# nubot-nudt/LCR-Net

Measured on AMD Instinct MI355X. Metric: scans/s (120k-pt KITTI-shape scan -> 256-D descriptor), higher is better.
Workload: dtype f32 (K-deep GEMMs, K >= 288 and N >= 64: fp32 operands as bf16 x 3 split, 6 of 9 products on the bf16 matrix cores, fp32 accumulate — error vs fp64 <= the fp32-MFMA kernel's; every other GEMM, KPConv and attention: fp32 MFMA); 1 GPU; configs[1]: batch of 8 synthetic 64-beam scans (~120k pts, 0.3 m voxel -> ~16k pts), voxelise + 3 subsamples + 10 radius searches + KPConv encoder + NetVLAD, seeded random weights; distinct_input_batches=4, streams=pre-processing stream (own host thread, 2 batches ahead) + 2 encoder stream(s), parallelism=scan-parallel x1, all-gather of descriptors

## Files before the change

### include/lcr_hip.h

```cpp
#ifndef LCR_HIP_H
#define LCR_HIP_H
#include <stddef.h>
#include <stdint.h>
#ifdef __cplusplus
extern "C" {
#endif

#define LCR_OK 0
#define LCR_EARG (-1)
#define LCR_ESPACE (-2)
#define LCR_EHIP (-3)

#define LCR_STATUS_KEY_OVERFLOW 1u
#define LCR_STATUS_LEN_MISMATCH 2u
#define LCR_GN_REPLICAS 8

const char* lcr_last_error(void);
void lcr_ktimer_enable(int on);
void lcr_ktimer_sample(int every);
void lcr_ktimer_kinds(unsigned mask);
int lcr_ktimer_read(int kind, int max_records, double* seconds, int64_t* meta);
int lcr_ktimer_read2(int kind, int max_records, double* seconds, double* seconds_kernel, int64_t* meta);
int lcr_stream_spin(int microseconds, void* stream);
int lcr_version(void);

int lcr_grid_subsample_ws_bytes(int64_t n_cap, int B, size_t* bytes);
int lcr_grid_subsample(const float* xyz, const int64_t* len, int B, int64_t n_cap, float voxel,
                       float* out_xyz, int64_t* out_len, uint32_t* status,
                       void* ws, size_t ws_bytes, void* stream);
int lcr_grid_subsample_ex(const float* xyz, const int64_t* len, int B, int64_t n_cap, float voxel, int key_bits_hint,
                          float* out_xyz, int64_t* out_len, uint32_t* status,
                          void* ws, size_t ws_bytes, void* stream);
int lcr_grid_subsample_rows(const float* xyz, int row_floats, const int64_t* len, int B, int64_t n_cap, float voxel, int key_bits_hint,
                            float* out_xyz, int64_t* out_len, uint32_t* status,
                            void* ws, size_t ws_bytes, void* stream);
int lcr_hashmap_order_host(const uint64_t* keys_host, int64_t n, int64_t* order_host);
int lcr_hashmap_bucket_host(const uint64_t* codes_host, int64_t n, int phase, int64_t* out_host);

int lcr_voxel_down_sample_ws_bytes(int64_t n_cap, int B, size_t* bytes);
int lcr_voxel_down_sample(const float* rows, int row_floats, int out_cols, const int64_t* len, int B, int64_t n_cap, double voxel,
                          int key_bits_hint, float* out_f32, double* out_f64, int64_t* out_len, uint32_t* status,
                          void* ws, size_t ws_bytes, void* stream);

int lcr_support_grid_ws_bytes(int64_t ns_cap, int B, size_t* bytes);
int lcr_support_grid_build(const float* s, const int64_t* slen, int B, int64_t ns_cap, float radius,
                           uint32_t* status, void* grid_ws, size_t grid_ws_bytes, void* stream);
int lcr_radius_query(const float* q, const int64_t* qlen, int B, int64_t nq_cap,
                     const void* grid_ws, int64_t ns_cap , float radius, int limit,
                     int64_t* out_idx64, int32_t* out_idx32, int32_t* out_cnt, void* stream);
int lcr_radius_query_ordered(const float* q, const int64_t* qlen, int B, int64_t nq_cap,
                             const void* grid_ws, int64_t ns_cap, float radius, int limit,
                             int64_t* out_idx64, int32_t* out_idx32, int32_t* out_cnt, const int32_t* q_order, void* stream);
typedef struct LcrRadiusQuery {
    const float*   q;
    const int64_t* qlen;
    int64_t        nq_cap;
    const void*    grid_ws;
    int64_t        ns_cap;
    float          radius;
    int            limit;
    int32_t*       out_idx32;
    const int32_t* q_order;
} LcrRadiusQuery;
#define LCR_RADIUS_QUERY_MULTI_MAX 12
int lcr_radius_query_multi(const LcrRadiusQuery* list, int n, int B, void* stream);
int lcr_support_grid_build_ex(const float* s, const int64_t* slen, int B, int64_t ns_cap, float radius,
                              uint32_t* status, void* grid_ws, size_t grid_ws_bytes, int32_t* order, void* stream);
int lcr_support_grid_order(const void* grid_ws, int64_t ns_cap, int B, int32_t* order, void* stream);
int lcr_radius_search_ws_bytes(int64_t nq_cap, int64_t ns_cap, int B, size_t* bytes);
int lcr_radius_search(const float* q, const float* s, const int64_t* qlen, const int64_t* slen, int B,
                      int64_t nq_cap, int64_t ns_cap, float radius, int limit,
                      int64_t* out_idx64, int32_t* out_idx32, int32_t* out_cnt, uint32_t* status,
                      void* ws, size_t ws_bytes, void* stream);

#define LCR_MAX_STAGES 8
typedef struct LcrPrecomputeLayout {
  int     num_stages, B, upsampling;
  int64_t n_raw;
  int     limits[LCR_MAX_STAGES];
  int64_t cap[LCR_MAX_STAGES];
  size_t  off_points[LCR_MAX_STAGES];
  size_t  off_lengths[LCR_MAX_STAGES];
  size_t  off_order[LCR_MAX_STAGES];
  size_t  off_neighbors[LCR_MAX_STAGES];
  size_t  off_subsampling[LCR_MAX_STAGES];
  size_t  off_upsampling[LCR_MAX_STAGES];
  size_t  out_bytes, ws_bytes;
} LcrPrecomputeLayout;
int lcr_precompute_layout(int64_t n0, int B, int num_stages, const int* limits, int upsampling, int64_t n_raw,
                          LcrPrecomputeLayout* layout);
int lcr_precompute_batch(const float* points0, const int64_t* lengths0, const LcrPrecomputeLayout* layout, float voxel_size,
                         float radius, float raw_voxel, int key_bits_hint, void* out, size_t out_bytes, void* ws, size_t ws_bytes,
                         int64_t* lengths_host, uint32_t* status_host, void* stream);
int lcr_precompute_batch_rows(const float* points0, int raw_row_floats, const int64_t* lengths0, const LcrPrecomputeLayout* layout,
                              float voxel_size, float radius, float raw_voxel, int key_bits_hint, void* out, size_t out_bytes, void* ws,
                              size_t ws_bytes, int64_t* lengths_host, uint32_t* status_host, void* stream);
int lcr_precompute_ws_bytes_ex(const LcrPrecomputeLayout* layout, int raw_method, size_t* bytes);
int lcr_precompute_batch_rows_ex(const float* points0, int raw_row_floats, const int64_t* lengths0, const LcrPrecomputeLayout* layout,
                                 float voxel_size, float radius, double raw_voxel, int raw_method, int key_bits_hint, void* out,
                                 size_t out_bytes, void* ws, size_t ws_bytes, int64_t* lengths_host, uint32_t* status_host, void* stream);

int lcr_gemm_f32(const float* A, const float* B, float* C, int64_t M, int N, int K, int transA, int transB,
                 const float* bias, const float* rowdiv, const int64_t* seg_len, int S, int groups, double* stats,
                 void* stream);
int lcr_split_bf16x3(const float* w, int64_t n, uint16_t* planes, void* stream);
int lcr_split_bf16x3_tiles(const float* w, int N, int K, uint16_t* tiles, void* stream);
int lcr_gemm_f32_bsplit(const float* A, const uint16_t* Bs_tiles, float* C, int64_t M, int N, int K, const float* bias, const float* rowdiv,
                        const int64_t* seg_len, int S, int groups, double* stats, void* stream);
int lcr_gemm_f32_masked(const float* A, const float* B, float* C, int64_t M, int N, int K, const float* bias, const float* rowdiv,
                        const int64_t* seg_len, int S, int groups, double* stats, const uint16_t* row_mask, int block_k, void* stream);
int lcr_gemm_f32_bsplit_masked(const float* A, const uint16_t* Bs_tiles, float* C, int64_t M, int N, int K, const float* bias,
                               const float* rowdiv, const int64_t* seg_len, int S, int groups, double* stats, const uint16_t* row_mask,
                               int block_k, void* stream);
int lcr_kpconv_mask_ok(int64_t M, int N, int K, int split);
int lcr_gemm_f32_anorm(const float* A, const float* B, float* C, int64_t M, int N, int K, const float* bias,
                       const double* a_stats, const float* a_gamma, const float* a_beta, int a_groups, float a_eps,
                       float a_slope, const int64_t* seg_len, int S, int groups, double* stats, void* stream);
int lcr_gemm_f32_batched_ta(const float* A, const float* B, float* C, int64_t M, int N, int count, const int* k_host,
                            const int64_t* a_off_host, const int64_t* b_off_host, const int64_t* c_off_host, void* stream);
int lcr_kpconv_aggregate(const float* s_feats, const uint8_t* s_pos, const float* q_pts, const float* s_pts,
                         const void* idx, int idx_is_64, int64_t M, int64_t Ns, int H, int C,
                         const float* kernel_points_host, float sigma, float* A, float* nn,
                         const int32_t* order , void* stream);
#define LCR_KP_VALID_FIRST 1
int lcr_kpconv_aggregate_ex(const float* s_feats, const uint8_t* s_pos, const float* q_pts, const float* s_pts,
                            const void* idx, int idx_is_64, int64_t M, int64_t Ns, int H, int C,
                            const float* kernel_points_host, float sigma, float* A, float* nn,
                            const int32_t* order, int flags, void* stream);
int lcr_kpconv_aggregate_mask(const float* s_feats, const uint8_t* s_pos, const float* q_pts, const float* s_pts,
                              const void* idx, int idx_is_64, int64_t M, int64_t Ns, int H, int C,
                              const float* kernel_points_host, float sigma, float* A, float* nn, uint16_t* mask,
                              const int32_t* order, int flags, void* stream);
int lcr_kpconv_fused(const float* s_feats, const uint8_t* s_pos, const float* q_pts, const float* s_pts, const void* idx,
                     int idx_is_64, int64_t M, int64_t Ns, int H, int C, const float* kernel_points_host, float sigma,
                     const float* W, const float* bias, float* out, const int64_t* seg_len, int S, int groups, double* stats,
                     const int32_t* order, void* stream);
int lcr_kpconv_cin1(const float* s_feats, const float* q_pts, const float* s_pts, const void* idx, int idx_is_64,
                    int64_t M, int64_t Ns, int H, const float* kernel_points_host, float sigma, const float* W,
                    const float* bias, int Cout, float* out, const int32_t* order, void* stream);
int lcr_maxpool(const float* x, const void* idx, int idx_is_64, int64_t M, int64_t Ns, int H, int C, float* out,
                const int32_t* order, void* stream);
int lcr_row_positive(const float* x, int64_t N, int C, uint8_t* pos, void* stream);
int lcr_groupnorm_stats(const float* x, int64_t N, int C, int groups, const int64_t* seg_len, int S, double* stats, void* stream);
int lcr_groupnorm_apply(const float* x, const double* stats, const float* gamma, const float* beta, const float* res,
                        const double* res_stats, const float* res_gamma, const float* res_beta, float* y, int64_t N, int C,
                        int groups, const int64_t* seg_len, int S, float eps, float slope, int act, uint8_t* pos, void* stream);

#define LCR_ENC_BLOCKS 10
typedef struct LcrUnaryW {
  const float *w, *b;
  const float *gn_w, *gn_b;
  const uint16_t* w_split;
} LcrUnaryW;
typedef struct LcrBlockW {
  int   cin, cout, strided;
  float sigma;
  const float* kernel_points_host;
  const float *kp_w, *kp_b;
  const float* kp_wt;
  const uint16_t* kp_wt_split;
  const float *normconv_w, *normconv_b;
  LcrUnaryW unary1, unary2, shortcut;
} LcrBlockW;
typedef struct LcrEncoderW {
  int   groups, c1_cout;
  float c1_sigma;
  const float* c1_kernel_points_host;
  const float *c1_w, *c1_b;
  const float *c1_gn_w, *c1_gn_b;
  LcrBlockW blocks[LCR_ENC_BLOCKS];
} LcrEncoderW;
int lcr_encoder_ws_bytes(const LcrEncoderW* W, const int64_t* n_host, int S, size_t* bytes);
int lcr_encoder_forward(const LcrEncoderW* W, const float* feats0, const float* const* points, const int32_t* const* neighbors,
                        const int32_t* const* subsampling, const int32_t* const* order, const int64_t* const* seg_len, int S,
                        const int64_t* n_host, const int64_t* seg_min_rows_host, const int* limits, float* const* out_feats, void* ws,
                        size_t ws_bytes, void* stream);
#define LCR_ENC_LISTS_VALID_FIRST 1u
int lcr_encoder_forward_ex(const LcrEncoderW* W, const float* feats0, const float* const* points, const int32_t* const* neighbors,
                           const int32_t* const* subsampling, const int32_t* const* order, const int64_t* const* seg_len, int S,
                           const int64_t* n_host, const int64_t* seg_min_rows_host, const int* limits, float* const* out_feats,
                           unsigned flags, void* ws, size_t ws_bytes, void* stream);

typedef struct LcrNetvladWeights {
  const float* cluster_weights;
  const float* cluster_weights2;
  const float* hidden1_weights;
  const float *bn1_w, *bn1_b, *bn1_mean, *bn1_var;
  const float *bn2_w, *bn2_b, *bn2_mean, *bn2_var;
  const float* gating_weights;
  const float *gbn_w, *gbn_b, *gbn_mean, *gbn_var;
} LcrNetvladWeights;
int lcr_netvlad_ws_bytes(int64_t n_rows, int S, size_t* bytes);
int lcr_netvlad_forward(const float* feats , const int64_t* seg_len_host, int S,
                        const LcrNetvladWeights* weights_host, float* out , void* ws, size_t ws_bytes, void* stream);

int lcr_rotary_embed(float* x, const float* theta, int64_t N, int heads, void* stream);
int lcr_attention_f32(const float* q, const float* k, const float* v, int64_t Nq, int64_t Nk, int heads, int head_dim,
                      float* out, void* stream);
int lcr_attention_seg_f32(const float* q, const float* k, const float* v, const int64_t* q_len_host, const int64_t* k_len_host, int P,
                          int heads, int head_dim, float* out, void* stream);
int lcr_attention_topk_f32(const float* q, const float* k, const float* v, const int64_t* q_len_host, const int64_t* k_len_host,
                           const int* kk_host, int P, int heads, int head_dim, float* out, void* stream);
int lcr_add_layernorm(const float* a, const float* b, const float* gamma, const float* beta, int64_t N, int D, float eps,
                      float* y, void* stream);
int lcr_relu_inplace(float* x, int64_t n, void* stream);

#define LCR_ROFORMER_MAX_BLOCKS 16
typedef struct LcrLinearW {
  const float *w, *b;
} LcrLinearW;
typedef struct LcrRoformerLayerW {
  LcrLinearW   q, k, v, lin;
  const float *ln1_w, *ln1_b;
  float        ln1_eps;
  LcrLinearW   expand, squeeze;
  const float *ln2_w, *ln2_b;
  float        ln2_eps;
} LcrRoformerLayerW;
typedef struct LcrRoformerW {
  int        d_in, d_model, d_out, heads, num_blocks;
  int        block_is_self[LCR_ROFORMER_MAX_BLOCKS];
  LcrLinearW emb1, emb2, in_proj, out_proj;
  LcrRoformerLayerW layers[LCR_ROFORMER_MAX_BLOCKS];
} LcrRoformerW;
int lcr_roformer_ws_bytes(const LcrRoformerW* W, int64_t n_rows, size_t* bytes);
int lcr_roformer_forward(const LcrRoformerW* W, const float* points, const float* feats, const int64_t* lens0_host, const int64_t* lens1_host,
                         int P, float* out, float* theta_out, void* ws, size_t ws_bytes, void* stream);

int lcr_retrieval_ws_bytes(int64_t Q, int64_t C, size_t* bytes);
int lcr_retrieval_topk(const float* queries , int64_t Q, int64_t q0, const float* database , int64_t C,
                       int D, int k, int exclude, int32_t* out_idx , float* out_d2 ,
                       void* ws, size_t ws_bytes, void* stream);

int lcr_gemm_f32_strided_batched(const float* A, const float* B, float* C, int64_t M, int N, int K, int transA, int transB,
                                 int64_t strideA, int64_t strideB, int64_t strideC, int count, void* stream);

int lcr_vote_shift(const float* xyz, const float* offsets, int64_t N, float max_range, float* out, void* stream);
int lcr_greedy_nms_ws_bytes(int64_t n_total, size_t* bytes);
int lcr_greedy_nms(const float* pts, const int64_t* len, int B, int64_t n_total, float radius, uint8_t* keep,
                   int64_t* out_len, void* ws, void* stream);
int lcr_neighbor_mean(const float* pts, const void* idx, int idx_is_64, int64_t M, int H, int64_t pad, float* out, void* stream);
int lcr_point_to_node_ws_bytes(int64_t N, int M, size_t* bytes);
int lcr_point_to_node_partition(const float* points, int64_t N, const float* nodes, int M, int K, int32_t* p2n, int64_t* knn,
                                uint8_t* knn_mask, uint8_t* node_mask, uint32_t* status, void* ws, size_t ws_bytes, void* stream);

int lcr_point_to_node_partition_stack(const float* points, const int64_t* point_off, const float* nodes, const int64_t* node_off, int C, int K,
                                      int32_t* p2n_out, int64_t* knn, uint8_t* knn_mask, uint8_t* node_mask, uint32_t* status, void* ws,
                                      size_t ws_bytes, void* stream);
int lcr_build_padded_scores(const float* raw, const uint8_t* row_mask, const uint8_t* col_mask, int64_t B, int M, int N,
                            float scale, const float* alpha, float inf_val, float* S, void* stream);
int lcr_log_sinkhorn(float* S, const uint8_t* row_mask, const uint8_t* col_mask, int64_t B, int M, int N, int iters,
                     float inf_val, float* uv_ws, void* stream);
int lcr_log_sinkhorn_ws_floats(int64_t B, int M, int N, size_t* floats);
int lcr_log_sinkhorn_form(int64_t B, int M, int N, int* form);
int lcr_log_sinkhorn_ex(float* S, const uint8_t* row_mask, const uint8_t* col_mask, int64_t B, int M, int N, int iters,
                        float inf_val, float* uv_ws, size_t uv_floats, void* stream);
int lcr_top1_matching_ws_bytes(int64_t B, int M, int N, size_t* bytes);
int lcr_top1_matching(const float* logS, int64_t B, int M, int N, const uint8_t* row_mask, const uint8_t* col_mask,
                      int64_t* total, int32_t* out_bij, float* out_score, void* ws, size_t ws_bytes, void* stream);
int lcr_top1_matching_ex(const float* logS, int64_t B, int M, int N, const uint8_t* row_mask, const uint8_t* col_mask, int mutual,
                         int64_t* total, int32_t* out_bij, float* out_score, void* ws, size_t ws_bytes, void* stream);
int lcr_patch_scores(const float* feats_a, int64_t Na, const float* feats_b, int64_t Nb, int C, const int64_t* idx_a, const int64_t* idx_b,
                     const uint8_t* mask_a, const uint8_t* mask_b, int64_t P, int K, float scale, const float* alpha, float inf_val, float* S,
                     void* stream);
int lcr_topk_matching_ws_bytes(int64_t B, int M, int N, size_t* bytes);
int lcr_topk_matching(const float* logS, int64_t B, int M, int N, const uint8_t* row_mask, const uint8_t* col_mask, int K, int mutual,
                      int64_t* total, int32_t* out_bij, float* out_score, void* ws, size_t ws_bytes, void* stream);
int lcr_topk_matching_ex(const float* logS, int64_t B, int M, int N, const uint8_t* row_mask, const uint8_t* col_mask, int K, int mutual,
                         int use_dustbin, float confidence_threshold, const float* global_scores, int64_t* total, int32_t* out_bij,
                         float* out_score, void* ws, size_t ws_bytes, void* stream);
int lcr_upsample_concat(const float* x, int64_t Nx, int C1, const void* idx, int idx_is_64, int H, const float* skip, int C2,
                        int64_t N, float* out, void* stream);
int lcr_gather_rows(const float* src, int64_t pad, int C, const int64_t* idx, int64_t R, float* out, void* stream);
int lcr_procrustes_batched(const float* src, const float* ref, const float* w, const int32_t* start, int P, float eps, float* T, void* stream);
int lcr_inlier_count(const float* T, int P, const float* src, const float* ref, int n, float radius, const int32_t* start,
                     int min_count, int32_t* counts, int32_t* best, void* stream);
int lcr_lgr_ws_bytes(int64_t n, int H, int S, size_t* bytes);
int lcr_local_global_registration(const float* src, const float* ref, const float* score, int64_t n, const int32_t* hyp_start, int H,
                                  const int32_t* seg_hyp_start, int S, float radius, int min_count, int steps, float* T_out,
                                  float* hyp_out, int32_t* counts_out, int32_t* best_out, void* ws, size_t ws_bytes, void* stream);
int lcr_local_global_registration_ex(const float* src, const float* ref, const float* score, int64_t n, const int32_t* hyp_start, int H,
                                     const int32_t* seg_hyp_start, int S, float radius, int min_count, int steps, int correspondence_limit,
                                     float* T_out, float* hyp_out, int32_t* counts_out, int32_t* best_out, void* ws, size_t ws_bytes,
                                     void* stream);
int lcr_inlier_weights(const float* T_all, const int32_t* sel, const float* src, const float* ref, const float* score, int n,
                       float radius, float* w_out, void* stream);

int lcr_ransac_ws_bytes(int S, int iterations, size_t* bytes);
int lcr_ransac_correspondences(const float* src, const float* ref, const int32_t* start, int S, float thr, int ransac_n, int iterations,
                               uint64_t seed, float* T, int32_t* inliers, float* rmse, int32_t* best_h, float* T_all, int32_t* counts_all,
                               float* sse_all, void* ws, size_t ws_bytes, void* stream);
int lcr_ransac_sample_host(uint64_t seed, int64_t h0, int64_t count, int ransac_n, int64_t n, int32_t* idx_host);
int lcr_ransac_ex_ws_bytes(int S, int iterations, int64_t n_corr, size_t* bytes);
int lcr_ransac_correspondences_ex(const float* src, const float* ref, const int32_t* start, int S, const int32_t* corr, const int32_t* src_start,
                                  const int32_t* ref_start, int64_t n_corr, float thr, int ransac_n, int iterations, uint64_t seed,
                                  float edge_similarity, float checker_distance, float* T, int32_t* inliers, float* rmse, int32_t* best_h,
                                  float* T_all, int32_t* counts_all, float* sse_all, uint8_t* reject_all, void* ws, size_t ws_bytes, void* stream);

int lcr_feature_nn_ws_bytes(int S, int64_t nq, int64_t nd, size_t* bytes);
int lcr_feature_nn(const float* qf, const float* df, const int32_t* q_start, const int32_t* d_start, int S, int C, int64_t nq, int64_t nd,
                   int32_t* nn, float* d2, void* ws, size_t ws_bytes, void* stream);
int lcr_feature_correspondences_ws_bytes(int S, size_t* bytes);
int lcr_feature_correspondences(const int32_t* nn_sr, const int32_t* src_start, const int32_t* nn_rs, const int32_t* ref_start, int S, int min_rows,
                                int32_t* corr, int32_t* start, int32_t* mutual_used, void* ws, size_t ws_bytes, void* stream);

#define LCR_STATUS_CAP_EXCEEDED 4u
int lcr_node_correspondences_ws_bytes(const int64_t* point_off, const int64_t* node_off, int P, int K, size_t* bytes);
int lcr_node_correspondences(const float* points, const int64_t* point_off, const float* nodes, const int64_t* node_off, const int64_t* knn,
                             const uint8_t* knn_mask, const uint8_t* node_mask, const float* transforms, int P, int K, double pos_radius,
                             int64_t cap, int32_t* corr, float* overlap, int32_t* start, uint32_t* status, void* ws, size_t ws_bytes,
                             void* stream);

int lcr_icp_ws_bytes(int S, int64_t ns, int64_t nt, size_t* bytes);
int lcr_icp_point_to_point(const float* src, const int64_t* src_len, const float* tgt, const int64_t* tgt_len, int S, const double* init,
                           float max_correspondence_distance, int max_iteration, double relative_fitness, double relative_rmse, double* T,
                           double* fitness, double* inlier_rmse, int32_t* iterations, int32_t* corr, double* T_hist, double* fitness_hist,
                           double* rmse_hist, int check_every, void* ws, size_t ws_bytes, void* stream);

int lcr_icp_plane_ws_bytes(int S, int64_t ns, int64_t nt, size_t* bytes);
int lcr_icp_point_to_plane(const float* src, const int64_t* src_len, const float* tgt, const int64_t* tgt_len, const float* tgt_normals, int S,
                           const double* init, float max_correspondence_distance, int max_iteration, double relative_fitness,
                           double relative_rmse, double* T, double* fitness, double* inlier_rmse, int32_t* iterations, int32_t* corr,
                           double* T_hist, double* fitness_hist, double* rmse_hist, int check_every, void* ws, size_t ws_bytes, void* stream);

int lcr_normals_ws_bytes(int B, int64_t n, size_t* bytes);
int lcr_estimate_normals(const float* points, const int64_t* lengths, int B, float radius, int max_nn, const float* viewpoint, float* normals,
                         float* curvature, int32_t* count, void* ws, size_t ws_bytes, void* stream);

int lcr_fpfh_ws_bytes(int B, int64_t n, int max_nn, size_t* bytes);
int lcr_fpfh(const float* points, const float* normals, const int64_t* lengths, int B, float radius, int max_nn, float* features, float* spfh,
             int32_t* count, void* ws, size_t ws_bytes, void* stream);

int lcr_range_images_ws_bytes(int B, size_t* bytes);
int lcr_range_images(const float* points, const int64_t* lengths, int B, int H, int W, double fov_up, double fov_down, double max_range,
                     float* images, int32_t* valid, void* ws, size_t ws_bytes, void* stream);
int lcr_scan_overlap_ws_bytes(int B, int64_t P, size_t* bytes);
int lcr_scan_overlap(const float* points, const int64_t* lengths, int B, const float* images, const int32_t* valid, const int32_t* pairs,
                     const double* rel, int64_t P, int H, int W, double fov_up, double fov_down, double max_range, double eps, int32_t* counts,
                     int32_t* status, void* ws, size_t ws_bytes, void* stream);

#define LCR_STATUS_INDEX_RANGE 8u
#define LCR_GAP_LABELS_POINTS 0
#define LCR_GAP_LABELS_OVERLAPS 1
int lcr_gap_loss_ws_bytes(int64_t rows, int64_t cols, size_t* bytes);
int lcr_gap_loss(const float* S, const int64_t* soff, const int64_t* roff, const int64_t* coff, const int32_t* seg_start, int64_t B, int P,
                 int n_max, int m_max, int64_t elems, int64_t rows, int64_t cols, int source, const float* p_pts, const float* q_pts,
                 const float* transforms, double positive_radius, const int64_t* corr, const float* overlaps, const int32_t* corr_start,
                 int64_t C, int64_t c_max, double positive_overlap, const uint8_t* pmask, const uint8_t* qmask, double gamma, float* terms,
                 int32_t* kept, uint8_t* labels, double* line_pos, double* line_hinge, int32_t* line_count, int32_t* line_active,
                 uint32_t* status, void* ws, size_t ws_bytes, void* stream);
int lcr_gap_loss_grad(const float* S, const int64_t* soff, const int64_t* roff, const int64_t* coff, const int32_t* seg_start, int64_t B,
                      int P, int n_max, int m_max, int64_t elems, int64_t rows, int64_t cols, double gamma, const float* upstream,
                      const int32_t* kept, const uint8_t* labels, const double* line_pos, const double* line_hinge,
                      const int32_t* line_count, const int32_t* line_active, float* dS, void* stream);
int lcr_min_dist(const float* A, const int32_t* a_start, int64_t na, const float* D, const int32_t* d_start, int64_t nd,
                 const uint8_t* valid, int P, int64_t q_max, float* dist, int32_t* arg, float* mean, int32_t* count, void* stream);
int lcr_min_dist_grad(const float* A, const int32_t* a_start, int64_t na, const float* D, const int32_t* d_start, int64_t nd,
                      const uint8_t* valid, int P, int64_t q_max, const int32_t* arg, const float* dist, const int32_t* count,
                      const float* upstream, float* dA, void* stream);

#ifdef __cplusplus
}
#endif
#endif
```

### lcr-net_amd/_lib.py

```python
import ctypes
import os

import torch

_PKG = os.path.dirname(os.path.abspath(__file__))
LIB_PATH = os.path.join(_PKG, "liblcr_hip.so")

_lib = None

c_f32p = ctypes.c_void_p
c_vp = ctypes.c_void_p
c_i64 = ctypes.c_int64
c_int = ctypes.c_int
c_float = ctypes.c_float
c_size_p = ctypes.POINTER(ctypes.c_size_t)
c_size_t = ctypes.c_size_t

_SIGS = {
    "lcr_last_error": (ctypes.c_char_p, []),
    "lcr_version": (c_int, []),
    "lcr_support_grid_ws_bytes": (c_int, [c_i64, c_int, c_size_p]),
    "lcr_support_grid_build": (c_int, [c_vp, c_vp, c_int, c_i64, c_float, c_vp, c_vp, ctypes.c_size_t, c_vp]),
    "lcr_precompute_layout": (c_int, [c_i64, c_int, c_int, c_vp, c_int, c_i64, c_vp]),
    "lcr_precompute_batch": (c_int, [c_vp, c_vp, c_vp, c_float, c_float, c_float, c_int, c_vp, c_size_t, c_vp, c_size_t, c_vp, c_vp, c_vp]),
    "lcr_precompute_batch_rows": (c_int, [c_vp, c_int, c_vp, c_vp, c_float, c_float, c_float, c_int, c_vp, c_size_t, c_vp, c_size_t, c_vp, c_vp, c_vp]),
    "lcr_precompute_ws_bytes_ex": (c_int, [c_vp, c_int, c_size_p]),
    "lcr_precompute_batch_rows_ex": (c_int, [c_vp, c_int, c_vp, c_vp, c_float, c_float, ctypes.c_double, c_int, c_int, c_vp, c_size_t, c_vp, c_size_t,
                                             c_vp, c_vp, c_vp]),
    "lcr_radius_query_multi": (c_int, [c_vp, c_int, c_int, c_vp]),
    "lcr_radius_query": (c_int, [c_vp, c_vp, c_int, c_i64, c_vp, c_i64, c_float, c_int, c_vp, c_vp, c_vp, c_vp]),
    "lcr_stream_spin": (c_int, [c_int, c_vp]),
    "lcr_radius_query_ordered": (c_int, [c_vp, c_vp, c_int, c_i64, c_vp, c_i64, c_float, c_int, c_vp, c_vp, c_vp, c_vp, c_vp]),
    "lcr_radius_search_ws_bytes": (c_int, [c_i64, c_i64, c_int, c_size_p]),
    "lcr_radius_search": (c_int, [c_vp, c_vp, c_vp, c_vp, c_int, c_i64, c_i64, c_float, c_int, c_vp, c_vp, c_vp, c_vp,
                                  c_vp, ctypes.c_size_t, c_vp]),
    "lcr_grid_subsample_ws_bytes": (c_int, [c_i64, c_int, c_size_p]),
    "lcr_grid_subsample": (c_int, [c_vp, c_vp, c_int, c_i64, c_float, c_vp, c_vp, c_vp, c_vp, ctypes.c_size_t, c_vp]),
    "lcr_grid_subsample_ex": (c_int, [c_vp, c_vp, c_int, c_i64, c_float, c_int, c_vp, c_vp, c_vp, c_vp, ctypes.c_size_t, c_vp]),
    "lcr_grid_subsample_rows": (c_int, [c_vp, c_int, c_vp, c_int, c_i64, c_float, c_int, c_vp, c_vp, c_vp, c_vp, ctypes.c_size_t, c_vp]),
    "lcr_hashmap_order_host": (c_int, [c_vp, c_i64, c_vp]),
    "lcr_hashmap_bucket_host": (c_int, [c_vp, c_i64, c_int, c_vp]),
    "lcr_voxel_down_sample_ws_bytes": (c_int, [c_i64, c_int, c_size_p]),
    "lcr_voxel_down_sample": (c_int, [c_vp, c_int, c_int, c_vp, c_int, c_i64, ctypes.c_double, c_int, c_vp, c_vp, c_vp, c_vp, c_vp, ctypes.c_size_t,
                                      c_vp]),
    "lcr_gemm_f32": (c_int, [c_vp, c_vp, c_vp, c_i64, c_int, c_int, c_int, c_int, c_vp, c_vp, c_vp, c_int, c_int, c_vp, c_vp]),
    "lcr_gemm_f32_anorm": (c_int, [c_vp, c_vp, c_vp, c_i64, c_int, c_int, c_vp, c_vp, c_vp, c_vp, c_int, c_float, c_float, c_vp, c_int,
                                   c_int, c_vp, c_vp]),
    "lcr_ktimer_enable": (None, [c_int]),
    "lcr_ktimer_sample": (None, [c_int]),
    "lcr_ktimer_kinds": (None, [ctypes.c_uint]),
    "lcr_ktimer_read": (c_int, [c_int, c_int, c_vp, c_vp]),
    "lcr_ktimer_read2": (c_int, [c_int, c_int, c_vp, c_vp, c_vp]),
    "lcr_encoder_ws_bytes": (c_int, [c_vp, c_vp, c_int, c_size_p]),
    "lcr_encoder_forward": (c_int, [c_vp, c_vp, c_vp, c_vp, c_vp, c_vp, c_vp, c_int, c_vp, c_vp, c_vp, c_vp, c_vp, c_size_t, c_vp]),
    "lcr_roformer_ws_bytes": (c_int, [c_vp, c_i64, c_size_p]),
    "lcr_roformer_forward": (c_int, [c_vp, c_vp, c_vp, c_vp, c_vp, c_int, c_vp, c_vp, c_vp, c_size_t, c_vp]),
    "lcr_encoder_forward_ex": (c_int, [c_vp, c_vp, c_vp, c_vp, c_vp, c_vp, c_vp, c_int, c_vp, c_vp, c_vp, c_vp, ctypes.c_uint, c_vp, c_size_t, c_vp]),
    "lcr_kpconv_aggregate": (c_int, [c_vp, c_vp, c_vp, c_vp, c_vp, c_int, c_i64, c_i64, c_int, c_int, c_vp, c_float, c_vp, c_vp, c_vp, c_vp]),
    "lcr_kpconv_aggregate_mask": (c_int, [c_vp, c_vp, c_vp, c_vp, c_vp, c_int, c_i64, c_i64, c_int, c_int, c_vp, c_float, c_vp, c_vp, c_vp, c_vp,
                                          c_int, c_vp]),
    "lcr_kpconv_fused": (c_int, [c_vp, c_vp, c_vp, c_vp, c_vp, c_int, c_i64, c_i64, c_int, c_int, c_vp, c_float, c_vp, c_vp, c_vp, c_vp, c_int,
                                 c_int, c_vp, c_vp, c_vp]),
    "lcr_kpconv_cin1": (c_int, [c_vp, c_vp, c_vp, c_vp, c_int, c_i64, c_i64, c_int, c_vp, c_float, c_vp, c_vp, c_int, c_vp, c_vp, c_vp]),
    "lcr_maxpool": (c_int, [c_vp, c_vp, c_int, c_i64, c_i64, c_int, c_int, c_vp, c_vp, c_vp]),
    "lcr_support_grid_order": (c_int, [c_vp, c_i64, c_int, c_vp, c_vp]),
    "lcr_row_positive": (c_int, [c_vp, c_i64, c_int, c_vp, c_vp]),
    "lcr_groupnorm_stats": (c_int, [c_vp, c_i64, c_int, c_int, c_vp, c_int, c_vp, c_vp]),
    "lcr_groupnorm_apply": (c_int, [c_vp, c_vp, c_vp, c_vp, c_vp, c_vp, c_vp, c_vp, c_vp, c_i64, c_int, c_int, c_vp, c_int,
                                    c_float, c_float, c_int, c_vp, c_vp]),
    "lcr_rotary_embed": (c_int, [c_vp, c_vp, c_i64, c_int, c_vp]),
    "lcr_attention_f32": (c_int, [c_vp, c_vp, c_vp, c_i64, c_i64, c_int, c_int, c_vp, c_vp]),
    "lcr_attention_seg_f32": (c_int, [c_vp, c_vp, c_vp, c_vp, c_vp, c_int, c_int, c_int, c_vp, c_vp]),
    "lcr_attention_topk_f32": (c_int, [c_vp, c_vp, c_vp, c_vp, c_vp, c_vp, c_int, c_int, c_int, c_vp, c_vp]),
    "lcr_add_layernorm": (c_int, [c_vp, c_vp, c_vp, c_vp, c_i64, c_int, c_float, c_vp, c_vp]),
    "lcr_relu_inplace": (c_int, [c_vp, c_i64, c_vp]),
    "lcr_retrieval_ws_bytes": (c_int, [c_i64, c_i64, c_size_p]),
    "lcr_retrieval_topk": (c_int, [c_vp, c_i64, c_i64, c_vp, c_i64, c_int, c_int, c_int, c_vp, c_vp, c_vp, ctypes.c_size_t, c_vp]),
    "lcr_gemm_f32_strided_batched": (c_int, [c_vp, c_vp, c_vp, c_i64, c_int, c_int, c_int, c_int, c_i64, c_i64, c_i64, c_int, c_vp]),
    "lcr_gemm_f32_batched_ta": (c_int, [c_vp, c_vp, c_vp, c_i64, c_int, c_int, c_vp, c_vp, c_vp, c_vp, c_vp]),
    "lcr_vote_shift": (c_int, [c_vp, c_vp, c_i64, c_float, c_vp, c_vp]),
    "lcr_greedy_nms_ws_bytes": (c_int, [c_i64, c_size_p]),
    "lcr_greedy_nms": (c_int, [c_vp, c_vp, c_int, c_i64, c_float, c_vp, c_vp, c_vp, c_vp]),
    "lcr_neighbor_mean": (c_int, [c_vp, c_vp, c_int, c_i64, c_int, c_i64, c_vp, c_vp]),
    "lcr_point_to_node_ws_bytes": (c_int, [c_i64, c_int, c_size_p]),
    "lcr_point_to_node_partition": (c_int, [c_vp, c_i64, c_vp, c_int, c_int, c_vp, c_vp, c_vp, c_vp, c_vp, c_vp, ctypes.c_size_t, c_vp]),
    "lcr_point_to_node_partition_stack": (c_int, [c_vp, c_vp, c_vp, c_vp, c_int, c_int, c_vp, c_vp, c_vp, c_vp, c_vp, c_vp, ctypes.c_size_t, c_vp]),
    "lcr_build_padded_scores": (c_int, [c_vp, c_vp, c_vp, c_i64, c_int, c_int, c_float, c_vp, c_float, c_vp, c_vp]),
    "lcr_log_sinkhorn": (c_int, [c_vp, c_vp, c_vp, c_i64, c_int, c_int, c_int, c_float, c_vp, c_vp]),
    "lcr_log_sinkhorn_ws_floats": (c_int, [c_i64, c_int, c_int, c_size_p]),
    "lcr_log_sinkhorn_form": (c_int, [c_i64, c_int, c_int, ctypes.POINTER(c_int)]),
    "lcr_split_bf16x3": (c_int, [c_vp, c_i64, c_vp, c_vp]),
    "lcr_split_bf16x3_tiles": (c_int, [c_vp, c_int, c_int, c_vp, c_vp]),
    "lcr_gemm_f32_bsplit": (c_int, [c_vp, c_vp, c_vp, c_i64, c_int, c_int, c_vp, c_vp, c_vp, c_int, c_int, c_vp, c_vp]),
    "lcr_gemm_f32_bsplit_masked": (c_int, [c_vp, c_vp, c_vp, c_i64, c_int, c_int, c_vp, c_vp, c_vp, c_int, c_int, c_vp, c_vp, c_int, c_vp]),
    "lcr_gemm_f32_masked": (c_int, [c_vp, c_vp, c_vp, c_i64, c_int, c_int, c_vp, c_vp, c_vp, c_int, c_int, c_vp, c_vp, c_int, c_vp]),
    "lcr_kpconv_mask_ok": (c_int, [c_i64, c_int, c_int, c_int]),
    "lcr_log_sinkhorn_ex": (c_int, [c_vp, c_vp, c_vp, c_i64, c_int, c_int, c_int, c_float, c_vp, ctypes.c_size_t, c_vp]),
    "lcr_top1_matching_ws_bytes": (c_int, [c_i64, c_int, c_int, c_size_p]),
    "lcr_top1_matching": (c_int, [c_vp, c_i64, c_int, c_int, c_vp, c_vp, c_vp, c_vp, c_vp, c_vp, ctypes.c_size_t, c_vp]),
    "lcr_top1_matching_ex": (c_int, [c_vp, c_i64, c_int, c_int, c_vp, c_vp, c_int, c_vp, c_vp, c_vp, c_vp, ctypes.c_size_t, c_vp]),
    "lcr_topk_matching_ws_bytes": (c_int, [c_i64, c_int, c_int, c_size_p]),
    "lcr_topk_matching": (c_int, [c_vp, c_i64, c_int, c_int, c_vp, c_vp, c_int, c_int, c_vp, c_vp, c_vp, c_vp, ctypes.c_size_t, c_vp]),
    "lcr_patch_scores": (c_int, [c_vp, c_i64, c_vp, c_i64, c_int, c_vp, c_vp, c_vp, c_vp, c_i64, c_int, c_float, c_vp, c_float, c_vp, c_vp]),
    "lcr_topk_matching_ex": (c_int, [c_vp, c_i64, c_int, c_int, c_vp, c_vp, c_int, c_int, c_int, c_float, c_vp, c_vp, c_vp, c_vp, c_vp, ctypes.c_size_t,
                                     c_vp]),
    "lcr_local_global_registration_ex": (c_int, [c_vp, c_vp, c_vp, c_i64, c_vp, c_int, c_vp, c_int, c_float, c_int, c_int, c_int, c_vp, c_vp, c_vp, c_vp,
                                                 c_vp, ctypes.c_size_t, c_vp]),
    "lcr_upsample_concat": (c_int, [c_vp, c_i64, c_int, c_vp, c_int, c_int, c_vp, c_int, c_i64, c_vp, c_vp]),
    "lcr_gather_rows": (c_int, [c_vp, c_i64, c_int, c_vp, c_i64, c_vp, c_vp]),
    "lcr_procrustes_batched": (c_int, [c_vp, c_vp, c_vp, c_vp, c_int, c_float, c_vp, c_vp]),
    "lcr_inlier_count": (c_int, [c_vp, c_int, c_vp, c_vp, c_int, c_float, c_vp, c_int, c_vp, c_vp, c_vp]),
    "lcr_inlier_weights": (c_int, [c_vp, c_vp, c_vp, c_vp, c_vp, c_int, c_float, c_vp, c_vp]),
    "lcr_lgr_ws_bytes": (c_int, [c_i64, c_int, c_int, c_size_p]),
    "lcr_local_global_registration": (c_int, [c_vp, c_vp, c_vp, c_i64, c_vp, c_int, c_vp, c_int, c_float, c_int, c_int, c_vp, c_vp, c_vp, c_vp, c_vp,
                                              ctypes.c_size_t, c_vp]),
    "lcr_netvlad_ws_bytes": (c_int, [c_i64, c_int, c_size_p]),
    "lcr_netvlad_forward": (c_int, [c_vp, c_vp, c_int, c_vp, c_vp, c_vp, ctypes.c_size_t, c_vp]),
    "lcr_ransac_ws_bytes": (c_int, [c_int, c_int, c_size_p]),
    "lcr_ransac_correspondences": (c_int, [c_vp, c_vp, c_vp, c_int, c_float, c_int, c_int, ctypes.c_uint64, c_vp, c_vp, c_vp, c_vp, c_vp, c_vp, c_vp,
                                           c_vp, ctypes.c_size_t, c_vp]),
    "lcr_ransac_sample_host": (c_int, [ctypes.c_uint64, c_i64, c_i64, c_int, c_i64, c_vp]),
    "lcr_ransac_ex_ws_bytes": (c_int, [c_int, c_int, c_i64, c_size_p]),
    "lcr_ransac_correspondences_ex": (c_int, [c_vp, c_vp, c_vp, c_int, c_vp, c_vp, c_vp, c_i64, c_float, c_int, c_int, ctypes.c_uint64, c_float,
                                              c_float, c_vp, c_vp, c_vp, c_vp, c_vp, c_vp, c_vp, c_vp, c_vp, ctypes.c_size_t, c_vp]),
    "lcr_feature_nn_ws_bytes": (c_int, [c_int, c_i64, c_i64, c_size_p]),
    "lcr_feature_nn": (c_int, [c_vp, c_vp, c_vp, c_vp, c_int, c_int, c_i64, c_i64, c_vp, c_vp, c_vp, ctypes.c_size_t, c_vp]),
    "lcr_feature_correspondences_ws_bytes": (c_int, [c_int, c_size_p]),
    "lcr_feature_correspondences": (c_int, [c_vp, c_vp, c_vp, c_vp, c_int, c_int, c_vp, c_vp, c_vp, c_vp, ctypes.c_size_t, c_vp]),
    "lcr_node_correspondences_ws_bytes": (c_int, [c_vp, c_vp, c_int, c_int, c_size_p]),
    "lcr_node_correspondences": (c_int, [c_vp, c_vp, c_vp, c_vp, c_vp, c_vp, c_vp, c_vp, c_int, c_int, ctypes.c_double, c_i64, c_vp, c_vp, c_vp,
                                         c_vp, c_vp, ctypes.c_size_t, c_vp]),
    "lcr_icp_ws_bytes": (c_int, [c_int, c_i64, c_i64, c_size_p]),
    "lcr_icp_point_to_point": (c_int, [c_vp, c_vp, c_vp, c_vp, c_int, c_vp, c_float, c_int, ctypes.c_double, ctypes.c_double, c_vp, c_vp, c_vp, c_vp,
                                       c_vp, c_vp, c_vp, c_vp, c_int, c_vp, ctypes.c_size_t, c_vp]),
    "lcr_icp_plane_ws_bytes": (c_int, [c_int, c_i64, c_i64, c_size_p]),
    "lcr_icp_point_to_plane": (c_int, [c_vp, c_vp, c_vp, c_vp, c_vp, c_int, c_vp, c_float, c_int, ctypes.c_double, ctypes.c_double, c_vp, c_vp,
                                       c_vp, c_vp, c_vp, c_vp, c_vp, c_vp, c_int, c_vp, ctypes.c_size_t, c_vp]),
    "lcr_normals_ws_bytes": (c_int, [c_int, c_i64, c_size_p]),
    "lcr_estimate_normals": (c_int, [c_vp, c_vp, c_int, c_float, c_int, c_vp, c_vp, c_vp, c_vp, c_vp, ctypes.c_size_t, c_vp]),
    "lcr_fpfh_ws_bytes": (c_int, [c_int, c_i64, c_int, c_size_p]),
    "lcr_fpfh": (c_int, [c_vp, c_vp, c_vp, c_int, c_float, c_int, c_vp, c_vp, c_vp, c_vp, ctypes.c_size_t, c_vp]),
    "lcr_range_images_ws_bytes": (c_int, [c_int, c_size_p]),
    "lcr_range_images": (c_int, [c_vp, c_vp, c_int, c_int, c_int, ctypes.c_double, ctypes.c_double, ctypes.c_double, c_vp, c_vp, c_vp,
                                 ctypes.c_size_t, c_vp]),
    "lcr_scan_overlap_ws_bytes": (c_int, [c_int, c_i64, c_size_p]),
    "lcr_scan_overlap": (c_int, [c_vp, c_vp, c_int, c_vp, c_vp, c_vp, c_vp, c_i64, c_int, c_int, ctypes.c_double, ctypes.c_double, ctypes.c_double,
                                 ctypes.c_double, c_vp, c_vp, c_vp, ctypes.c_size_t, c_vp]),
    "lcr_gap_loss_ws_bytes": (c_int, [c_i64, c_i64, c_size_p]),
    "lcr_gap_loss": (c_int, [c_vp, c_vp, c_vp, c_vp, c_vp, c_i64, c_int, c_int, c_int, c_i64, c_i64, c_i64, c_int, c_vp, c_vp, c_vp,
                             ctypes.c_double, c_vp, c_vp, c_vp, c_i64, c_i64, ctypes.c_double, c_vp, c_vp, ctypes.c_double, c_vp, c_vp, c_vp,
                             c_vp, c_vp, c_vp, c_vp, c_vp, c_vp, ctypes.c_size_t, c_vp]),
    "lcr_gap_loss_grad": (c_int, [c_vp, c_vp, c_vp, c_vp, c_vp, c_i64, c_int, c_int, c_int, c_i64, c_i64, c_i64, ctypes.c_double, c_vp, c_vp,
                                  c_vp, c_vp, c_vp, c_vp, c_vp, c_vp, c_vp]),
    "lcr_min_dist": (c_int, [c_vp, c_vp, c_i64, c_vp, c_vp, c_i64, c_vp, c_int, c_i64, c_vp, c_vp, c_vp, c_vp, c_vp]),
    "lcr_min_dist_grad": (c_int, [c_vp, c_vp, c_i64, c_vp, c_vp, c_i64, c_vp, c_int, c_i64, c_vp, c_vp, c_vp, c_vp, c_vp, c_vp]),
}


_RELEASES_GIL = {"lcr_roformer_forward", "lcr_precompute_batch", "lcr_precompute_batch_rows", "lcr_precompute_batch_rows_ex", "lcr_hashmap_bucket_host", "lcr_encoder_forward", "lcr_encoder_forward_ex", "lcr_ktimer_read",
                 "lcr_ktimer_read2", "lcr_hashmap_order_host", "lcr_ransac_sample_host", "lcr_icp_point_to_point", "lcr_icp_point_to_plane", "lcr_netvlad_forward", "lcr_log_sinkhorn", "lcr_log_sinkhorn_ex",
                 "lcr_local_global_registration", "lcr_local_global_registration_ex", "lcr_retrieval_topk", "lcr_stream_spin"}


def build():
    import importlib.util
    spec = importlib.util.spec_from_file_location("_lcr_build", os.path.join(_PKG, "csrc", "build.py"))
    mod = importlib.util.module_from_spec(spec)
    spec.loader.exec_module(mod)
    return mod.build()


def lib():
    global _lib
    if _lib is None:
        if not os.path.exists(LIB_PATH):
            raise RuntimeError(
                "liblcr_hip.so not found at %s — build it with `python lcr-net_amd/csrc/build.py` "
                "(there is no CPU fallback for the lcr-net_amd hot path)" % LIB_PATH)
        L = ctypes.CDLL(LIB_PATH)
        for name, (res, args) in _SIGS.items():
            if not hasattr(L, name):
                continue
            fn = getattr(L, name)
            fn.restype = res
            fn.argtypes = args
        if os.environ.get("LCR_CTYPES_KEEP_GIL", "1") != "0":
            K = ctypes.PyDLL(LIB_PATH)
            for name, (res, args) in _SIGS.items():
                if name in _RELEASES_GIL or not hasattr(K, name):
                    continue
                fn = getattr(K, name)
                fn.restype = res
                fn.argtypes = args
                setattr(L, name, fn)
        _lib = L
    return _lib


def check(rc, what):
    if rc != 0:
        msg = lib().lcr_last_error()
        raise RuntimeError("%s failed (rc=%d): %s" % (what, rc, msg.decode() if msg else ""))


def ptr(t):
    return ctypes.c_void_p(t.data_ptr()) if t is not None else ctypes.c_void_p(0)


def stream_ptr(device=None):
    idx = device.index if isinstance(device, torch.device) else None
    if idx is None:
        idx = torch.cuda.current_device() if not isinstance(device, int) else device
    return ctypes.c_void_p(torch._C._cuda_getCurrentRawStream(idx))


def require_cuda(*tensors):
    for t in tensors:
        if t is not None and not t.is_cuda:
            raise RuntimeError("lcr-net_amd ops run on the GPU only: got a %s tensor (no CPU fallback)" % t.device)


def workspace(nbytes, device):
    return torch.empty(max(int(nbytes), 256), dtype=torch.uint8, device=device)
```

### lcr-net_amd/csrc/encoder.hip

```cpp
#include <algorithm>
#include <cstdlib>
#include <cstring>

#include "common.h"

#define TURN(call) ([&]() { LaunchTurn turn_; return (call); }())

namespace lcr {

constexpr float ENC_GN_EPS = 1e-5f;
constexpr float ENC_SLOPE = 0.1f;

struct Arena {
  char*  base;
  size_t off, cap;
  template <typename T>
  T* take(size_t n) {
    const size_t o = off;
    off = align_up(off + n * sizeof(T));
    return (base && off <= cap) ? reinterpret_cast<T*>(base + o) : nullptr;
  }
};

struct StageIO {
  const float*   pts;
  const int64_t* seg;
  const int32_t* order;
  int64_t        n;
  int64_t        min_rows;
};

struct StatsPool {
  double* base;
  size_t  off, cap;
  int     S, groups;
  double* take() {
    const size_t n = static_cast<size_t>(GN_REPLICAS) * S * groups * 2;
    if (off + n > cap) return nullptr;
    double* p = base + off;
    off += n;
    return p;
  }
};

static size_t stats_doubles(int S, int groups) { return static_cast<size_t>(GN_REPLICAS) * S * groups * 2 * 44; }

static int unary_raw(const LcrUnaryW& u, const float* x, int64_t n, int cin, int cout, const StageIO& st, StatsPool& sp, Arena& ws,
                     float** y_out, double** stats_out, hipStream_t s) {
  float* y = ws.take<float>(static_cast<size_t>(n) * cout);
  double* stats = sp.take();
  if (!y || !stats) return LCR_ESPACE;
  const bool split = u.w_split && cin >= 288 && cin % 32 == 0 && cout >= 64;
  int rc = split ? TURN(lcr_gemm_f32_bsplit(x, u.w_split, y, n, cout, cin, u.b, nullptr, st.seg, sp.S, sp.groups, stats, s))
                 : TURN(lcr_gemm_f32(x, u.w, y, n, cout, cin, 0, 1, u.b, nullptr, st.seg, sp.S, sp.groups, stats, s));
  *y_out = y;
  *stats_out = stats;
  return rc;
}

static int residual_block(const LcrBlockW& b, const float* s_feats, const StageIO& q, const StageIO& sup, const void* idx, int H,
                          StatsPool& sp, Arena& ws, float* out, unsigned enc_flags, hipStream_t s) {
  const int mid = b.cout / 4, g = sp.groups;
  const int64_t M = q.n, Ns = sup.n;
  int rc;
  const float* x = s_feats;
  uint8_t* pos = ws.take<uint8_t>(static_cast<size_t>(Ns));
  if (!pos) return LCR_ESPACE;
  if (b.unary1.w) {
    float* y1;
    double* st1;
    if ((rc = unary_raw(b.unary1, s_feats, Ns, b.cin, mid, sup, sp, ws, &y1, &st1, s))) return rc;
    float* x1 = ws.take<float>(static_cast<size_t>(Ns) * mid);
    if (!x1) return LCR_ESPACE;
    if ((rc = TURN(lcr_groupnorm_apply(y1, st1, b.unary1.gn_w, b.unary1.gn_b, nullptr, nullptr, nullptr, nullptr, x1, Ns, mid, g, sup.seg, sp.S,
                                  ENC_GN_EPS, ENC_SLOPE, 1, pos, s))))
      return rc;
    x = x1;
  } else if ((rc = TURN(lcr_row_positive(s_feats, Ns, b.cin, pos, s)))) {
    return rc;
  }
  float* A = ws.take<float>(static_cast<size_t>(M) * 15 * mid);
  float* nn = ws.take<float>(static_cast<size_t>(M));
  float* kpo = ws.take<float>(static_cast<size_t>(M) * mid);
  uint16_t* kmask = ws.take<uint16_t>(static_cast<size_t>(M));
  double* stc = sp.take();
  if (!A || !nn || !kpo || !kmask || !stc) return LCR_ESPACE;
  static const bool vf_env_off = getenv("LCR_KP_VALID_FIRST") && atoi(getenv("LCR_KP_VALID_FIRST")) == 0;
  const int vf_flag = ((enc_flags & LCR_ENC_LISTS_VALID_FIRST) && !vf_env_off) ? LCR_KP_VALID_FIRST : 0;
  static const bool fused32 = getenv("LCR_KPCONV_FUSED") != nullptr;
  if (fused32 && mid == 32 && sp.S <= 64) {
    if ((rc = TURN(lcr_kpconv_fused(x, pos, q.pts, sup.pts, idx, 0, M, Ns, H, mid, b.kernel_points_host, b.sigma, b.kp_w, b.kp_b, kpo, q.seg, sp.S, g,
                                    stc, q.order, s))))
      return rc;
  } else {
    const bool split = b.kp_wt_split && mid >= 64;
    if (!((split || b.kp_wt) && lcr_kpconv_mask_ok(M, mid, 15 * mid, split))) kmask = nullptr;
    if ((rc = TURN(lcr_kpconv_aggregate_mask(x, pos, q.pts, sup.pts, idx, 0, M, Ns, H, mid, b.kernel_points_host, b.sigma, A, nn, kmask, q.order, vf_flag,
                                             s))))
      return rc;
    if (split) {
      if ((rc = TURN(kmask ? lcr_gemm_f32_bsplit_masked(A, b.kp_wt_split, kpo, M, mid, 15 * mid, b.kp_b, nn, q.seg, sp.S, g, stc, kmask, mid, s)
                           : lcr_gemm_f32_bsplit(A, b.kp_wt_split, kpo, M, mid, 15 * mid, b.kp_b, nn, q.seg, sp.S, g, stc, s))))
        return rc;
    } else if (kmask) {
      if ((rc = TURN(lcr_gemm_f32_masked(A, b.kp_wt, kpo, M, mid, 15 * mid, b.kp_b, nn, q.seg, sp.S, g, stc, kmask, mid, s)))) return rc;
    } else if ((rc = TURN(b.kp_wt ? lcr_gemm_f32(A, b.kp_wt, kpo, M, mid, 15 * mid, 0, 1, b.kp_b, nn, q.seg, sp.S, g, stc, s)
                                  : lcr_gemm_f32(A, b.kp_w, kpo, M, mid, 15 * mid, 0, 0, b.kp_b, nn, q.seg, sp.S, g, stc, s)))) return rc;
  }
  float* y;
  double* sty;
  static const bool no_anorm = getenv("LCR_NO_NORM_ON_LOAD") != nullptr;
  if (!no_anorm && mid <= 256 && mid % 4 == 0 && b.cout > 32 && q.min_rows >= 64) {
    y = ws.take<float>(static_cast<size_t>(M) * b.cout);
    sty = sp.take();
    if (!y || !sty) return LCR_ESPACE;
    if ((rc = TURN(lcr_gemm_f32_anorm(kpo, b.unary2.w, y, M, b.cout, mid, b.unary2.b, stc, b.normconv_w, b.normconv_b, g, ENC_GN_EPS, ENC_SLOPE,
                                      q.seg, sp.S, g, sty, s))))
      return rc;
  } else {
    float* x2 = ws.take<float>(static_cast<size_t>(M) * mid);
    if (!x2) return LCR_ESPACE;
    if ((rc = TURN(lcr_groupnorm_apply(kpo, stc, b.normconv_w, b.normconv_b, nullptr, nullptr, nullptr, nullptr, x2, M, mid, g, q.seg, sp.S, ENC_GN_EPS,
                                  ENC_SLOPE, 1, nullptr, s))))
      return rc;
    if ((rc = unary_raw(b.unary2, x2, M, mid, b.cout, q, sp, ws, &y, &sty, s))) return rc;
  }
  const float* res = s_feats;
  if (b.strided) {
    float* pooled = ws.take<float>(static_cast<size_t>(M) * b.cin);
    if (!pooled) return LCR_ESPACE;
    if ((rc = TURN(lcr_maxpool(s_feats, idx, 0, M, Ns, H, b.cin, pooled, q.order, s)))) return rc;
    res = pooled;
  }
  const double* str = nullptr;
  if (b.shortcut.w) {
    float* r;
    double* st;
    if ((rc = unary_raw(b.shortcut, res, M, b.cin, b.cout, q, sp, ws, &r, &st, s))) return rc;
    res = r;
    str = st;
  }
  return TURN(lcr_groupnorm_apply(y, sty, b.unary2.gn_w, b.unary2.gn_b, res, str, str ? b.shortcut.gn_w : nullptr, str ? b.shortcut.gn_b : nullptr, out,
                             M, b.cout, g, q.seg, sp.S, ENC_GN_EPS, ENC_SLOPE, 1, nullptr, s));
}

static size_t block_ws_bytes(const LcrBlockW& b, int64_t M, int64_t Ns) {
  Arena a{nullptr, 0, ~size_t(0)};
  const int mid = b.cout / 4;
  a.take<uint8_t>(Ns);
  a.take<float>(static_cast<size_t>(Ns) * mid);
  a.take<float>(static_cast<size_t>(Ns) * mid);
  a.take<float>(static_cast<size_t>(M) * 15 * mid);
  a.take<float>(M);
  a.take<float>(static_cast<size_t>(M) * mid);
  a.take<uint16_t>(static_cast<size_t>(M));
  a.take<float>(static_cast<size_t>(M) * mid);
  a.take<float>(static_cast<size_t>(M) * b.cout);
  a.take<float>(static_cast<size_t>(M) * b.cin);
  a.take<float>(static_cast<size_t>(M) * b.cout);
  return a.off;
}

static const int BLOCK_Q[LCR_ENC_BLOCKS] = {0, 1, 1, 1, 2, 2, 2, 3, 3, 3};
static const int BLOCK_S[LCR_ENC_BLOCKS] = {0, 0, 1, 1, 1, 2, 2, 2, 3, 3};

}

using namespace lcr;

extern "C" int lcr_encoder_ws_bytes(const LcrEncoderW* W, const int64_t* n_host, int S, size_t* bytes) {
  if (!W || !n_host || !bytes || S < 1) return LCR_EARG;
  size_t blk = 0, pp = 0;
  for (int i = 0; i < LCR_ENC_BLOCKS; ++i) {
    blk = std::max(blk, block_ws_bytes(W->blocks[i], n_host[BLOCK_Q[i]], n_host[BLOCK_S[i]]));
    pp = std::max(pp, align_up(sizeof(float) * static_cast<size_t>(n_host[BLOCK_Q[i]]) * W->blocks[i].cout));
  }
  pp = std::max(pp, align_up(sizeof(float) * static_cast<size_t>(n_host[0]) * W->c1_cout * 2));
  *bytes = blk + 2 * pp + align_up(sizeof(double) * stats_doubles(S, W->groups)) + 4096;
  return LCR_OK;
}

extern "C" int lcr_encoder_forward(const LcrEncoderW* W, const float* feats0, const float* const* points, const int32_t* const* neighbors,
                                   const int32_t* const* subsampling, const int32_t* const* order, const int64_t* const* seg_len, int S,
                                   const int64_t* n_host, const int64_t* seg_min_rows_host, const int* limits, float* const* out_feats,
                                   void* ws, size_t ws_bytes, void* stream) {
  return lcr_encoder_forward_ex(W, feats0, points, neighbors, subsampling, order, seg_len, S, n_host, seg_min_rows_host, limits, out_feats, 0u, ws,
                                ws_bytes, stream);
}

extern "C" int lcr_encoder_forward_ex(const LcrEncoderW* W, const float* feats0, const float* const* points, const int32_t* const* neighbors,
                                      const int32_t* const* subsampling, const int32_t* const* order, const int64_t* const* seg_len, int S,
                                      const int64_t* n_host, const int64_t* seg_min_rows_host, const int* limits, float* const* out_feats,
                                      unsigned flags, void* ws, size_t ws_bytes, void* stream) {
  if (!W || !feats0 || !points || !neighbors || !subsampling || !seg_len || !n_host || !limits || !out_feats || !ws || S < 1) {
    set_error("lcr_encoder_forward: bad argument");
    return LCR_EARG;
  }
  size_t need = 0;
  lcr_encoder_ws_bytes(W, n_host, S, &need);
  if (ws_bytes < need) {
    set_error("lcr_encoder_forward: workspace too small (%zu < %zu)", ws_bytes, need);
    return LCR_ESPACE;
  }
  hipStream_t s = static_cast<hipStream_t>(stream);
  StageIO st[4];
  for (int i = 0; i < 4; ++i) st[i] = StageIO{points[i], seg_len[i], order ? order[i] : nullptr, n_host[i], seg_min_rows_host ? seg_min_rows_host[i] : 0};
  Arena top{static_cast<char*>(ws), 0, ws_bytes};
  StatsPool sp{top.take<double>(stats_doubles(S, W->groups)), 0, stats_doubles(S, W->groups), S, W->groups};
  size_t pp = 0;
  for (int i = 0; i < LCR_ENC_BLOCKS; ++i) pp = std::max(pp, sizeof(float) * static_cast<size_t>(n_host[BLOCK_Q[i]]) * W->blocks[i].cout);
  pp = std::max(pp, sizeof(float) * static_cast<size_t>(n_host[0]) * W->c1_cout * 2);
  float* ping = reinterpret_cast<float*>(top.take<char>(pp));
  float* pong = reinterpret_cast<float*>(top.take<char>(pp));
  const size_t scratch0 = top.off;
  if (!sp.base || !ping || !pong) return LCR_ESPACE;
  hipMemsetAsync(sp.base, 0, sizeof(double) * sp.cap, s);

  int rc;
  float* cur;
  {
    const int64_t n0 = n_host[0];
    float* raw = ping;
    float* f = ping + static_cast<size_t>(n0) * W->c1_cout;
    double* stt = sp.take();
    if ((rc = TURN(lcr_kpconv_cin1(feats0, st[0].pts, st[0].pts, neighbors[0], 0, n0, n0, limits[0], W->c1_kernel_points_host, W->c1_sigma, W->c1_w,
                              W->c1_b, W->c1_cout, raw, st[0].order, s))))
      return rc;
    if ((rc = TURN(lcr_groupnorm_stats(raw, n0, W->c1_cout, W->groups, st[0].seg, S, stt, s)))) return rc;
    if ((rc = TURN(lcr_groupnorm_apply(raw, stt, W->c1_gn_w, W->c1_gn_b, nullptr, nullptr, nullptr, nullptr, f, n0, W->c1_cout, W->groups, st[0].seg, S,
                                  ENC_GN_EPS, ENC_SLOPE, 1, nullptr, s))))
      return rc;
    cur = f;
  }
  static const int STAGE_LAST[4] = {0, 3, 6, 9};
  for (int i = 0; i < LCR_ENC_BLOCKS; ++i) {
    const int qs = BLOCK_Q[i], ss = BLOCK_S[i];
    const bool strided = qs != ss;
    const void* idx = strided ? static_cast<const void*>(subsampling[ss]) : static_cast<const void*>(neighbors[qs]);
    const int H = limits[ss];
    float* out = nullptr;
    for (int k = 0; k < 4; ++k)
      if (STAGE_LAST[k] == i) out = out_feats[k];
    if (!out) out = (cur >= ping && cur < ping + pp / sizeof(float)) ? pong : ping;
    Arena scratch{static_cast<char*>(ws), scratch0, ws_bytes};
    if ((rc = residual_block(W->blocks[i], cur, st[qs], st[ss], idx, H, sp, scratch, out, flags, s))) {
      if (rc == LCR_ESPACE) set_error("lcr_encoder_forward: block %d ran out of workspace", i);
      return rc;
    }
    cur = out;
  }
  return check_launch("lcr_encoder_forward");
}
```

### lcr-net_amd/csrc/gemm_f32.hip

```cpp
#include <cstdio>
#include <cstdlib>
#include <map>
#include <mutex>
#include <type_traits>

#include "common.h"

namespace lcr {

typedef float floatx16 __attribute__((ext_vector_type(16)));

constexpr int GM_BK = 32;
constexpr int GM_T = 256;

constexpr int GM_MAX_BATCH = 64;
struct GemmBatch {
  int     count;
  int     strided;
  int     k[GM_MAX_BATCH];
  int64_t a_off[GM_MAX_BATCH], b_off[GM_MAX_BATCH], c_off[GM_MAX_BATCH];
};

struct GemmEpilogue {
  const float*   bias;
  const float*   rowdiv;
  const int64_t* seg_len;
  int            S;
  int            groups;
  double*        stats;
};

struct ANorm {
  const double* stats;
  const float*  gamma;
  const float*  beta;
  int           groups;
  float         eps, slope;
};
constexpr int AN_KMAX = 256;

__device__ __forceinline__ float4 ld4(const float* p) { return *reinterpret_cast<const float4*>(p); }

template <int R, int LD, bool VEC, bool RM = false>
struct LoaderT {
  static constexpr int PIECES = R * 8 / GM_T;
  float4 reg[PIECES];
  unsigned okmask;
  int kb;
  __device__ __forceinline__ void load(const float* __restrict__ src, int64_t rows_total, int K, int64_t r0, int k0) {
    kb = k0;
#pragma unroll
    for (int j = 0; j < PIECES; ++j) {
      const int f = threadIdx.x + GM_T * j;
      const int row = f >> 3, c4 = f & 7;
      int64_t gr = r0 + row;
      gr = gr < rows_total ? gr : rows_total - 1;
      const int gk = k0 + c4 * 4;
      if (VEC) {
        const bool ok = gk < K;
        reg[j] = ld4(src + gr * K + (ok ? gk : 0));
        okmask = j == 0 ? (ok ? 1u : 0u) : (okmask | (ok ? (1u << j) : 0u));
      } else {
        const float* p = src + gr * K;
        float4 v;
        v.x = gk + 0 < K ? p[gk + 0] : 0.f;
        v.y = gk + 1 < K ? p[gk + 1] : 0.f;
        v.z = gk + 2 < K ? p[gk + 2] : 0.f;
        v.w = gk + 3 < K ? p[gk + 3] : 0.f;
        reg[j] = v;
        okmask = ~0u;
      }
    }
  }
  __device__ __forceinline__ void store_piece(float* __restrict__ S, int j) const {
    const int f = threadIdx.x + GM_T * j;
    const int row = f >> 3, c4 = f & 7;
    const bool ok = (okmask >> j) & 1u;
    if (RM) {
      *reinterpret_cast<float4*>(&S[row * LD + c4 * 4]) = ok ? reg[j] : make_float4(0.f, 0.f, 0.f, 0.f);
      return;
    }
    S[(c4 * 4 + 0) * LD + row] = ok ? reg[j].x : 0.f;
    S[(c4 * 4 + 1) * LD + row] = ok ? reg[j].y : 0.f;
    S[(c4 * 4 + 2) * LD + row] = ok ? reg[j].z : 0.f;
    S[(c4 * 4 + 3) * LD + row] = ok ? reg[j].w : 0.f;
  }
  __device__ __forceinline__ void store(float* __restrict__ S) const {
#pragma unroll
    for (int j = 0; j < PIECES; ++j) store_piece(S, j);
  }
  __device__ __forceinline__ void store_norm(float* __restrict__ S, const float* __restrict__ tab, int split, float slope) const {
    static_assert(RM, "normalise-on-load is built for the row-major A tile");
#pragma unroll
    for (int j = 0; j < PIECES; ++j) {
      const int f = threadIdx.x + GM_T * j;
      const int row = f >> 3, c4 = f & 7;
      const bool ok = (okmask >> j) & 1u;
      const float* t = tab + (row >= split ? 2 * AN_KMAX : 0) + (ok ? kb + c4 * 4 : 0);
      const float4 sc = *reinterpret_cast<const float4*>(t), sh = *reinterpret_cast<const float4*>(t + AN_KMAX);
      float4 v;
      v.x = fmaf(reg[j].x, sc.x, sh.x), v.y = fmaf(reg[j].y, sc.y, sh.y), v.z = fmaf(reg[j].z, sc.z, sh.z), v.w = fmaf(reg[j].w, sc.w, sh.w);
      v.x = v.x > 0.f ? v.x : v.x * slope, v.y = v.y > 0.f ? v.y : v.y * slope;
      v.z = v.z > 0.f ? v.z : v.z * slope, v.w = v.w > 0.f ? v.w : v.w * slope;
      *reinterpret_cast<float4*>(&S[row * LD + c4 * 4]) = ok ? v : make_float4(0.f, 0.f, 0.f, 0.f);
    }
  }
};

template <int W, int LD, bool VEC>
struct LoaderN {
  static constexpr int PIECES = 8 * W / GM_T;
  float4 reg[PIECES];
  unsigned okmask;
  __device__ __forceinline__ void load(const float* __restrict__ src, int64_t cols_total, int K, int64_t c0, int k0) {
#pragma unroll
    for (int j = 0; j < PIECES; ++j) {
      const int f = threadIdx.x + GM_T * j;
      const int kr = f / (W / 4), c4 = f % (W / 4);
      const int gk = k0 + kr;
      const int64_t gc = c0 + c4 * 4;
      const bool kok = gk < K;
      const float* p = src + static_cast<int64_t>(kok ? gk : 0) * cols_total;
      if (VEC) {
        const bool ok = kok && gc < cols_total;
        reg[j] = ld4(p + (gc < cols_total ? gc : 0));
        okmask = j == 0 ? (ok ? 1u : 0u) : (okmask | (ok ? (1u << j) : 0u));
      } else {
        float4 v;
        v.x = (kok && gc + 0 < cols_total) ? p[gc + 0] : 0.f;
        v.y = (kok && gc + 1 < cols_total) ? p[gc + 1] : 0.f;
        v.z = (kok && gc + 2 < cols_total) ? p[gc + 2] : 0.f;
        v.w = (kok && gc + 3 < cols_total) ? p[gc + 3] : 0.f;
        reg[j] = v;
        okmask = ~0u;
      }
    }
  }
  __device__ __forceinline__ void store_piece(float* __restrict__ S, int j) const {
    const int f = threadIdx.x + GM_T * j;
    const int kr = f / (W / 4), c4 = f % (W / 4);
    const bool ok = (okmask >> j) & 1u;
    *reinterpret_cast<float4*>(&S[kr * LD + c4 * 4]) = ok ? reg[j] : make_float4(0.f, 0.f, 0.f, 0.f);
  }
  __device__ __forceinline__ void store(float* __restrict__ S) const {
#pragma unroll
    for (int j = 0; j < PIECES; ++j) store_piece(S, j);
  }
};

__device__ __forceinline__ int seg_of_row(const int64_t* __restrict__ seg_len, int S, int64_t row) {
  int s = 0;
  int64_t end = seg_len[0];
  while (s + 1 < S && row >= end) {
    ++s;
    end += seg_len[s];
  }
  return s;
}

template <int BM, int BN, int WM, int WN, int NT>
__device__ __forceinline__ void gemm_epilogue(floatx16 (&acc)[NT], float* __restrict__ C, int64_t M, int N, int64_t m0, int n0, int64_t m_tile,
                                              const GemmEpilogue& ep, const float (&bias_v)[NT], int blk_first, int64_t blk_seg_start,
                                              int64_t blk_seg_end, int wm, int wn, int lane) {
  const bool want_stats = ep.stats != nullptr;
  const int gs = want_stats ? N / ep.groups : 1;
  const int64_t wrow0 = m0 + wm * 32;

  const bool interior = m0 + BM <= M && n0 + BN <= N && M * static_cast<int64_t>(N) < (int64_t(1) << 30);
  if (interior) {
    const unsigned row_l = static_cast<unsigned>(wrow0) + 4u * static_cast<unsigned>(lane >> 5);
#pragma unroll
    for (int j = 0; j < NT; ++j) {
      const unsigned col = static_cast<unsigned>(n0 + wn * (32 * NT) + j * 32 + (lane & 31));
      const float bv = bias_v[j];
      const unsigned off0 = row_l * static_cast<unsigned>(N) + col;
      if (ep.rowdiv) {
#pragma unroll
        for (int r = 0; r < 16; ++r) {
          const unsigned dr = static_cast<unsigned>((r & 3) + 8 * (r >> 2));
          const float v = acc[j][r] / ep.rowdiv[row_l + dr] + bv;
          C[off0 + dr * static_cast<unsigned>(N)] = v;
          acc[j][r] = v;
        }
      } else {
#pragma unroll
        for (int r = 0; r < 16; ++r) {
          const unsigned dr = static_cast<unsigned>((r & 3) + 8 * (r >> 2));
          const float v = acc[j][r] + bv;
          C[off0 + dr * static_cast<unsigned>(N)] = v;
          acc[j][r] = v;
        }
      }
    }
  } else
#pragma unroll
  for (int j = 0; j < NT; ++j) {
    const int col = n0 + wn * (32 * NT) + j * 32 + (lane & 31);
    const float bv = bias_v[j];
#pragma unroll
    for (int r = 0; r < 16; ++r) {
      const int64_t row = wrow0 + (r & 3) + 8 * (r >> 2) + 4 * (lane >> 5);
      float v = acc[j][r];
      if (row < M) {
        if (ep.rowdiv) v = v / ep.rowdiv[row];
        v += bv;
        if (col < N) C[row * N + col] = v;
      } else {
        v = 0.f;
      }
      acc[j][r] = v;
    }
  }

  if (want_stats) {
    __shared__ float s_part[2][2 * WM][BN];
    double* rep = ep.stats + static_cast<int64_t>(m_tile % GN_REPLICAS) * ep.S * ep.groups * 2;
    int64_t seg_start = blk_seg_start, seg_end = blk_seg_end;
    const int64_t blk_last_row = min(m0 + BM - 1, M - 1);
    constexpr int GN_EXACT_ROWS = 32;
    auto exact_segment = [&](int64_t rows) { return rows < GN_EXACT_ROWS && gs <= 32; };
    const bool uniform = blk_last_row < seg_end && !exact_segment(seg_end - seg_start);
    if (uniform) {
#pragma unroll
      for (int j = 0; j < NT; ++j) {
        float s = 0.f, ss = 0.f;
#pragma unroll
        for (int r = 0; r < 16; ++r) {
          s += acc[j][r];
          ss = fmaf(acc[j][r], acc[j][r], ss);
        }
        const int cl = wn * (32 * NT) + j * 32 + (lane & 31);
        s_part[0][2 * wm + (lane >> 5)][cl] = s;
        s_part[1][2 * wm + (lane >> 5)][cl] = ss;
      }
      __syncthreads();
      if (threadIdx.x < BN) {
        const int cl = threadIdx.x;
        double ds = 0.0, dss = 0.0;
#pragma unroll
        for (int r = 0; r < 2 * WM; ++r) {
          ds += static_cast<double>(s_part[0][r][cl]);
          dss += static_cast<double>(s_part[1][r][cl]);
        }
        const int span = gs < 64 ? gs : 64;
        for (int d = 1; d < span; d <<= 1) {
          ds += __shfl_xor(ds, d);
          dss += __shfl_xor(dss, d);
        }
        const int col = n0 + cl;
        if ((cl & (span - 1)) == 0 && col < N) {
          double* d = rep + (static_cast<int64_t>(blk_first) * ep.groups + col / gs) * 2;
          atomicAdd(d, ds);
          atomicAdd(d + 1, dss);
        }
      }
    } else if (wrow0 < M) {
      const int64_t wlast = min(wrow0 + 31, M - 1);
      int sg = blk_first;
      while (sg + 1 < ep.S && wrow0 >= seg_end) {
        ++sg;
        seg_start = seg_end;
        seg_end += ep.seg_len[sg];
      }
      while (true) {
        const bool whole = seg_start <= wrow0 && wlast < seg_end;
#pragma unroll
        for (int j = 0; j < NT; ++j) {
          const int col = n0 + wn * (32 * NT) + j * 32 + (lane & 31);
          double ds, dss;
          if (exact_segment(seg_end - seg_start)) {
            ds = dss = 0.0;
#pragma unroll
            for (int r = 0; r < 16; ++r) {
              const int64_t row = wrow0 + (r & 3) + 8 * (r >> 2) + 4 * (lane >> 5);
              float vf = (row >= seg_start && row < seg_end) ? acc[j][r] : 0.f;
              asm volatile("" : "+v"(vf));
              const double v = vf;
              ds += v;
              dss = fma(v, v, dss);
            }
          } else {
            float s = 0.f, ss = 0.f;
#pragma unroll
            for (int r = 0; r < 16; ++r) {
              const int64_t row = wrow0 + (r & 3) + 8 * (r >> 2) + 4 * (lane >> 5);
              const float v = (whole || (row >= seg_start && row < seg_end)) ? acc[j][r] : 0.f;
              s += v;
              ss = fmaf(v, v, ss);
            }
            ds = s, dss = ss;
          }
          ds += __shfl_xor(ds, 32);
          dss += __shfl_xor(dss, 32);
          const int span = gs < 32 ? gs : 32;
          for (int d = 1; d < span; d <<= 1) {
            ds += __shfl_xor(ds, d);
            dss += __shfl_xor(dss, d);
          }
          if (lane < 32 && (lane & (span - 1)) == 0 && col < N) {
            double* d = rep + (static_cast<int64_t>(sg) * ep.groups + col / gs) * 2;
            atomicAdd(d, ds);
            atomicAdd(d + 1, dss);
          }
        }
        if (wlast < seg_end || sg + 1 >= ep.S) break;
        ++sg;
        seg_start = seg_end;
        seg_end += ep.seg_len[sg];
      }
    }
  }
}

template <int BM, int BN, int WM, int WN, bool TA, bool TB, bool VEC, bool SHORT = false, bool ANORM = false>
__global__ __launch_bounds__(GM_T, SHORT ? 6 : 2) void k_gemm_f32(const float* __restrict__ A, const float* __restrict__ B, float* __restrict__ C,
                                                       int64_t M, int N, int K, GemmEpilogue ep, GemmBatch batch, ANorm an) {
  static_assert(!ANORM || (SHORT && !TA && VEC && BN / (32 * WN) == 1), "normalise-on-load: light form, row-major A");
  static_assert(WM * WN == 4 && BM == 32 * WM, "one 32-row MFMA tile per wavefront along M");
  constexpr int k_begin = 0;
  if (batch.count) {
    const int z = blockIdx.z;
    if (batch.strided) {
      A += static_cast<int64_t>(z) * batch.a_off[0];
      B += static_cast<int64_t>(z) * batch.b_off[0];
      C += static_cast<int64_t>(z) * batch.c_off[0];
      K = batch.k[0];
    } else {
      A += batch.a_off[z];
      B += batch.b_off[z];
      C += batch.c_off[z];
      K = batch.k[z];
    }
  }
  constexpr int NT = BN / (32 * WN);
  constexpr int NBUF = SHORT ? 1 : 2;
  constexpr bool NEWP = NT == 1;
  constexpr bool ARM = NEWP && !TA, BRM = NEWP && TB;
  constexpr int LDR = GM_BK + 4;
  constexpr int LDA = ARM ? LDR : (TA ? BM + 4 : BM + 1);
  constexpr int LDB = BRM ? LDR : (TB ? BN + 1 : BN + 4);
  __shared__ __attribute__((aligned(16))) float As[NBUF][ARM ? BM * LDR : GM_BK * LDA];
  __shared__ __attribute__((aligned(16))) float Bs[NBUF][BRM ? BN * LDR : GM_BK * LDB];

  const int lane = threadIdx.x & 63, w = __builtin_amdgcn_readfirstlane(threadIdx.x >> 6);
  const int wm = w / WN, wn = w % WN;
  const int ntn = (N + BN - 1) / BN;
  const int xcd = blockIdx.x & 7, slot = blockIdx.x >> 3;
  const int64_t m_tile = static_cast<int64_t>(slot / ntn) * 8 + xcd;
  const int64_t m0 = m_tile * BM;
  const int n0 = (slot % ntn) * BN;
  if (m0 >= M) return;

  LoaderT<BM, LDA, VEC, ARM> la_t[NBUF];
  LoaderN<BM, LDA, VEC> la_n[NBUF];
  LoaderT<BN, LDB, VEC, BRM> lb_t[NBUF];
  LoaderN<BN, LDB, VEC> lb_n[NBUF];

  auto gload = [&](int k0, int r) {
    if (TA) la_n[r].load(A, M, K, m0, k0);
    else la_t[r].load(A, M, K, m0, k0);
    if (TB) lb_t[r].load(B, N, K, n0, k0);
    else lb_n[r].load(B, N, K, n0, k0);
  };
  auto sstore = [&](int buf, int r) {
    if (TA) la_n[r].store(As[buf]);
    else la_t[r].store(As[buf]);
    if (TB) lb_t[r].store(Bs[buf]);
    else lb_n[r].store(Bs[buf]);
  };

  constexpr int NACC = (NT == 1 && BM == 128) ? 2 : 1;
  floatx16 acc[NT], acc2[NT];
#pragma unroll
  for (int j = 0; j < NT; ++j)
#pragma unroll
    for (int r = 0; r < 16; ++r) {
      acc[j][r] = 0.f;
      acc2[j][r] = 0.f;
    }

  const int nk = (K + GM_BK - 1) / GM_BK;
  gload(k_begin, 0);
  if (!SHORT) gload(k_begin + GM_BK, NBUF - 1);
  const bool want_stats = ep.stats != nullptr;
  float bias_v[NT];
#pragma unroll
  for (int j = 0; j < NT; ++j) {
    const int col = n0 + (w % WN) * (32 * NT) + j * 32 + (lane & 31);
    bias_v[j] = (ep.bias && col < N) ? ep.bias[col] : 0.f;
  }
  float an_g[2] = {0.f, 0.f}, an_b[2] = {0.f, 0.f};
  if constexpr (ANORM) {
#pragma unroll
    for (int u = 0; u < 2; ++u) {
      const int e = threadIdx.x + u * GM_T;
      if (e < 2 * K) {
        const int k = e >= K ? e - K : e;
        an_g[u] = an.gamma[k];
        an_b[u] = an.beta[k];
      }
    }
  }
  int blk_first = 0;
  int64_t blk_seg_start = 0, blk_seg_end = 0;
  if (want_stats || ANORM) {
    blk_seg_end = ep.seg_len[0];
    while (blk_first + 1 < ep.S && m0 >= blk_seg_end) {
      ++blk_first;
      blk_seg_start = blk_seg_end;
      blk_seg_end += ep.seg_len[blk_first];
    }
  }
  __shared__ __attribute__((aligned(16))) float s_an[ANORM ? 4 * AN_KMAX : 4];
  int an_split = BM;
  if constexpr (ANORM) {
    an_split = static_cast<int>(min(static_cast<int64_t>(BM), blk_seg_end - m0));
    const int gs = K / an.groups;
    __shared__ float2 s_mr[2 * 64];
    for (int e = threadIdx.x; e < 2 * an.groups; e += GM_T) {
      const int slot = e >= an.groups ? 1 : 0, g = e - slot * an.groups;
      const int sg = min(blk_first + slot, ep.S - 1);
      const double cnt = static_cast<double>(ep.seg_len[sg]) * gs;
      double sx = 0.0, sxx = 0.0;
      for (int rep = 0; rep < GN_REPLICAS; ++rep) {
        const int64_t o = ((static_cast<int64_t>(rep) * ep.S + sg) * an.groups + g) * 2;
        sx += an.stats[o];
        sxx += an.stats[o + 1];
      }
      const double mean = sx / cnt;
      const double var = fmax(sxx / cnt - mean * mean, 0.0);
      s_mr[e] = make_float2(static_cast<float>(mean), static_cast<float>(1.0 / sqrt(var + static_cast<double>(an.eps))));
    }
    __syncthreads();
#pragma unroll
    for (int u = 0; u < 2; ++u) {
      const int e = threadIdx.x + u * GM_T;
      if (e < 2 * K) {
        const int slot = e >= K ? 1 : 0, k = e - slot * K;
        const float2 mr = s_mr[slot * an.groups + k / gs];
        const float sc = mr.y * an_g[u];
        s_an[slot * 2 * AN_KMAX + k] = sc;
        s_an[slot * 2 * AN_KMAX + AN_KMAX + k] = fmaf(-mr.x, sc, an_b[u]);
      }
    }
    __syncthreads();
  }
  auto sstore_a0 = [&]() {
    if constexpr (ANORM) la_t[0].store_norm(As[0], s_an, an_split, an.slope);
  };
  if constexpr (ANORM) {
    sstore_a0();
    lb_t[0].store(Bs[0]);
  } else {
    sstore(0, 0);
  }
  __syncthreads();
  const int half = lane >> 5;
  const int a_off = ARM ? (wm * 32 + (lane & 31)) * LDR + half * 16 : half * (NEWP ? 16 : 1) * LDA + wm * 32 + (lane & 31);
  const int b_off = BRM ? (wn * (32 * NT) + (lane & 31)) * LDR + half * 16 : half * (NEWP ? 16 : 1) * LDB + wn * (32 * NT) + (lane & 31);
  auto fetch4_a = [&](const float* as, int q, float (&o)[4]) {
    if (ARM) {
      const float4 v = *reinterpret_cast<const float4*>(as + 4 * q);
      o[0] = v.x, o[1] = v.y, o[2] = v.z, o[3] = v.w;
    } else {
#pragma unroll
      for (int i = 0; i < 4; ++i) o[i] = as[(4 * q + i) * LDA];
    }
  };
  auto fetch4_b = [&](const float* bs, int q, float (&o)[4]) {
    if (BRM) {
      const float4 v = *reinterpret_cast<const float4*>(bs + 4 * q);
      o[0] = v.x, o[1] = v.y, o[2] = v.z, o[3] = v.w;
    } else {
#pragma unroll
      for (int i = 0; i < 4; ++i) o[i] = bs[(4 * q + i) * LDB];
    }
  };
  if constexpr (SHORT) {
    constexpr int KKS = GM_BK / 2, PFS = 4;
    for (int t = 0; t < nk; ++t) {
      if (t > 0) {
        gload(k_begin + t * GM_BK, 0);
        __syncthreads();
        if constexpr (ANORM) {
          sstore_a0();
          lb_t[0].store(Bs[0]);
        } else {
          sstore(0, 0);
        }
        __syncthreads();
      }
      const float* as = As[0] + a_off;
      const float* bs = Bs[0] + b_off;
      static_assert(NEWP, "the light form is only instantiated for single-accumulator tiles");
      float af[2][4], bf[2][4];
      fetch4_a(as, 0, af[0]);
      fetch4_b(bs, 0, bf[0]);
      fetch4_a(as, 1, af[1]);
      fetch4_b(bs, 1, bf[1]);
#pragma unroll
      for (int q = 0; q < KKS / 4; ++q) {
#pragma unroll
        for (int i = 0; i < 4; ++i) acc[0] = __builtin_amdgcn_mfma_f32_32x32x2f32(af[q & 1][i], bf[q & 1][i], acc[0], 0, 0, 0);
        if (q + 2 < KKS / 4) {
          fetch4_a(as, q + 2, af[q & 1]);
          fetch4_b(bs, q + 2, bf[q & 1]);
        }
      }
    }
  } else {
  constexpr int KK = GM_BK / 2;
  constexpr int PF = NT == 1 ? KK : (NT == 2 ? 8 : 4);
  constexpr int PA = BM * 8 / GM_T, PB = BN * 8 / GM_T;
  constexpr int ST0 = KK - (PA + PB) - 1 > 2 ? (KK - (PA + PB)) / 2 : 1;
  auto step = [&](auto buf_c, auto full_c, int t) {
    constexpr int BUF = decltype(buf_c)::value;
    constexpr bool FULL = decltype(full_c)::value;
    if (FULL || t + 2 < nk) gload(k_begin + (t + 2) * GM_BK, BUF);
    const bool do_store = FULL || t + 1 < nk;
    const float* as = As[BUF] + a_off;
    const float* bs = Bs[BUF] + b_off;
    float af[PF], bf[PF][NT];
    if constexpr (NEWP) {
#pragma unroll
      for (int q = 0; q < KK / 4; ++q) {
        float a4[4], b4[4];
        fetch4_a(as, q, a4);
        fetch4_b(bs, q, b4);
#pragma unroll
        for (int i = 0; i < 4; ++i) {
          af[4 * q + i] = a4[i];
          bf[4 * q + i][0] = b4[i];
        }
      }
    } else {
#pragma unroll
      for (int d = 0; d < PF; ++d) {
        af[d] = as[d * 2 * LDA];
#pragma unroll
        for (int j = 0; j < NT; ++j) bf[d][j] = bs[d * 2 * LDB + j * 32];
      }
    }
    __builtin_amdgcn_sched_barrier(0);
#pragma unroll
    for (int kk = 0; kk < KK; ++kk) {
      const int sl = kk % PF;
#pragma unroll
      for (int j = 0; j < NT; ++j) {
        if (NACC == 2 && (kk & 1)) acc2[j] = __builtin_amdgcn_mfma_f32_32x32x2f32(af[sl], bf[sl][j], acc2[j], 0, 0, 0);
        else acc[j] = __builtin_amdgcn_mfma_f32_32x32x2f32(af[sl], bf[sl][j], acc[j], 0, 0, 0);
      }
      if (kk + PF < KK) {
        af[sl] = as[(kk + PF) * 2 * LDA];
#pragma unroll
        for (int j = 0; j < NT; ++j) bf[sl][j] = bs[(kk + PF) * 2 * LDB + j * 32];
      }
      const int piece = kk - ST0;
      if (do_store && piece >= 0 && piece < PA + PB) {
        if (piece < PA) {
          if (TA) la_n[1 - BUF].store_piece(As[1 - BUF], piece);
          else la_t[1 - BUF].store_piece(As[1 - BUF], piece);
        } else {
          if (TB) lb_t[1 - BUF].store_piece(Bs[1 - BUF], piece - PA);
          else lb_n[1 - BUF].store_piece(Bs[1 - BUF], piece - PA);
        }
      }
    }
    __syncthreads();
  };
  int t = 0;
  for (; t + 3 < nk; t += 2) {
    step(std::integral_constant<int, 0>{}, std::true_type{}, t);
    step(std::integral_constant<int, 1>{}, std::true_type{}, t + 1);
  }
  for (; t < nk; t += 2) {
    step(std::integral_constant<int, 0>{}, std::false_type{}, t);
    if (t + 1 >= nk) break;
    step(std::integral_constant<int, 1>{}, std::false_type{}, t + 1);
  }

  }

  if (NACC == 2) {
#pragma unroll
    for (int j = 0; j < NT; ++j)
#pragma unroll
      for (int r = 0; r < 16; ++r) acc[j][r] += acc2[j][r];
  }

  gemm_epilogue<BM, BN, WM, WN, NT>(acc, C, M, N, m0, n0, m_tile, ep, bias_v, blk_first, blk_seg_start, blk_seg_end, wm, wn, lane);
}

template <int N_OUTSTANDING>
__device__ __forceinline__ void wait_vmcnt() {
  asm volatile("s_waitcnt vmcnt(%0)" ::"n"(N_OUTSTANDING) : "memory");
}
__device__ __forceinline__ void glds16(const float* base, unsigned off, unsigned lds_dst) {
  unsigned keep;
  asm volatile("s_mov_b32 %0, m0\n\ts_mov_b32 m0, %3\n\ts_nop 0\n\tglobal_load_lds_dwordx4 %1, %2\n\ts_mov_b32 m0, %0"
               : "=&s"(keep)
               : "v"(off), "s"(base), "s"(lds_dst)
               : "memory");
}

__device__ __forceinline__ void glds16_v(const float* addr, unsigned lds_dst) {
  unsigned keep;
  asm volatile("s_mov_b32 %0, m0\n\ts_mov_b32 m0, %2\n\ts_nop 0\n\tglobal_load_lds_dwordx4 %1, off\n\ts_mov_b32 m0, %0"
               : "=&s"(keep)
               : "v"(addr), "s"(lds_dst)
               : "memory");
}
__device__ __attribute__((aligned(16))) float g_zero16[4];

template <int BM, int BN, int WM, int WN, bool MASK = false>
__global__ __launch_bounds__(GM_T, (BM == 64 ? 3 : 2)) void k_gemm_f32_deep(const float* __restrict__ A, const float* __restrict__ B, float* __restrict__ C,
                                                            int64_t M, int N, int K, GemmEpilogue ep, const uint16_t* __restrict__ amask,
                                                            int kshift) {
  static_assert(WM * WN == 4 && BM == 32 * WM && BN == 32 * WN, "one 32x32 accumulator per wavefront");
  constexpr int LA = BM / 32, LB = BN / 32, LPW = LA + LB;
  constexpr int STAGE_A = BM * 128, STAGE = (BM + BN) * 128;
  constexpr int NS = 3;
  __shared__ __attribute__((aligned(1024))) char lds[NS * STAGE];
  const int lane = threadIdx.x & 63, w = __builtin_amdgcn_readfirstlane(threadIdx.x >> 6);
  const int wm = w / WN, wn = w % WN;
  const int ntn = (N + BN - 1) / BN;
  const int xcd = blockIdx.x & 7, slot = blockIdx.x >> 3;
  const int64_t m_tile = static_cast<int64_t>(slot / ntn) * 8 + xcd;
  const int64_t m0 = m_tile * BM;
  const int n0 = (slot % ntn) * BN;
  if (m0 >= M) return;
  const unsigned lds_base = static_cast<unsigned>(reinterpret_cast<uintptr_t>(lds));

  unsigned oa[LA], ob[LB];
  uint32_t rmask[MASK ? LA : 1];
#pragma unroll
  for (int j = 0; j < LA; ++j) {
    const int row = (w * LA + j) * 8 + (lane >> 3);
    const int c = (lane & 7) ^ ((row >> 1) & 7);
    int64_t gr = m0 + row;
    gr = gr < M ? gr : M - 1;
    oa[j] = static_cast<unsigned>((gr * K + c * 4) * 4);
    if constexpr (MASK) rmask[j] = amask[gr];
  }
#pragma unroll
  for (int j = 0; j < LB; ++j) {
    const int row = (w * LB + j) * 8 + (lane >> 3);
    const int c = (lane & 7) ^ ((row >> 1) & 7);
    int gr = n0 + row;
    gr = gr < N ? gr : N - 1;
    ob[j] = static_cast<unsigned>((static_cast<int64_t>(gr) * K + c * 4) * 4);
  }
  const unsigned dst_a = lds_base + w * LA * 1024, dst_b = lds_base + STAGE_A + w * LB * 1024;
  const float* Ak = A;
  const float* Bk = B;
  int kt = 0;
  auto issue_one = [&](int stage, int j) {
    if (j < LA) {
      if constexpr (MASK) {
        const float* src = ((rmask[j] >> (kt >> kshift)) & 1u)
                               ? reinterpret_cast<const float*>(reinterpret_cast<const char*>(A) + (oa[j] + static_cast<unsigned>(kt * GM_BK * 4)))
                               : g_zero16;
        glds16_v(src, dst_a + stage * STAGE + j * 1024);
      } else {
        glds16(Ak, oa[j], dst_a + stage * STAGE + j * 1024);
      }
    } else {
      glds16(Bk, ob[j - LA], dst_b + stage * STAGE + (j - LA) * 1024);
    }
  };
  auto advance = [&] {
    Ak += GM_BK;
    Bk += GM_BK;
    if constexpr (MASK) ++kt;
  };
  auto issue = [&](int stage) {
#pragma unroll
    for (int j = 0; j < LPW; ++j) issue_one(stage, j);
    advance();
  };

  const int half = lane >> 5;
  const int ra = wm * 32 + (lane & 31), rb = wn * 32 + (lane & 31);
  int offa[4], offb[4];
#pragma unroll
  for (int q = 0; q < 4; ++q) {
    offa[q] = ra * 128 + (((4 * half + q) ^ ((ra >> 1) & 7)) << 4);
    offb[q] = STAGE_A + rb * 128 + (((4 * half + q) ^ ((rb >> 1) & 7)) << 4);
  }
  float4 fa[4], fb[4];
  floatx16 acc;
#pragma unroll
  for (int r = 0; r < 16; ++r) acc[r] = 0.f;
  const int nk = K / GM_BK;

  issue(0);
  if (nk > 1) issue(1);
  if (nk > 2) issue(2);
  float bias_v[1];
  {
    const int col = n0 + wn * 32 + (lane & 31);
    bias_v[0] = (ep.bias && col < N) ? ep.bias[col] : 0.f;
  }
  int blk_first = 0;
  int64_t blk_seg_start = 0, blk_seg_end = 0;
  if (ep.stats != nullptr) {
    blk_seg_end = ep.seg_len[0];
    while (blk_first + 1 < ep.S && m0 >= blk_seg_end) {
      ++blk_first;
      blk_seg_start = blk_seg_end;
      blk_seg_end += ep.seg_len[blk_first];
    }
  }
  if (nk > 2) wait_vmcnt<2 * LPW>();
  else if (nk > 1) wait_vmcnt<LPW>();
  else wait_vmcnt<0>();
  __syncthreads();
#pragma unroll
  for (int q = 0; q < 4; ++q) {
    fa[q] = *reinterpret_cast<const float4*>(lds + offa[q]);
    fb[q] = *reinterpret_cast<const float4*>(lds + offb[q]);
  }

  auto mfma = [&](float a, float b) { acc = __builtin_amdgcn_mfma_f32_32x32x2f32(a, b, acc, 0, 0, 0); };
  auto mfma4 = [&](const float4& a, const float4& b) {
    mfma(a.x, b.x);
    mfma(a.y, b.y);
    mfma(a.z, b.z);
    mfma(a.w, b.w);
  };
  auto pin = [] { __builtin_amdgcn_sched_barrier(0); };
  auto step = [&](auto st_c, auto full_c, int t) {
    constexpr int ST = decltype(st_c)::value;
    constexpr bool FULL = decltype(full_c)::value;
    constexpr int NXT = (ST + 1) % NS;
    float4 na[4], nb[4];
    mfma4(fa[0], fb[0]);
    const bool more = FULL || t + 1 < nk;
    const bool load = FULL || t + 3 < nk;
    pin();
    if (more) {
      if (FULL || t + 2 < nk) wait_vmcnt<LPW>();
      else wait_vmcnt<0>();
      __syncthreads();
    }
    const float a1[4] = {fa[1].x, fa[1].y, fa[1].z, fa[1].w}, b1[4] = {fb[1].x, fb[1].y, fb[1].z, fb[1].w};
    const float a2[4] = {fa[2].x, fa[2].y, fa[2].z, fa[2].w}, b2[4] = {fb[2].x, fb[2].y, fb[2].z, fb[2].w};
#pragma unroll
    for (int q = 0; q < 4; ++q) {
      if (more) {
        na[q] = *reinterpret_cast<const float4*>(lds + NXT * STAGE + offa[q]);
        nb[q] = *reinterpret_cast<const float4*>(lds + NXT * STAGE + offb[q]);
      }
      pin();
      mfma(a1[q], b1[q]);
      pin();
    }
#pragma unroll
    for (int q = 0; q < 4; ++q) {
      if (more && load) {
#pragma unroll
        for (int j = q; j < LPW; j += 4) issue_one(ST, j);
      }
      pin();
      mfma(a2[q], b2[q]);
      pin();
    }
    if (more && load) advance();
    mfma4(fa[3], fb[3]);
    if (more) {
#pragma unroll
      for (int q = 0; q < 4; ++q) fa[q] = na[q], fb[q] = nb[q];
    }
  };
  using I0 = std::integral_constant<int, 0>;
  using I1 = std::integral_constant<int, 1>;
  using I2 = std::integral_constant<int, 2>;
  int t = 0;
  for (; t + 6 <= nk; t += 3) {
    step(I0{}, std::true_type{}, t);
    step(I1{}, std::true_type{}, t + 1);
    step(I2{}, std::true_type{}, t + 2);
  }
  for (; t < nk; t += 3) {
    step(I0{}, std::false_type{}, t);
    if (t + 1 < nk) step(I1{}, std::false_type{}, t + 1);
    if (t + 2 < nk) step(I2{}, std::false_type{}, t + 2);
  }

  floatx16 accs[1] = {acc};
  gemm_epilogue<BM, BN, WM, WN, 1>(accs, C, M, N, m0, n0, m_tile, ep, bias_v, blk_first, blk_seg_start, blk_seg_end, wm, wn, lane);
}

template <int BM, int BN, int WM, int WN>
static int launch_gemm_deep(const float* A, const float* B, float* C, int64_t M, int N, int K, const GemmEpilogue& ep, hipStream_t st,
                            const uint16_t* amask = nullptr, int kshift = 0) {
  const int mt8 = (div_up(M, BM) + 7) / 8 * 8;
  if (amask)
    LCR_LAUNCH_TIMED((k_gemm_f32_deep<BM, BN, WM, WN, true>), dim3(mt8 * div_up(N, BN)), dim3(GM_T), 0, st, A, B, C, M, N, K, ep, amask, kshift);
  else
    LCR_LAUNCH_TIMED((k_gemm_f32_deep<BM, BN, WM, WN>), dim3(mt8 * div_up(N, BN)), dim3(GM_T), 0, st, A, B, C, M, N, K, ep, amask, kshift);
  return check_launch("lcr_gemm_f32");
}

typedef __bf16 bf16x8_t __attribute__((ext_vector_type(8)));
typedef __bf16 bf16x2_t __attribute__((ext_vector_type(2)));
typedef float f32x2_t __attribute__((ext_vector_type(2)));
typedef float f32x4_t __attribute__((ext_vector_type(4)));
typedef uint32_t u32x4_t __attribute__((ext_vector_type(4)));

__device__ __forceinline__ uint32_t pk_bf16(float a, float b) {
  f32x2_t v = {a, b};
  return __builtin_bit_cast(uint32_t, __builtin_convertvector(v, bf16x2_t));
}
__device__ __forceinline__ void split2(float x0, float x1, uint32_t& h1, uint32_t& h2, uint32_t& h3) {
  h1 = pk_bf16(x0, x1);
  const float r0 = fsub(x0, __uint_as_float(h1 << 16)), r1 = fsub(x1, __uint_as_float(h1 & 0xffff0000u));
  h2 = pk_bf16(r0, r1);
  const float s0 = fsub(r0, __uint_as_float(h2 << 16)), s1 = fsub(r1, __uint_as_float(h2 & 0xffff0000u));
  h3 = pk_bf16(s0, s1);
}

__global__ __launch_bounds__(256) void k_split_bf16x3(const float* __restrict__ w, int64_t n, uint16_t* __restrict__ planes) {
  for (int64_t i = (blockIdx.x * static_cast<int64_t>(blockDim.x) + threadIdx.x) * 2; i < n; i += static_cast<int64_t>(gridDim.x) * blockDim.x * 2) {
    const float x0 = w[i], x1 = i + 1 < n ? w[i + 1] : 0.f;
    uint32_t h1, h2, h3;
    split2(x0, x1, h1, h2, h3);
    planes[i] = static_cast<uint16_t>(h1), planes[n + i] = static_cast<uint16_t>(h2), planes[2 * n + i] = static_cast<uint16_t>(h3);
    if (i + 1 < n) planes[i + 1] = static_cast<uint16_t>(h1 >> 16), planes[n + i + 1] = static_cast<uint16_t>(h2 >> 16), planes[2 * n + i + 1] = static_cast<uint16_t>(h3 >> 16);
  }
}

__global__ __launch_bounds__(256) void k_split_bf16x3_tiles(const float* __restrict__ w, int N, int K, uint16_t* __restrict__ tiles) {
  const int KS = K / GM_BK;
  const int64_t blk = blockIdx.x;
  const int ct = static_cast<int>(blk / KS), ks = static_cast<int>(blk % KS);
  const int row = threadIdx.x >> 2, kc = threadIdx.x & 3;
  const int n = ct * 64 + row;
  u32x4_t p1 = {0u, 0u, 0u, 0u}, p2 = p1, p3 = p1;
  if (n < N) {
    const float* src = w + static_cast<int64_t>(n) * K + ks * GM_BK + kc * 8;
    const float4 x0 = ld4(src), x1 = ld4(src + 4);
    uint32_t h1, h2, h3;
    split2(x0.x, x0.y, h1, h2, h3), p1.x = h1, p2.x = h2, p3.x = h3;
    split2(x0.z, x0.w, h1, h2, h3), p1.y = h1, p2.y = h2, p3.y = h3;
    split2(x1.x, x1.y, h1, h2, h3), p1.z = h1, p2.z = h2, p3.z = h3;
    split2(x1.z, x1.w, h1, h2, h3), p1.w = h1, p2.w = h2, p3.w = h3;
  }
  char* dst = reinterpret_cast<char*>(tiles) + blk * 12288 + row * 64 + ((kc ^ ((row >> 2) & 3)) << 4);
  *reinterpret_cast<u32x4_t*>(dst) = p1;
  *reinterpret_cast<u32x4_t*>(dst + 4096) = p2;
  *reinterpret_cast<u32x4_t*>(dst + 8192) = p3;
}

template <int ABL, int NWM, int D = 2, bool MASK = false>
__global__ __launch_bounds__(128 * NWM, 2) void k_gemm_f32_bsplit_p(const float* __restrict__ A, const uint16_t* __restrict__ Bs, float* __restrict__ C,
                                                             int64_t M, int N, int K, GemmEpilogue ep, const uint16_t* __restrict__ amask,
                                                             int kshift) {
  constexpr int BM = 32 * NWM, BN = 64, RS = 64, T = 128 * NWM, PLA = BM * RS, STGA = 3 * PLA, PL = 64 * RS;
  constexpr int NPB = (768 + T - 1) / T;
  constexpr int STG = 3 * PL + (NPB * T - 768) * 16;
  __shared__ __attribute__((aligned(16))) char sA[2 * STGA];
  __shared__ __attribute__((aligned(16))) char sB[2 * STG];
  const int lane = threadIdx.x & 63, w = __builtin_amdgcn_readfirstlane(threadIdx.x >> 6);
  const int wm = w >> 1, wn = w & 1;
  const int ntn = (N + BN - 1) / BN;
  const int xcd = blockIdx.x & 7, slot = blockIdx.x >> 3;
  const int64_t m_tile = static_cast<int64_t>(slot / ntn) * 8 + xcd;
  const int64_t m0 = m_tile * BM;
  const int n0 = (slot % ntn) * BN;
  if (m0 >= M) return;
  const int srow = threadIdx.x >> 3, spc = threadIdx.x & 7;
  const float* ap[2];
  int soff[2];
  uint32_t aoff[2], rmask[2];
#pragma unroll
  for (int j = 0; j < 2; ++j) {
    const int r = srow + j * (T / 8);
    int64_t ga = m0 + r;
    ga = ga < M ? ga : M - 1;
    ap[j] = A + ga * K + spc * 4;
    if constexpr (MASK) {
      aoff[j] = static_cast<uint32_t>((ga * K + spc * 4) * 4);
      rmask[j] = amask[ga];
    } else {
      aoff[j] = rmask[j] = 0;
    }
    soff[j] = r * RS + (((spc >> 1) ^ ((r >> 2) & 3)) << 4) + (spc & 1) * 8;
  }
  const char* bp = reinterpret_cast<const char*>(Bs) + static_cast<int64_t>(n0 / 64) * (K / GM_BK) * 12288;
  int bsrc[NPB], bdst[NPB];
#pragma unroll
  for (int j = 0; j < NPB; ++j) {
    const int q = threadIdx.x + T * j;
    bsrc[j] = (q < 768 ? q : threadIdx.x) * 16;
    bdst[j] = q * 16;
  }
  const int fsw = ((lane & 31) >> 2) & 3, fc0 = ((lane >> 5) ^ fsw) << 4, fc1 = (((lane >> 5) + 2) ^ fsw) << 4;
  const int fa = (wm * 32 + (lane & 31)) * RS, fb = (wn * 32 + (lane & 31)) * RS;
  floatx16 acc, acc2;
#pragma unroll
  for (int r = 0; r < 16; ++r) acc[r] = 0.f, acc2[r] = 0.f;
  const int nk = K / GM_BK;
  f32x4_t ra[D][2];
  u32x4_t rb[D][NPB];
  __amdgpu_buffer_rsrc_t arsrc;
  if constexpr (MASK) arsrc = __builtin_amdgcn_make_buffer_rsrc(const_cast<float*>(A), 0, static_cast<int>(M * K * 4), 0x00020000);
  auto fetch = [&](auto st_c, int t) {
    constexpr int st = decltype(st_c)::value;
    const int tt = t < nk ? t : nk - 1;
    if constexpr (MASK) {
      const int kb = tt >> kshift;
#pragma unroll
      for (int j = 0; j < 2; ++j) {
        const uint32_t o = ((rmask[j] >> kb) & 1u) ? aoff[j] + static_cast<uint32_t>(tt * GM_BK * 4) : 0x80000000u;
        ra[st][j] = __builtin_bit_cast(f32x4_t, __builtin_amdgcn_raw_buffer_load_b128(arsrc, static_cast<int>(o), 0, 0));
      }
    } else {
      ra[st][0] = *reinterpret_cast<const f32x4_t*>(ap[0] + tt * GM_BK), ra[st][1] = *reinterpret_cast<const f32x4_t*>(ap[1] + tt * GM_BK);
    }
#pragma unroll
    for (int j = 0; j < NPB; ++j) rb[st][j] = *reinterpret_cast<const u32x4_t*>(bp + static_cast<int64_t>(tt) * 12288 + bsrc[j]);
  };
  auto park = [&](auto st_c, int lds_stage) {
    constexpr int st = decltype(st_c)::value;
    char* da = sA + lds_stage * STGA;
    char* db = sB + lds_stage * STG;
#pragma unroll
    for (int j = 0; j < 2; ++j) {
      uint32_t h1, h2, h3, g1, g2, g3;
      if constexpr (ABL & 2) {
        h1 = __float_as_uint(ra[st][j].x), h2 = __float_as_uint(ra[st][j].y), h3 = h1, g1 = __float_as_uint(ra[st][j].z), g2 = __float_as_uint(ra[st][j].w), g3 = g1;
      } else {
        split2(ra[st][j].x, ra[st][j].y, h1, h2, h3);
        split2(ra[st][j].z, ra[st][j].w, g1, g2, g3);
      }
      if constexpr (ABL & 4) {
        asm volatile("" ::"v"(h1), "v"(h2), "v"(h3), "v"(g1), "v"(g2), "v"(g3));
      } else {
        *reinterpret_cast<uint2*>(da + soff[j]) = make_uint2(h1, g1);
        *reinterpret_cast<uint2*>(da + PLA + soff[j]) = make_uint2(h2, g2);
        *reinterpret_cast<uint2*>(da + 2 * PLA + soff[j]) = make_uint2(h3, g3);
      }
    }
#pragma unroll
    for (int j = 0; j < NPB; ++j) {
      const u32x4_t v = rb[st][j];
      if constexpr (ABL & 4) {
        asm volatile("" ::"v"(v));
      } else {
        *reinterpret_cast<u32x4_t*>(db + bdst[j]) = v;
      }
    }
  };
  using I0 = std::integral_constant<int, 0>;
  fetch(I0{}, 0);
  if constexpr (D > 1) fetch(std::integral_constant<int, 1 % D>{}, 1);
  if constexpr (D > 2) fetch(std::integral_constant<int, 2 % D>{}, 2);
  if constexpr (D > 3) fetch(std::integral_constant<int, 3 % D>{}, 3);
  float bias_v[1];
  {
    const int col = n0 + wn * 32 + (lane & 31);
    bias_v[0] = (ep.bias && col < N) ? ep.bias[col] : 0.f;
  }
  int blk_first = 0;
  int64_t blk_seg_start = 0, blk_seg_end = 0;
  if (ep.stats != nullptr) {
    blk_seg_end = ep.seg_len[0];
    while (blk_first + 1 < ep.S && m0 >= blk_seg_end) {
      ++blk_first;
      blk_seg_start = blk_seg_end;
      blk_seg_end += ep.seg_len[blk_first];
    }
  }
  park(I0{}, 0);
  fetch(I0{}, D);
  __syncthreads();
  auto step = [&](auto lds_c, auto reg_c, int t) {
    constexpr int P = decltype(lds_c)::value;
    using NX = std::integral_constant<int, (decltype(reg_c)::value + 1) % D>;
    const char* la = sA + P * STGA + fa;
    const char* lb = sB + P * STG + fb;
    bf16x8_t a0[3], b0[3], a1[3], b1[3];
    auto mm = [&](const bf16x8_t& x, const bf16x8_t& y, floatx16& c) {
      if constexpr (ABL & 1) {
        asm volatile("" ::"v"(x), "v"(y));
      } else {
        c = __builtin_amdgcn_mfma_f32_32x32x16_bf16(x, y, c, 0, 0, 0);
      }
    };
    if constexpr (ABL & 16) {
      u32x4_t z = {static_cast<uint32_t>(t), 0u, 0u, 0u};
      asm volatile("" : "+v"(z));
#pragma unroll
      for (int p = 0; p < 3; ++p) a0[p] = b0[p] = a1[p] = b1[p] = __builtin_bit_cast(bf16x8_t, z);
      (void)la, (void)lb;
    } else {
#pragma unroll
      for (int p = 0; p < 3; ++p) {
        a0[p] = __builtin_bit_cast(bf16x8_t, *reinterpret_cast<const u32x4_t*>(la + p * PLA + fc0));
        b0[p] = __builtin_bit_cast(bf16x8_t, *reinterpret_cast<const u32x4_t*>(lb + p * PL + fc0));
      }
#pragma unroll
      for (int p = 0; p < 3; ++p) {
        a1[p] = __builtin_bit_cast(bf16x8_t, *reinterpret_cast<const u32x4_t*>(la + p * PLA + fc1));
        b1[p] = __builtin_bit_cast(bf16x8_t, *reinterpret_cast<const u32x4_t*>(lb + p * PL + fc1));
      }
    }
    mm(a0[2], b0[0], acc);
    mm(a0[0], b0[2], acc2);
    mm(a0[1], b0[1], acc);
    mm(a0[1], b0[0], acc2);
    mm(a0[0], b0[1], acc);
    mm(a0[0], b0[0], acc2);
    park(NX{}, P ^ 1);
    mm(a1[2], b1[0], acc);
    mm(a1[0], b1[2], acc2);
    mm(a1[1], b1[1], acc);
    mm(a1[1], b1[0], acc2);
    mm(a1[0], b1[1], acc);
    mm(a1[0], b1[0], acc2);
    if constexpr (!(ABL & 8)) fetch(NX{}, t + 1 + D);
    __syncthreads();
  };
  static_assert(D == 2 || D == 4, "register stages");
  using I1 = std::integral_constant<int, 1>;
  using I2 = std::integral_constant<int, 2>;
  using I3 = std::integral_constant<int, 3>;
  int t = 0;
  if constexpr (D == 2) {
    for (; t + 2 <= nk; t += 2) {
      step(I0{}, I0{}, t);
      step(I1{}, I1{}, t + 1);
    }
    if (t < nk) step(I0{}, I0{}, t);
  } else {
    for (; t + 4 <= nk; t += 4) {
      step(I0{}, I0{}, t);
      step(I1{}, I1{}, t + 1);
      step(I0{}, I2{}, t + 2);
      step(I1{}, I3{}, t + 3);
    }
    if (t < nk) step(I0{}, I0{}, t);
    if (t + 1 < nk) step(I1{}, I1{}, t + 1);
    if (t + 2 < nk) step(I0{}, I2{}, t + 2);
  }
#pragma unroll
  for (int r = 0; r < 16; ++r) acc[r] += acc2[r];
  floatx16 accs[1] = {acc};
  gemm_epilogue<BM, BN, NWM, 2, 1>(accs, C, M, N, m0, n0, m_tile, ep, bias_v, blk_first, blk_seg_start, blk_seg_end, wm, wn, lane);
}

struct GemmStreamK {
  float*    partial;
  uint32_t* arrived;
  int       U;
};

template <int BM, int BN, int WM, int WN>
__global__ __launch_bounds__(GM_T, 3) void k_gemm_f32_sk(const float* __restrict__ A, const float* __restrict__ B, float* __restrict__ C,
                                                         int64_t M, int N, int K, GemmEpilogue ep, GemmStreamK sk) {
  static_assert(WM * WN == 4 && BM == 32 * WM, "one 32-row MFMA tile per wavefront along M");
  constexpr int LDA = BM + 1, LDB = BN + 4;
  constexpr int NT = BN / (32 * WN);
  __shared__ __attribute__((aligned(16))) float As[2][GM_BK * LDA];
  __shared__ __attribute__((aligned(16))) float Bs[2][GM_BK * LDB];
  const int lane = threadIdx.x & 63, w = __builtin_amdgcn_readfirstlane(threadIdx.x >> 6);
  const int wm = w / WN, wn = w % WN;
  const int ntn = (N + BN - 1) / BN;
  const int64_t mt = (M + BM - 1) / BM;
  const int xcd = blockIdx.x & 7, u = blockIdx.x >> 3;
  const int64_t mt_x = mt > xcd ? (mt - xcd + 7) / 8 : 0;
  const int nk = (K + GM_BK - 1) / GM_BK;
  const int64_t I = mt_x * ntn * nk;
  auto first_it = [&](int uu) { return static_cast<int64_t>(uu) * I / sk.U; };
  const int64_t it_begin = first_it(u), it_end = first_it(u + 1);
  LoaderT<BM, LDA, true> la[2];
  LoaderN<BN, LDB, true> lb[2];
  const int a_off = (lane >> 5) * LDA + wm * 32 + (lane & 31);
  const int b_off = (lane >> 5) * LDB + wn * (32 * NT) + (lane & 31);
  constexpr int PIECE = NT * 16 * GM_T;
  __shared__ unsigned s_arrived;

  int64_t it = it_begin;
  while (it < it_end) {
    const int64_t lt = it / nk;
    const int ks = static_cast<int>(it - lt * nk);
    const int ns = static_cast<int>(min(static_cast<int64_t>(nk - ks), it_end - it));
    const int64_t m_tile = (lt / ntn) * 8 + xcd;
    const int64_t m0 = m_tile * BM;
    const int n0 = static_cast<int>(lt % ntn) * BN;
    const int k_begin = ks * GM_BK;
    auto gload = [&](int k0, int r) {
      la[r].load(A, M, K, m0, k0);
      lb[r].load(B, N, K, n0, k0);
    };
    floatx16 acc[NT];
#pragma unroll
    for (int j = 0; j < NT; ++j)
#pragma unroll
      for (int r = 0; r < 16; ++r) acc[j][r] = 0.f;
    gload(k_begin, 0);
    gload(k_begin + GM_BK, 1);
    const bool covers_end = ks + ns == nk, covers_start = ks == 0;
    float bias_v[NT];
#pragma unroll
    for (int j = 0; j < NT; ++j) {
      const int col = n0 + wn * (32 * NT) + j * 32 + (lane & 31);
      bias_v[j] = (ep.bias && col < N) ? ep.bias[col] : 0.f;
    }
    int blk_first = 0;
    int64_t blk_seg_start = 0, blk_seg_end = 0;
    la[0].store(As[0]);
    lb[0].store(Bs[0]);
    __syncthreads();

    constexpr int KK = GM_BK / 2;
    constexpr int PF = NT == 1 ? KK : (NT == 2 ? 8 : 4);
    constexpr int PA = BM * 8 / GM_T, PB = BN * 8 / GM_T;
    constexpr int ST0 = KK - (PA + PB) - 1 > 2 ? (KK - (PA + PB)) / 2 : 1;
    auto step = [&](auto buf_c, auto full_c, int t) {
      constexpr int BUF = decltype(buf_c)::value;
      constexpr bool FULL = decltype(full_c)::value;
      if (FULL || t + 2 < ns) gload(k_begin + (t + 2) * GM_BK, BUF);
      const bool do_store = FULL || t + 1 < ns;
      const float* as = As[BUF] + a_off;
      const float* bs = Bs[BUF] + b_off;
      float af[PF], bf[PF][NT];
#pragma unroll
      for (int d = 0; d < PF; ++d) {
        af[d] = as[d * 2 * LDA];
#pragma unroll
        for (int j = 0; j < NT; ++j) bf[d][j] = bs[d * 2 * LDB + j * 32];
      }
      __builtin_amdgcn_sched_barrier(0);
#pragma unroll
      for (int kk = 0; kk < KK; ++kk) {
        const int sl = kk % PF;
#pragma unroll
        for (int j = 0; j < NT; ++j) acc[j] = __builtin_amdgcn_mfma_f32_32x32x2f32(af[sl], bf[sl][j], acc[j], 0, 0, 0);
        if (kk + PF < KK) {
          af[sl] = as[(kk + PF) * 2 * LDA];
#pragma unroll
          for (int j = 0; j < NT; ++j) bf[sl][j] = bs[(kk + PF) * 2 * LDB + j * 32];
        }
        const int piece = kk - ST0;
        if (do_store && piece >= 0 && piece < PA + PB) {
          if (piece < PA) la[1 - BUF].store_piece(As[1 - BUF], piece);
          else lb[1 - BUF].store_piece(Bs[1 - BUF], piece - PA);
        }
      }
      __syncthreads();
    };
    int t = 0;
    for (; t + 3 < ns; t += 2) {
      step(std::integral_constant<int, 0>{}, std::true_type{}, t);
      step(std::integral_constant<int, 1>{}, std::true_type{}, t + 1);
    }
    for (; t < ns; t += 2) {
      step(std::integral_constant<int, 0>{}, std::false_type{}, t);
      if (t + 1 >= ns) break;
      step(std::integral_constant<int, 1>{}, std::false_type{}, t + 1);
    }

    bool finish = true;
    if (!(covers_start && covers_end)) {
      float* mine = sk.partial + (static_cast<int64_t>(blockIdx.x) * 2 + (it == it_begin ? 0 : 1)) * PIECE;
#pragma unroll
      for (int j = 0; j < NT; ++j)
#pragma unroll
        for (int r = 0; r < 16; ++r)
          __hip_atomic_store(&mine[(j * 16 + r) * GM_T + threadIdx.x], acc[j][r], __ATOMIC_RELAXED, __HIP_MEMORY_SCOPE_AGENT);
      const int64_t tile_it0 = lt * nk, tile_it1 = tile_it0 + nk;
      int uf = static_cast<int>(tile_it0 * sk.U / I);
      while (uf > 0 && first_it(uf) > tile_it0) --uf;
      while (first_it(uf + 1) <= tile_it0) ++uf;
      int ul = uf, pieces = 0;
      for (int uu = uf; uu < sk.U && first_it(uu) < tile_it1; ++uu)
        if (first_it(uu + 1) > first_it(uu)) {
          ul = uu;
          ++pieces;
        }
      __builtin_amdgcn_s_waitcnt(0);
      __builtin_amdgcn_fence(__ATOMIC_RELEASE, "workgroup");
      __syncthreads();
      uint32_t* cnt = sk.arrived + (m_tile * ntn + lt % ntn);
      if (threadIdx.x == 0) s_arrived = __hip_atomic_fetch_add(cnt, 1u, __ATOMIC_RELAXED, __HIP_MEMORY_SCOPE_AGENT);
      __syncthreads();
      finish = s_arrived == static_cast<unsigned>(pieces - 1);
      if (finish) {
        __builtin_amdgcn_fence(__ATOMIC_ACQUIRE, "workgroup");
#pragma unroll
        for (int j = 0; j < NT; ++j)
#pragma unroll
          for (int r = 0; r < 16; ++r) acc[j][r] = 0.f;
        for (int uu = uf; uu <= ul; ++uu) {
          if (first_it(uu + 1) <= first_it(uu)) continue;
          const float* pp = sk.partial + (static_cast<int64_t>(uu * 8 + xcd) * 2 + (first_it(uu) >= tile_it0 ? 0 : 1)) * PIECE;
#pragma unroll
          for (int j = 0; j < NT; ++j)
#pragma unroll
            for (int r = 0; r < 16; ++r)
              acc[j][r] += __hip_atomic_load(&pp[(j * 16 + r) * GM_T + threadIdx.x], __ATOMIC_RELAXED, __HIP_MEMORY_SCOPE_AGENT);
        }
        if (threadIdx.x == 0) __hip_atomic_store(cnt, 0u, __ATOMIC_RELAXED, __HIP_MEMORY_SCOPE_AGENT);
      }
    }
    if (finish) {
      if (ep.stats != nullptr) {
        blk_first = 0;
        blk_seg_start = 0;
        blk_seg_end = ep.seg_len[0];
        while (blk_first + 1 < ep.S && m0 >= blk_seg_end) {
          ++blk_first;
          blk_seg_start = blk_seg_end;
          blk_seg_end += ep.seg_len[blk_first];
        }
      }
      gemm_epilogue<BM, BN, WM, WN, NT>(acc, C, M, N, m0, n0, m_tile, ep, bias_v, blk_first, blk_seg_start, blk_seg_end, wm, wn, lane);
    }
    it += ns;
    __syncthreads();
  }
}

template <int BM, int BN, int WM, int WN, bool VEC, bool SHORT = false>
static int launch_gemm(const float* A, const float* B, float* C, int64_t M, int N, int K, int transA, int transB, const GemmEpilogue& ep,
                       hipStream_t st, const GemmBatch* batch = nullptr) {
  static const GemmBatch no_batch = {};
  const GemmBatch& bt = batch ? *batch : no_batch;
  const int mt8 = (div_up(M, BM) + 7) / 8 * 8;
  dim3 grid(mt8 * div_up(N, BN), 1, bt.count ? bt.count : 1);
  dim3 block(GM_T);
  if (!transA && !transB) LCR_LAUNCH_TIMED((k_gemm_f32<BM, BN, WM, WN, false, false, VEC, SHORT>), grid, block, 0, st, A, B, C, M, N, K, ep, bt, ANorm{});
  else if (!transA && transB) LCR_LAUNCH_TIMED((k_gemm_f32<BM, BN, WM, WN, false, true, VEC, SHORT>), grid, block, 0, st, A, B, C, M, N, K, ep, bt, ANorm{});
  else if (transA && !transB) LCR_LAUNCH_TIMED((k_gemm_f32<BM, BN, WM, WN, true, false, VEC, SHORT>), grid, block, 0, st, A, B, C, M, N, K, ep, bt, ANorm{});
  else LCR_LAUNCH_TIMED((k_gemm_f32<BM, BN, WM, WN, true, true, VEC, SHORT>), grid, block, 0, st, A, B, C, M, N, K, ep, bt, ANorm{});
  return check_launch("lcr_gemm_f32");
}

struct SkScratch {
  float*    partial = nullptr;
  uint32_t* arrived = nullptr;
};
static std::mutex g_sk_mu;
static std::map<std::pair<int, hipStream_t>, SkScratch> g_sk_scratch;
constexpr int SK_MAX_GRID = 1024;
constexpr int SK_MAX_TILES = 8192;

static int sk_cu_count() {
  static const int n = [] {
    int dev = 0, cus = 0;
    hipGetDevice(&dev);
    if (hipDeviceGetAttribute(&cus, hipDeviceAttributeMultiprocessorCount, dev) != hipSuccess || cus <= 0) cus = 256;
    return cus;
  }();
  return n;
}

static bool sk_worth(int64_t M, int N, int K) {
  const int cus = sk_cu_count();
  const int64_t tiles = static_cast<int64_t>(div_up(M, 64)) * div_up(N, 64);
  if (K < 480 || tiles < cus / 2 || tiles > 6 * static_cast<int64_t>(cus) || tiles > SK_MAX_TILES) return false;
  const double avg = static_cast<double>(tiles) / cus;
  const double worst = static_cast<double>((tiles + cus - 1) / cus);
  return worst / avg >= 1.10;
}

static int launch_gemm_sk(const float* A, const float* B, float* C, int64_t M, int N, int K, const GemmEpilogue& ep, hipStream_t st) {
  const int cus = sk_cu_count();
  const int64_t iters = static_cast<int64_t>(div_up(M, 64)) * div_up(N, 64) * div_up(K, GM_BK);
  int per_cu = 3;
  while (per_cu > 1 && iters / (static_cast<int64_t>(cus) * per_cu) < 24) --per_cu;
  if (getenv("LCR_SK_PER_CU")) per_cu = atoi(getenv("LCR_SK_PER_CU"));
  int U = cus * per_cu / 8;
  if (U < 1) U = 1;
  if (8 * U > SK_MAX_GRID) U = SK_MAX_GRID / 8;
  int dev = 0;
  hipGetDevice(&dev);
  GemmStreamK sk;
  {
    std::lock_guard<std::mutex> lk(g_sk_mu);
    SkScratch& sc = g_sk_scratch[{dev, st}];
    if (!sc.partial) {
      if (hipMalloc(reinterpret_cast<void**>(&sc.partial), sizeof(float) * 2 * 16 * GM_T * SK_MAX_GRID) != hipSuccess ||
          hipMalloc(reinterpret_cast<void**>(&sc.arrived), sizeof(uint32_t) * SK_MAX_TILES) != hipSuccess) {
        set_error("lcr_gemm_f32: cannot allocate the stream-K scratch");
        return LCR_EHIP;
      }
      hipMemsetAsync(sc.arrived, 0, sizeof(uint32_t) * SK_MAX_TILES, st);
    }
    sk.partial = sc.partial;
    sk.arrived = sc.arrived;
    sk.U = U;
  }
  LCR_LAUNCH_TIMED((k_gemm_f32_sk<64, 64, 2, 2>), dim3(8 * U), dim3(GM_T), 0, st, A, B, C, M, N, K, ep, sk);
  return check_launch("lcr_gemm_f32");
}

}

using namespace lcr;

static int g_force_tile = 0;
extern "C" void lcr_gemm_debug_force_tile(int t) { g_force_tile = t; }
static int g_force_streamk = -1;
static int g_force_deep = -1;
extern "C" void lcr_gemm_debug_deep(int mode) { g_force_deep = mode; }
extern "C" void lcr_gemm_debug_streamk(int mode) { g_force_streamk = mode; }

static int gemm_impl(const float* A, const float* B, float* C, int64_t M, int N, int K, int transA, int transB, const float* bias,
                     const float* rowdiv, const int64_t* seg_len, int S, int groups, double* stats, void* stream);

static int env_int(const char* name, int unset) { return getenv(name) ? atoi(getenv(name)) : unset; }
enum GemmForm { GF_SCALAR, GF_FORCED_TILE, GF_SHORT, GF_DEEP, GF_STREAMK, GF_TILE };
static GemmForm gemm_form(int64_t M, int N, int K, int transA, int transB, bool vec) {
  static const bool no_short = getenv("LCR_GEMM_NO_SHORT") != nullptr;
  static const int short_k = env_int("LCR_GEMM_SHORT_K", 256);
  static const int deep_env = env_int("LCR_GEMM_DEEP", 1);
  static const int sk_env = env_int("LCR_GEMM_STREAMK", 0);
  if (!vec) return GF_SCALAR;
  if (g_force_tile >= 1 && g_force_tile <= 5) return GF_FORCED_TILE;
  const int deep_mode = g_force_deep >= 0 ? g_force_deep : deep_env;
  const bool deep_ok = !transA && transB && K % GM_BK == 0 && !g_force_tile && M * K < (int64_t(1) << 30) && static_cast<int64_t>(N) * K < (int64_t(1) << 30);
  if (deep_mode == 2 && deep_ok) return GF_DEEP;
  if (!no_short && K <= short_k && !transA) return GF_SHORT;
  if (deep_mode && deep_ok) return GF_DEEP;
  if (N <= 32) return GF_TILE;
  const int sk_mode = g_force_streamk >= 0 ? g_force_streamk : sk_env;
  const bool sk_legal = !transA && !transB && K >= 64 && static_cast<int64_t>(div_up(M, 64)) * div_up(N, 64) <= SK_MAX_TILES;
  if (sk_mode && sk_legal && (sk_mode == 2 || sk_worth(M, N, K))) return GF_STREAMK;
  return GF_TILE;
}

extern "C" int lcr_gemm_f32_anorm(const float* A, const float* B, float* C, int64_t M, int N, int K, const float* bias,
                                  const double* a_stats, const float* a_gamma, const float* a_beta, int a_groups, float a_eps,
                                  float a_slope, const int64_t* seg_len, int S, int groups, double* stats, void* stream) {
  if (!A || !B || !C || M < 0 || N <= 32 || K <= 0 || K > AN_KMAX || K % 4 != 0 || !a_stats || !a_gamma || !a_beta || a_groups < 1 ||
      K % a_groups != 0 || a_groups > 64 || !seg_len || S < 1 || reinterpret_cast<uintptr_t>(A) % 16 != 0 || reinterpret_cast<uintptr_t>(B) % 16 != 0) {
    set_error("lcr_gemm_f32_anorm: needs 32 < N, K <= 256, K % 4 == 0, a_groups dividing K, a segment table and 16-byte aligned operands");
    return LCR_EARG;
  }
  if (stats) {
    const int gs = groups >= 1 && N % groups == 0 ? N / groups : 3;
    if ((gs & (gs - 1)) != 0) {
      set_error("lcr_gemm_f32_anorm: statistics need groups dividing N into power-of-two sized groups");
      return LCR_EARG;
    }
  }
  hipStream_t st = static_cast<hipStream_t>(stream);
  KernelTimerScope timed(KT_GEMM, st, M, N, K);
  if (M == 0) return LCR_OK;
  GemmEpilogue ep{bias, nullptr, seg_len, S, groups, stats};
  ANorm an{a_stats, a_gamma, a_beta, a_groups, a_eps, a_slope};
  const int mt8 = (div_up(M, 64) + 7) / 8 * 8;
  LCR_LAUNCH_TIMED((k_gemm_f32<64, 64, 2, 2, false, true, true, true, true>), dim3(mt8 * div_up(N, 64)), dim3(GM_T), 0, st, A, B, C, M,
                     N, K, ep, GemmBatch{}, an);
  return check_launch("lcr_gemm_f32_anorm");
}

extern "C" int lcr_gemm_f32(const float* A, const float* B, float* C, int64_t M, int N, int K, int transA, int transB, const float* bias,
                            const float* rowdiv, const int64_t* seg_len, int S, int groups, double* stats, void* stream) {
  return gemm_impl(A, B, C, M, N, K, transA, transB, bias, rowdiv, seg_len, S, groups, stats, stream);
}

static int gemm_impl(const float* A, const float* B, float* C, int64_t M, int N, int K, int transA, int transB, const float* bias,
                     const float* rowdiv, const int64_t* seg_len, int S, int groups, double* stats, void* stream) {
  if (!A || !B || !C || M < 0 || N <= 0 || K <= 0) {
    set_error("lcr_gemm_f32: bad argument");
    return LCR_EARG;
  }
  if (stats && (!seg_len || S < 1 || groups < 1 || N % groups != 0)) {
    set_error("lcr_gemm_f32: statistics need seg_len, S >= 1 and groups dividing N");
    return LCR_EARG;
  }
  if (stats) {
    const int gs = N / groups;
    if ((gs & (gs - 1)) != 0) {
      set_error("lcr_gemm_f32: channels per group must be a power of two");
      return LCR_EARG;
    }
  }
  hipStream_t st = static_cast<hipStream_t>(stream);
  KernelTimerScope timed(KT_GEMM, st, M, N, K);
  if (M == 0) return LCR_OK;
  GemmEpilogue ep{bias, rowdiv, seg_len, S, groups, stats};
  const int64_t lda = transA ? M : K, ldb = transB ? K : N;
  const bool vec = (lda % 4 == 0) && (ldb % 4 == 0) && (reinterpret_cast<uintptr_t>(A) % 16 == 0) && (reinterpret_cast<uintptr_t>(B) % 16 == 0);
  switch (gemm_form(M, N, K, transA, transB, vec)) {
    case GF_SCALAR: return launch_gemm<128, 64, 4, 1, false>(A, B, C, M, N, K, transA, transB, ep, st);
    case GF_FORCED_TILE:
      switch (g_force_tile) {
        case 1: return launch_gemm<128, 128, 4, 1, true>(A, B, C, M, N, K, transA, transB, ep, st);
        case 2: return launch_gemm<128, 64, 4, 1, true>(A, B, C, M, N, K, transA, transB, ep, st);
        case 3: return launch_gemm<128, 32, 4, 1, true>(A, B, C, M, N, K, transA, transB, ep, st);
        case 4: return launch_gemm<64, 64, 2, 2, true>(A, B, C, M, N, K, transA, transB, ep, st);
        default: return launch_gemm<64, 128, 2, 2, true>(A, B, C, M, N, K, transA, transB, ep, st);
      }
    case GF_SHORT:
      if (N <= 32) return launch_gemm<128, 32, 4, 1, true, true>(A, B, C, M, N, K, transA, transB, ep, st);
      return launch_gemm<64, 64, 2, 2, true, true>(A, B, C, M, N, K, transA, transB, ep, st);
    case GF_DEEP:
      if (N <= 32) return launch_gemm_deep<128, 32, 4, 1>(A, B, C, M, N, K, ep, st);
      return launch_gemm_deep<64, 64, 2, 2>(A, B, C, M, N, K, ep, st);
    case GF_STREAMK: return launch_gemm_sk(A, B, C, M, N, K, ep, st);
    case GF_TILE: break;
  }
  if (N <= 32) return launch_gemm<128, 32, 4, 1, true>(A, B, C, M, N, K, transA, transB, ep, st);
  const int64_t b128 = (M + 127) / 128, nb128 = (N + 127) / 128;
  if (K >= 512 && b128 * nb128 >= 512) return launch_gemm<128, 128, 4, 1, true>(A, B, C, M, N, K, transA, transB, ep, st);
  return launch_gemm<64, 64, 2, 2, true>(A, B, C, M, N, K, transA, transB, ep, st);
}

extern "C" int lcr_split_bf16x3(const float* w, int64_t n, uint16_t* planes, void* stream) {
  if (!w || !planes || n < 0) {
    set_error("lcr_split_bf16x3: bad argument");
    return LCR_EARG;
  }
  if (n == 0) return LCR_OK;
  hipLaunchKernelGGL(k_split_bf16x3, dim3(min(div_up(n, 512), 2048)), dim3(256), 0, static_cast<hipStream_t>(stream), w, n, planes);
  return check_launch("lcr_split_bf16x3");
}

extern "C" int lcr_split_bf16x3_tiles(const float* w, int N, int K, uint16_t* tiles, void* stream) {
  if (!w || !tiles || N < 1 || K < GM_BK || K % GM_BK != 0 || reinterpret_cast<uintptr_t>(w) % 16 != 0 || reinterpret_cast<uintptr_t>(tiles) % 16 != 0) {
    set_error("lcr_split_bf16x3_tiles: needs K %% 32 == 0 and 16-byte aligned buffers");
    return LCR_EARG;
  }
  hipLaunchKernelGGL(k_split_bf16x3_tiles, dim3(div_up(N, 64) * (K / GM_BK)), dim3(256), 0, static_cast<hipStream_t>(stream), w, N, K, tiles);
  return check_launch("lcr_split_bf16x3_tiles");
}

static int bsplit_impl(const float* A, const uint16_t* Bs, float* C, int64_t M, int N, int K, const float* bias, const float* rowdiv,
                       const int64_t* seg_len, int S, int groups, double* stats, const uint16_t* amask, int kshift, void* stream) {
  if (!A || !Bs || !C || M < 0 || N <= 0 || K <= 0 || K % GM_BK != 0 || reinterpret_cast<uintptr_t>(A) % 16 != 0 || reinterpret_cast<uintptr_t>(Bs) % 16 != 0 ||
      K < GM_BK) {
    set_error("lcr_gemm_f32_bsplit: needs K %% 32 == 0 and 16-byte aligned operands");
    return LCR_EARG;
  }
  if (stats && (!seg_len || S < 1 || groups < 1 || N % groups != 0 || ((N / groups) & (N / groups - 1)) != 0)) {
    set_error("lcr_gemm_f32_bsplit: statistics need seg_len, S >= 1 and groups dividing N into power-of-two sized groups");
    return LCR_EARG;
  }
  hipStream_t st = static_cast<hipStream_t>(stream);
  KernelTimerScope timed(KT_GEMM, st, M, N, K);
  if (M == 0) return LCR_OK;
  GemmEpilogue ep{bias, rowdiv, seg_len, S, groups, stats};
  const int mt8 = (div_up(M, 64) + 7) / 8 * 8;
  static const int abl = getenv("LCR_SPLIT_ABL") ? atoi(getenv("LCR_SPLIT_ABL")) : 0;
  const dim3 grid(mt8 * div_up(N, 64)), block(256);
  if (amask) {
    LCR_LAUNCH_TIMED((k_gemm_f32_bsplit_p<0, 2, 2, true>), grid, block, 0, st, A, Bs, C, M, N, K, ep, amask, kshift);
    return check_launch("lcr_gemm_f32_bsplit_masked");
  }
  switch (abl) {
    case 1: LCR_LAUNCH_TIMED((k_gemm_f32_bsplit_p<1, 2>), grid, block, 0, st, A, Bs, C, M, N, K, ep, amask, kshift); break;
    case 2: LCR_LAUNCH_TIMED((k_gemm_f32_bsplit_p<2, 2>), grid, block, 0, st, A, Bs, C, M, N, K, ep, amask, kshift); break;
    case 4: LCR_LAUNCH_TIMED((k_gemm_f32_bsplit_p<4, 2>), grid, block, 0, st, A, Bs, C, M, N, K, ep, amask, kshift); break;
    case 8: LCR_LAUNCH_TIMED((k_gemm_f32_bsplit_p<8, 2>), grid, block, 0, st, A, Bs, C, M, N, K, ep, amask, kshift); break;
    case 16: LCR_LAUNCH_TIMED((k_gemm_f32_bsplit_p<16, 2>), grid, block, 0, st, A, Bs, C, M, N, K, ep, amask, kshift); break;
    case 23: LCR_LAUNCH_TIMED((k_gemm_f32_bsplit_p<23, 2>), grid, block, 0, st, A, Bs, C, M, N, K, ep, amask, kshift); break;
    case 30: LCR_LAUNCH_TIMED((k_gemm_f32_bsplit_p<30, 2>), grid, block, 0, st, A, Bs, C, M, N, K, ep, amask, kshift); break;
    default: LCR_LAUNCH_TIMED((k_gemm_f32_bsplit_p<0, 2>), grid, block, 0, st, A, Bs, C, M, N, K, ep, amask, kshift); break;
  }
  return check_launch("lcr_gemm_f32_bsplit");
}

extern "C" int lcr_gemm_f32_bsplit(const float* A, const uint16_t* Bs, float* C, int64_t M, int N, int K, const float* bias, const float* rowdiv,
                                   const int64_t* seg_len, int S, int groups, double* stats, void* stream) {
  return bsplit_impl(A, Bs, C, M, N, K, bias, rowdiv, seg_len, S, groups, stats, nullptr, 0, stream);
}

static int mask_kshift(int K, int block_k) {
  for (int s = 0; s <= 3; ++s)
    if (block_k == (GM_BK << s)) return K <= 16 * block_k ? s : -1;
  return -1;
}

extern "C" int lcr_gemm_f32_bsplit_masked(const float* A, const uint16_t* Bs, float* C, int64_t M, int N, int K, const float* bias,
                                          const float* rowdiv, const int64_t* seg_len, int S, int groups, double* stats, const uint16_t* row_mask,
                                          int block_k, void* stream) {
  const int ks = mask_kshift(K, block_k);
  if (!row_mask || ks < 0 || M * static_cast<int64_t>(K) >= (int64_t(1) << 29)) {
    set_error("lcr_gemm_f32_bsplit_masked: needs a row mask, block_k = 32 << s (s <= 3) with K <= 16 block_k, and M*K < 2^29");
    return LCR_EARG;
  }
  return bsplit_impl(A, Bs, C, M, N, K, bias, rowdiv, seg_len, S, groups, stats, row_mask, ks, stream);
}

extern "C" int lcr_kpconv_mask_ok(int64_t M, int N, int K, int split) {
  static const bool off = getenv("LCR_KP_MASK") && atoi(getenv("LCR_KP_MASK")) == 0;
  if (off || M <= 0 || N <= 0 || K % 15 != 0 || mask_kshift(K, K / 15) < 0) return 0;
  if (split) return M * static_cast<int64_t>(K) < (int64_t(1) << 29);
  return gemm_form(M, N, K, 0, 1, true) == GF_DEEP;
}

extern "C" int lcr_gemm_f32_masked(const float* A, const float* B, float* C, int64_t M, int N, int K, const float* bias, const float* rowdiv,
                                   const int64_t* seg_len, int S, int groups, double* stats, const uint16_t* row_mask, int block_k, void* stream) {
  const int ks = mask_kshift(K, block_k);
  if (!A || !B || !C || !row_mask || M < 0 || N <= 0 || K <= 0 || K % GM_BK != 0 || ks < 0 || M * static_cast<int64_t>(K) >= (int64_t(1) << 30) ||
      static_cast<int64_t>(N) * K >= (int64_t(1) << 30) || reinterpret_cast<uintptr_t>(A) % 16 != 0 || reinterpret_cast<uintptr_t>(B) % 16 != 0) {
    set_error("lcr_gemm_f32_masked: needs a row mask, block_k = 32 << s (s <= 3) with K <= 16 block_k, K %% 32 == 0, M*K and N*K < 2^30, "
              "16-byte aligned operands");
    return LCR_EARG;
  }
  if (stats && (!seg_len || S < 1 || groups < 1 || N % groups != 0 || ((N / groups) & (N / groups - 1)) != 0)) {
    set_error("lcr_gemm_f32_masked: statistics need seg_len, S >= 1 and groups dividing N into power-of-two sized groups");
    return LCR_EARG;
  }
  hipStream_t st = static_cast<hipStream_t>(stream);
  KernelTimerScope timed(KT_GEMM, st, M, N, K);
  if (M == 0) return LCR_OK;
  GemmEpilogue ep{bias, rowdiv, seg_len, S, groups, stats};
  if (N <= 32) return launch_gemm_deep<128, 32, 4, 1>(A, B, C, M, N, K, ep, st, row_mask, ks);
  return launch_gemm_deep<64, 64, 2, 2>(A, B, C, M, N, K, ep, st, row_mask, ks);
}

extern "C" int lcr_gemm_f32_batched_ta(const float* A, const float* B, float* C, int64_t M, int N, int count, const int* k_host,
                                       const int64_t* a_off_host, const int64_t* b_off_host, const int64_t* c_off_host, void* stream) {
  if (!A || !B || !C || M <= 0 || N <= 0 || count < 1 || count > GM_MAX_BATCH || !k_host || !a_off_host || !b_off_host || !c_off_host) {
    set_error("lcr_gemm_f32_batched_ta: bad argument (count <= %d)", GM_MAX_BATCH);
    return LCR_EARG;
  }
  GemmBatch bt = {};
  bt.count = count;
  for (int i = 0; i < count; ++i) {
    bt.k[i] = k_host[i];
    bt.a_off[i] = a_off_host[i];
    bt.b_off[i] = b_off_host[i];
    bt.c_off[i] = c_off_host[i];
    if (a_off_host[i] % 4 || b_off_host[i] % 4 || k_host[i] < 1) {
      set_error("lcr_gemm_f32_batched_ta: offsets must be multiples of 4 floats and K >= 1");
      return LCR_EARG;
    }
  }
  if ((M % 4) || (N % 4)) {
    set_error("lcr_gemm_f32_batched_ta: M and N must be multiples of 4");
    return LCR_EARG;
  }
  GemmEpilogue ep{nullptr, nullptr, nullptr, 0, 0, nullptr};
  return launch_gemm<64, 64, 2, 2, true>(A, B, C, M, N,  1, 1, 0, ep, static_cast<hipStream_t>(stream), &bt);
}

extern "C" int lcr_gemm_f32_strided_batched(const float* A, const float* B, float* C, int64_t M, int N, int K, int transA, int transB,
                                            int64_t strideA, int64_t strideB, int64_t strideC, int count, void* stream) {
  if (!A || !B || !C || M <= 0 || N <= 0 || K <= 0 || count < 1 || count > 65535 || (strideA % 4) || (strideB % 4)) {
    set_error("lcr_gemm_f32_strided_batched: bad argument");
    return LCR_EARG;
  }
  const int64_t lda = transA ? M : K, ldb = transB ? K : N;
  if ((lda % 4) || (ldb % 4)) {
    set_error("lcr_gemm_f32_strided_batched: leading dimensions must be multiples of 4");
    return LCR_EARG;
  }
  GemmBatch bt = {};
  bt.count = count;
  bt.strided = 1;
  bt.k[0] = K;
  bt.a_off[0] = strideA;
  bt.b_off[0] = strideB;
  bt.c_off[0] = strideC;
  GemmEpilogue ep{nullptr, nullptr, nullptr, 0, 0, nullptr};
  static const int batch_tile = env_int("LCR_GEMM_BATCH_TILE", 64);
  if (batch_tile == 128 && M >= 128 && N >= 128) return launch_gemm<128, 128, 4, 1, true>(A, B, C, M, N, K, transA, transB, ep, static_cast<hipStream_t>(stream), &bt);
  static const bool batch_short = env_int("LCR_GEMM_BATCH_SHORT", 1) != 0;
  if (batch_short && K <= 256 && !transA) return launch_gemm<64, 64, 2, 2, true, true>(A, B, C, M, N, K, transA, transB, ep, static_cast<hipStream_t>(stream), &bt);
  return launch_gemm<64, 64, 2, 2, true>(A, B, C, M, N, K, transA, transB, ep, static_cast<hipStream_t>(stream), &bt);
}
```

### lcr-net_amd/functional.py

```python
import ctypes
import os
import threading

import numpy as np
import torch

from . import _lib

GN_EPS = 1e-5
GN_REPLICAS = 8


class KernelTimer:
    KINDS = {"gemm": 0, "kpconv_aggregate": 1, "radius_query": 2, "attention": 3, "kpconv_fused": 4, "sinkhorn": 5}

    def __init__(self, names):
        self.names = set(names)
        self._cache = None

    def summary(self):
        return {k: [(b, m) for b, _, m in v] for k, v in self.records().items()}

    def records(self):
        if self._cache is None:
            out = {}
            L = _lib.lib()
            for name in self.names:
                kind = self.KINDS[name]
                n = L.lcr_ktimer_read2(kind, 0, None, None, None)
                sec = (ctypes.c_double * max(n, 1))()
                ksec = (ctypes.c_double * max(n, 1))()
                meta = (ctypes.c_int64 * (5 * max(n, 1)))()
                L.lcr_ktimer_read2(kind, n, ctypes.cast(sec, ctypes.c_void_p), ctypes.cast(ksec, ctypes.c_void_p), ctypes.cast(meta, ctypes.c_void_p))
                width = 3 if name == "gemm" else 5
                out[name] = [(sec[i], ksec[i] if ksec[i] >= 0 else None, tuple(int(meta[5 * i + k]) for k in range(width))) for i in range(n)]
            self._cache = out
        return self._cache


def set_timer(timer, sample_every=1):
    _lib.lib().lcr_ktimer_sample(int(sample_every))
    mask = 0
    for name in (timer.names if timer is not None else ()):
        mask |= 1 << KernelTimer.KINDS[name]
    _lib.lib().lcr_ktimer_kinds(mask if timer is not None else 0xffffffff)
    _lib.lib().lcr_ktimer_enable(1 if timer is not None else 0)


def _timed(name, fn, meta=None):
    return fn()


def _seg(seg_len, n, device):
    if seg_len is None:
        return torch.full((1,), int(n), dtype=torch.int64, device=device)
    return seg_len


def host_values(values, dtype, device):
    return torch.tensor(values, dtype=dtype).pin_memory().to(device, non_blocking=True)


def host_tensor(t, device):
    if not torch.is_tensor(t):
        t = torch.from_numpy(t)
    return t.pin_memory().to(device, non_blocking=True)


def _idx_args(idx):
    if idx.dtype == torch.int64:
        return 1
    if idx.dtype == torch.int32:
        return 0
    raise RuntimeError("neighbor indices must be int32 or int64")


class _StatsArena(threading.local):
    buf = None
    off = 0


_ARENA = _StatsArena()


class stats_arena:

    def __init__(self, device, entries=1 << 18):
        self.device, self.entries = device, entries

    def __enter__(self):
        self.prev = (_ARENA.buf, _ARENA.off)
        _ARENA.buf = torch.zeros(self.entries, dtype=torch.float64, device=self.device)
        _ARENA.off = 0
        return self

    def __exit__(self, *exc):
        _ARENA.buf, _ARENA.off = self.prev
        return False


def _zero_stats(S, groups, device):
    n = GN_REPLICAS * S * groups * 2
    buf = _ARENA.buf
    if buf is not None and buf.device == device and _ARENA.off + n <= buf.numel():
        v = buf[_ARENA.off:_ARENA.off + n].view(GN_REPLICAS, S, groups, 2)
        _ARENA.off += n
        return v
    return torch.zeros((GN_REPLICAS, S, groups, 2), dtype=torch.float64, device=device)


def gemm(a, b, trans_b=False, trans_a=False, bias=None, rowdiv=None, seg_len=None, groups=0, row_mask=None):
    if row_mask is not None:
        return _gemm_masked(a, b, trans_b, trans_a, bias, rowdiv, seg_len, groups, row_mask)
    _lib.require_cuda(a, b)
    assert a.dtype == torch.float32 and b.dtype == torch.float32 and a.is_contiguous() and b.is_contiguous()
    M, K = (a.shape[1], a.shape[0]) if trans_a else (a.shape[0], a.shape[1])
    N = b.shape[0] if trans_b else b.shape[1]
    assert (b.shape[1] if trans_b else b.shape[0]) == K, "inner dimensions differ"
    c = torch.empty((M, N), dtype=torch.float32, device=a.device)
    stats = None
    S = 0
    if groups:
        seg_len = _seg(seg_len, M, a.device)
        S = seg_len.numel()
        stats = _zero_stats(S, groups, a.device)
    _timed("gemm", lambda: _lib.check(_lib.lib().lcr_gemm_f32(
        _lib.ptr(a), _lib.ptr(b), _lib.ptr(c), M, N, K, int(trans_a), int(trans_b), _lib.ptr(bias), _lib.ptr(rowdiv),
        _lib.ptr(seg_len) if groups else None, S, int(groups), _lib.ptr(stats), _lib.stream_ptr(a.device)), "lcr_gemm_f32"),
        meta=(M, N, K))
    return c, stats


def kpconv_mask_ok(M, N, K, split):
    return bool(_lib.lib().lcr_kpconv_mask_ok(int(M), int(N), int(K), int(bool(split))))


def _mask_args(a, row_mask):
    M, K = a.shape
    assert row_mask.dtype == torch.int16 and row_mask.is_contiguous() and row_mask.numel() == M and row_mask.device == a.device
    assert K % 15 == 0
    return K // 15


def _gemm_masked(a, b, trans_b, trans_a, bias, rowdiv, seg_len, groups, row_mask):
    _lib.require_cuda(a, b)
    assert trans_b and not trans_a, "the masked form takes A [M,K] and B [N,K]"
    assert a.dtype == torch.float32 and b.dtype == torch.float32 and a.is_contiguous() and b.is_contiguous()
    block_k = _mask_args(a, row_mask)
    M, K = a.shape
    N = b.shape[0]
    assert b.shape[1] == K, "inner dimensions differ"
    c = torch.empty((M, N), dtype=torch.float32, device=a.device)
    stats, S = None, 0
    if groups:
        seg_len = _seg(seg_len, M, a.device)
        S = seg_len.numel()
        stats = _zero_stats(S, groups, a.device)
    _timed("gemm", lambda: _lib.check(_lib.lib().lcr_gemm_f32_masked(
        _lib.ptr(a), _lib.ptr(b), _lib.ptr(c), M, N, K, _lib.ptr(bias), _lib.ptr(rowdiv), _lib.ptr(seg_len) if groups else None, S,
        int(groups), _lib.ptr(stats), _lib.ptr(row_mask), block_k, _lib.stream_ptr(a.device)), "lcr_gemm_f32_masked"), meta=(M, N, K))
    return c, stats


_GEMM_SPLIT = [os.environ.get("LCR_GEMM_SPLIT", "1") not in ("", "0")]


def gemm_split_enabled():
    return _GEMM_SPLIT[0]


def set_gemm_split(on):
    _GEMM_SPLIT[0] = bool(on)


def gemm_split_ok(N, K):
    return K >= 288 and K % 32 == 0 and N >= 64


derived_lock = threading.RLock()


class WeightStamp:
    __slots__ = ("ref", "ptr", "ver", "dev")

    def __init__(self, t):
        import weakref
        self.ref, self.ptr, self.ver, self.dev = weakref.ref(t), t.data_ptr(), t._version, t.device

    def same(self, t):
        return self.ref is not None and self.ref() is t and self.ptr == t.data_ptr() and self.ver == t._version and self.dev == t.device

    def __reduce__(self):
        return (_dead_stamp, ())


def _dead_stamp():
    s = WeightStamp.__new__(WeightStamp)
    s.ref, s.ptr, s.ver, s.dev = None, 0, -1, None
    return s


def drop_derived(module, *names):
    for n in names:
        if n in module.__dict__:
            module.__dict__[n] = None



def publish_derived(t):
    torch.cuda.current_stream(t.device).synchronize()
    return t


def split_bf16x3(w):
    w = w.detach().contiguous()
    N, K = w.shape
    assert K % 32 == 0
    tiles = torch.empty(((N + 63) // 64, K // 32, 3, 64, 32), dtype=torch.int16, device=w.device)
    _lib.check(_lib.lib().lcr_split_bf16x3_tiles(_lib.ptr(w), int(N), int(K), _lib.ptr(tiles), _lib.stream_ptr(w.device)), "lcr_split_bf16x3_tiles")
    tiles.lcr_n = int(N)
    return tiles


def unsplit_bf16x3(tiles):
    CT, KS = tiles.shape[0], tiles.shape[1]
    t = tiles.view(CT, KS, 3, 64, 4, 8)
    row = torch.arange(64, device=tiles.device)
    phys = torch.arange(4, device=tiles.device)[None, :] ^ ((row >> 2) & 3)[:, None]
    t = torch.gather(t, 4, phys.view(1, 1, 1, 64, 4, 1).expand(CT, KS, 3, 64, 4, 8))
    t = t.reshape(CT, KS, 3, 64, 32).permute(2, 0, 3, 1, 4).reshape(3, CT * 64, KS * 32)
    return t[:, :tiles.lcr_n].contiguous().view(torch.bfloat16).float()


def gemm_bsplit(a, planes, bias=None, rowdiv=None, seg_len=None, groups=0, row_mask=None):
    _lib.require_cuda(a, planes)
    assert a.dtype == torch.float32 and a.is_contiguous() and planes.dtype == torch.int16 and planes.is_contiguous() and planes.dim() == 5
    M, K = a.shape
    N = planes.lcr_n
    assert planes.shape[1] * 32 == K and planes.shape[0] == (N + 63) // 64, "inner dimensions differ"
    c = torch.empty((M, N), dtype=torch.float32, device=a.device)
    stats, S = None, 0
    if groups:
        seg_len = _seg(seg_len, M, a.device)
        S = seg_len.numel()
        stats = _zero_stats(S, groups, a.device)
    if row_mask is not None:
        block_k = _mask_args(a, row_mask)
        _lib.check(_lib.lib().lcr_gemm_f32_bsplit_masked(_lib.ptr(a), _lib.ptr(planes), _lib.ptr(c), M, N, K, _lib.ptr(bias), _lib.ptr(rowdiv),
                                                         _lib.ptr(seg_len) if groups else None, S, int(groups), _lib.ptr(stats),
                                                         _lib.ptr(row_mask), block_k, _lib.stream_ptr(a.device)), "lcr_gemm_f32_bsplit_masked")
        return c, stats
    _lib.check(_lib.lib().lcr_gemm_f32_bsplit(_lib.ptr(a), _lib.ptr(planes), _lib.ptr(c), M, N, K, _lib.ptr(bias), _lib.ptr(rowdiv),
                                              _lib.ptr(seg_len) if groups else None, S, int(groups), _lib.ptr(stats), _lib.stream_ptr(a.device)),
               "lcr_gemm_f32_bsplit")
    return c, stats


ANORM_MAX_K, ANORM_MIN_SEG_ROWS = 256, 64


def gemm_anorm_ok(K, N):
    return K <= ANORM_MAX_K and K % 4 == 0 and N > 32


def gemm_anorm(a, a_stats, a_gamma, a_beta, a_groups, weight, bias=None, seg_len=None, groups=0, slope=0.1):
    _lib.require_cuda(a, weight)
    assert a.dtype == torch.float32 and weight.dtype == torch.float32 and a.is_contiguous() and weight.is_contiguous()
    M, K = a.shape
    N = weight.shape[0]
    assert weight.shape[1] == K and gemm_anorm_ok(K, N)
    c = torch.empty((M, N), dtype=torch.float32, device=a.device)
    seg_len = _seg(seg_len, M, a.device)
    S = seg_len.numel()
    stats = _zero_stats(S, groups, a.device) if groups else None
    _timed("gemm", lambda: _lib.check(_lib.lib().lcr_gemm_f32_anorm(
        _lib.ptr(a), _lib.ptr(weight), _lib.ptr(c), M, N, K, _lib.ptr(bias), _lib.ptr(a_stats), _lib.ptr(a_gamma), _lib.ptr(a_beta),
        int(a_groups), GN_EPS, float(slope), _lib.ptr(seg_len), S, int(groups), _lib.ptr(stats), _lib.stream_ptr(a.device)),
        "lcr_gemm_f32_anorm"), meta=(M, N, K))
    return c, stats


def groupnorm_stats(x, groups, seg_len=None):
    seg_len = _seg(seg_len, x.shape[0], x.device)
    stats = _zero_stats(seg_len.numel(), groups, x.device)
    _lib.check(_lib.lib().lcr_groupnorm_stats(_lib.ptr(x), x.shape[0], x.shape[1], groups, _lib.ptr(seg_len), seg_len.numel(),
                                              _lib.ptr(stats), _lib.stream_ptr(x.device)), "lcr_groupnorm_stats")
    return stats


def groupnorm_apply(x, stats, gamma, beta, groups, seg_len=None, res=None, res_norm=None, slope=0.1, act=True, want_pos=False):
    seg_len = _seg(seg_len, x.shape[0], x.device)
    y = torch.empty_like(x)
    pos = torch.empty((x.shape[0],), dtype=torch.uint8, device=x.device) if want_pos else None
    rs, rg, rb = res_norm if res_norm is not None else (None, None, None)
    _lib.check(_lib.lib().lcr_groupnorm_apply(_lib.ptr(x), _lib.ptr(stats), _lib.ptr(gamma), _lib.ptr(beta), _lib.ptr(res), _lib.ptr(rs),
                                              _lib.ptr(rg), _lib.ptr(rb), _lib.ptr(y), x.shape[0], x.shape[1], groups, _lib.ptr(seg_len),
                                              seg_len.numel(), GN_EPS, float(slope), int(act), _lib.ptr(pos),
                                              _lib.stream_ptr(x.device)), "lcr_groupnorm_apply")
    return (y, pos) if want_pos else y


def row_positive(x):
    pos = torch.empty((x.shape[0],), dtype=torch.uint8, device=x.device)
    _lib.check(_lib.lib().lcr_row_positive(_lib.ptr(x), x.shape[0], x.shape[1], _lib.ptr(pos), _lib.stream_ptr(x.device)), "lcr_row_positive")
    return pos


def _kp_host(kernel_points):
    kp = np.ascontiguousarray(kernel_points, dtype=np.float32)
    assert kp.shape == (15, 3)
    return kp


def kpconv_aggregate(s_feats, s_pos, q_points, s_points, idx, kernel_points_host, sigma, order=None, emit_mask=False):
    _lib.require_cuda(s_feats, q_points, s_points, idx)
    M, H = idx.shape
    Ns, C = s_feats.shape
    assert idx.is_contiguous() and s_feats.is_contiguous() and q_points.is_contiguous() and s_points.is_contiguous()
    A = torch.empty((M, 15 * C), dtype=torch.float32, device=s_feats.device)
    nn = torch.empty((M,), dtype=torch.float32, device=s_feats.device)
    kp = _kp_host(kernel_points_host)
    if emit_mask:
        mask = torch.empty((M,), dtype=torch.int16, device=s_feats.device)
        _timed("kpconv_aggregate", lambda: _lib.check(_lib.lib().lcr_kpconv_aggregate_mask(
            _lib.ptr(s_feats), _lib.ptr(s_pos), _lib.ptr(q_points), _lib.ptr(s_points), _lib.ptr(idx), _idx_args(idx), M, Ns, H, C,
            ctypes.c_void_p(kp.ctypes.data), float(sigma), _lib.ptr(A), _lib.ptr(nn), _lib.ptr(mask), _lib.ptr(order), 0,
            _lib.stream_ptr(s_feats.device)), "lcr_kpconv_aggregate_mask"), meta=(M, Ns, H, C, idx.element_size()))
        return A, nn, mask
    _timed("kpconv_aggregate", lambda: _lib.check(_lib.lib().lcr_kpconv_aggregate(
        _lib.ptr(s_feats), _lib.ptr(s_pos), _lib.ptr(q_points), _lib.ptr(s_points), _lib.ptr(idx), _idx_args(idx), M, Ns, H, C,
        ctypes.c_void_p(kp.ctypes.data), float(sigma), _lib.ptr(A), _lib.ptr(nn), _lib.ptr(order), _lib.stream_ptr(s_feats.device)),
        "lcr_kpconv_aggregate"), meta=(M, Ns, H, C, idx.element_size()))
    return A, nn


KPCONV_FUSED_C = 32


def kpconv_fused(s_feats, s_pos, q_points, s_points, idx, kernel_points_host, sigma, weights, bias, seg_len=None, groups=0, order=None):
    _lib.require_cuda(s_feats, q_points, s_points, idx)
    M, H = idx.shape
    Ns, C = s_feats.shape
    assert C == KPCONV_FUSED_C and tuple(weights.shape) == (15, C, C) and weights.is_contiguous()
    assert idx.is_contiguous() and s_feats.is_contiguous() and q_points.is_contiguous() and s_points.is_contiguous()
    out = torch.empty((M, C), dtype=torch.float32, device=s_feats.device)
    stats, S = None, 0
    if groups:
        seg_len = _seg(seg_len, M, s_feats.device)
        S = seg_len.numel()
        stats = _zero_stats(S, groups, s_feats.device)
    kp = _kp_host(kernel_points_host)
    _timed("kpconv_fused", lambda: _lib.check(_lib.lib().lcr_kpconv_fused(
        _lib.ptr(s_feats), _lib.ptr(s_pos), _lib.ptr(q_points), _lib.ptr(s_points), _lib.ptr(idx), _idx_args(idx), M, Ns, H, C,
        ctypes.c_void_p(kp.ctypes.data), float(sigma), _lib.ptr(weights), _lib.ptr(bias), _lib.ptr(out),
        _lib.ptr(seg_len) if groups else None, S, int(groups), _lib.ptr(stats), _lib.ptr(order), _lib.stream_ptr(s_feats.device)),
        "lcr_kpconv_fused"), meta=(M, Ns, H, C, idx.element_size()))
    return out, stats


def kpconv_cin1(s_feats, q_points, s_points, idx, kernel_points_host, sigma, weights, bias, order=None):
    M, H = idx.shape
    Ns = s_feats.shape[0]
    Cout = weights.shape[-1]
    out = torch.empty((M, Cout), dtype=torch.float32, device=s_feats.device)
    kp = _kp_host(kernel_points_host)
    _lib.check(_lib.lib().lcr_kpconv_cin1(_lib.ptr(s_feats), _lib.ptr(q_points), _lib.ptr(s_points), _lib.ptr(idx), _idx_args(idx), M, Ns, H,
                                          ctypes.c_void_p(kp.ctypes.data), float(sigma), _lib.ptr(weights), _lib.ptr(bias), Cout,
                                          _lib.ptr(out), _lib.ptr(order), _lib.stream_ptr(s_feats.device)), "lcr_kpconv_cin1")
    return out


def maxpool(x, idx, order=None):
    M, H = idx.shape
    out = torch.empty((M, x.shape[1]), dtype=torch.float32, device=x.device)
    _lib.check(_lib.lib().lcr_maxpool(_lib.ptr(x), _lib.ptr(idx), _idx_args(idx), M, x.shape[0], H, x.shape[1], _lib.ptr(out),
                                      _lib.ptr(order), _lib.stream_ptr(x.device)), "lcr_maxpool")
    return out


class NetvladWeights(ctypes.Structure):
    _fields_ = [(n, ctypes.c_void_p) for n in (
        "cluster_weights", "cluster_weights2", "hidden1_weights", "bn1_w", "bn1_b", "bn1_mean", "bn1_var",
        "bn2_w", "bn2_b", "bn2_mean", "bn2_var", "gating_weights", "gbn_w", "gbn_b", "gbn_mean", "gbn_var")]


def netvlad_forward(feats, seg_len_host, weights_struct):
    _lib.require_cuda(feats)
    seg = np.ascontiguousarray(seg_len_host, dtype=np.int64)
    S = int(seg.shape[0])
    assert int(seg.sum()) == feats.shape[0] and feats.shape[1] == 1024 and feats.is_contiguous()
    nbytes = ctypes.c_size_t(0)
    _lib.check(_lib.lib().lcr_netvlad_ws_bytes(feats.shape[0], S, ctypes.byref(nbytes)), "lcr_netvlad_ws_bytes")
    ws = _lib.workspace(nbytes.value, feats.device)
    out = torch.empty((S, 256), dtype=torch.float32, device=feats.device)
    _lib.check(_lib.lib().lcr_netvlad_forward(_lib.ptr(feats), ctypes.c_void_p(seg.ctypes.data), S, ctypes.byref(weights_struct),
                                              _lib.ptr(out), _lib.ptr(ws), ws.numel(), _lib.stream_ptr(feats.device)),
               "lcr_netvlad_forward")
    return out


def gemm_batched_ta(a, b, c, M, N, k, a_off, b_off, c_off):
    _lib.require_cuda(a, b, c)
    assert all(t.dtype == torch.float32 and t.is_contiguous() for t in (a, b, c))
    kk = np.ascontiguousarray(k, dtype=np.int32)
    ao, bo, co = (np.ascontiguousarray(v, dtype=np.int64) for v in (a_off, b_off, c_off))
    count = int(kk.shape[0])
    assert ao.shape == bo.shape == co.shape == (count,)
    for i in range(count):
        assert 0 <= ao[i] and ao[i] + max(int(kk[i]), 0) * M <= a.numel(), "A entry out of range"
        assert 0 <= bo[i] and bo[i] + max(int(kk[i]), 0) * N <= b.numel(), "B entry out of range"
        assert 0 <= co[i] and co[i] + M * N <= c.numel(), "C entry out of range"
    _lib.check(_lib.lib().lcr_gemm_f32_batched_ta(_lib.ptr(a), _lib.ptr(b), _lib.ptr(c), int(M), int(N), count, ctypes.c_void_p(kk.ctypes.data),
                                                  ctypes.c_void_p(ao.ctypes.data), ctypes.c_void_p(bo.ctypes.data),
                                                  ctypes.c_void_p(co.ctypes.data), _lib.stream_ptr(a.device)), "lcr_gemm_f32_batched_ta")
    return c


def linear(x, weight, bias=None, relu=False):
    y = gemm(x.contiguous(), weight, trans_b=True, bias=bias)[0]
    if relu:
        _lib.check(_lib.lib().lcr_relu_inplace(_lib.ptr(y), y.numel(), _lib.stream_ptr(y.device)), "lcr_relu_inplace")
    return y


def relu_(x):
    _lib.check(_lib.lib().lcr_relu_inplace(_lib.ptr(x), x.numel(), _lib.stream_ptr(x.device)), "lcr_relu_inplace")
    return x


def rotary_embed_(x, theta, heads):
    assert x.is_contiguous() and theta.is_contiguous() and x.shape[1] == heads * 32 and theta.shape[1] == heads * 16
    _lib.check(_lib.lib().lcr_rotary_embed(_lib.ptr(x), _lib.ptr(theta), x.shape[0], heads, _lib.stream_ptr(x.device)), "lcr_rotary_embed")
    return x


def attention(q, k, v, heads, q_lens=None, k_lens=None):
    assert q.is_contiguous() and k.is_contiguous() and v.is_contiguous()
    out = torch.empty_like(q)
    if q_lens is not None:
        P = len(q_lens)
        assert len(k_lens) == P and sum(q_lens) == q.shape[0] and sum(k_lens) == k.shape[0]
        ql, kl = (ctypes.c_int64 * P)(*[int(x) for x in q_lens]), (ctypes.c_int64 * P)(*[int(x) for x in k_lens])
        _lib.check(_lib.lib().lcr_attention_seg_f32(_lib.ptr(q), _lib.ptr(k), _lib.ptr(v), ctypes.cast(ql, ctypes.c_void_p),
                                                    ctypes.cast(kl, ctypes.c_void_p), P, heads, q.shape[1] // heads, _lib.ptr(out),
                                                    _lib.stream_ptr(q.device)), "lcr_attention_seg_f32")
        return out
    _lib.check(_lib.lib().lcr_attention_f32(_lib.ptr(q), _lib.ptr(k), _lib.ptr(v), q.shape[0], k.shape[0], heads, q.shape[1] // heads,
                                            _lib.ptr(out), _lib.stream_ptr(q.device)), "lcr_attention_f32")
    return out


ATTENTION_TOPK_MAX_KEYS = 4096


def attention_topk(q, k, v, heads, q_lens, k_lens, kks):
    assert q.is_contiguous() and k.is_contiguous() and v.is_contiguous()
    P = len(q_lens)
    assert len(k_lens) == P and len(kks) == P and sum(q_lens) == q.shape[0] and sum(k_lens) == k.shape[0]
    out = torch.empty_like(q)
    ql, kl = (ctypes.c_int64 * P)(*[int(x) for x in q_lens]), (ctypes.c_int64 * P)(*[int(x) for x in k_lens])
    kk = (ctypes.c_int * P)(*[int(x) for x in kks])
    _lib.check(_lib.lib().lcr_attention_topk_f32(_lib.ptr(q), _lib.ptr(k), _lib.ptr(v), ctypes.cast(ql, ctypes.c_void_p), ctypes.cast(kl, ctypes.c_void_p),
                                                 ctypes.cast(kk, ctypes.c_void_p), P, heads, q.shape[1] // heads, _lib.ptr(out), _lib.stream_ptr(q.device)),
               "lcr_attention_topk_f32")
    return out


def add_layernorm(a, b, gamma, beta, eps=1e-5):
    y = torch.empty_like(a)
    _lib.check(_lib.lib().lcr_add_layernorm(_lib.ptr(a), _lib.ptr(b), _lib.ptr(gamma), _lib.ptr(beta), a.shape[0], a.shape[1], float(eps),
                                            _lib.ptr(y), _lib.stream_ptr(a.device)), "lcr_add_layernorm")
    return y


def _L():
    return _lib.lib()


def _sp(t):
    return _lib.stream_ptr(t.device)


def vote_shift(xyz, offsets, max_range):
    out = torch.empty_like(xyz)
    _lib.check(_L().lcr_vote_shift(_lib.ptr(xyz.contiguous()), _lib.ptr(offsets.contiguous()), xyz.shape[0], float(max_range), _lib.ptr(out),
                                   _sp(xyz)), "lcr_vote_shift")
    return out


def greedy_nms(points, lengths, radius):
    n, B = points.shape[0], lengths.numel()
    keep = torch.empty((n,), dtype=torch.uint8, device=points.device)
    out_len = torch.empty((B,), dtype=torch.int64, device=points.device)
    nbytes = ctypes.c_size_t(0)
    _lib.check(_L().lcr_greedy_nms_ws_bytes(n, ctypes.byref(nbytes)), "lcr_greedy_nms_ws_bytes")
    ws = _lib.workspace(nbytes.value, points.device)
    _lib.check(_L().lcr_greedy_nms(_lib.ptr(points.contiguous()), _lib.ptr(lengths), B, n, float(radius), _lib.ptr(keep), _lib.ptr(out_len),
                                   _lib.ptr(ws), _sp(points)), "lcr_greedy_nms")
    return keep, out_len


def neighbor_mean(points, idx, pad):
    out = torch.empty((idx.shape[0], 3), dtype=torch.float32, device=points.device)
    _lib.check(_L().lcr_neighbor_mean(_lib.ptr(points.contiguous()), _lib.ptr(idx.contiguous()), _idx_args(idx), idx.shape[0], idx.shape[1], int(pad),
                                      _lib.ptr(out), _sp(points)), "lcr_neighbor_mean")
    return out


def point_to_node_partition(points, nodes, point_limit):
    N, M, dev = points.shape[0], nodes.shape[0], points.device
    nbytes = ctypes.c_size_t(0)
    _lib.check(_L().lcr_point_to_node_ws_bytes(N, M, ctypes.byref(nbytes)), "lcr_point_to_node_ws_bytes")
    ws = _lib.workspace(nbytes.value, dev)
    p2n = torch.empty((N,), dtype=torch.int32, device=dev)
    knn = torch.empty((M, point_limit), dtype=torch.int64, device=dev)
    km = torch.empty((M, point_limit), dtype=torch.uint8, device=dev)
    nm = torch.empty((M,), dtype=torch.uint8, device=dev)
    status = torch.zeros(1, dtype=torch.int32, device=dev)
    _lib.check(_L().lcr_point_to_node_partition(_lib.ptr(points.contiguous()), N, _lib.ptr(nodes.contiguous()), M, int(point_limit), _lib.ptr(p2n),
                                                _lib.ptr(knn), _lib.ptr(km), _lib.ptr(nm), _lib.ptr(status), _lib.ptr(ws), ws.numel(), _sp(points)),
               "lcr_point_to_node_partition")
    return p2n, nm.bool(), knn, km.bool()


def point_to_node_partition_stack(points, point_off, nodes, node_off, point_limit):
    import numpy as np
    C = len(point_off) - 1
    assert len(node_off) == C + 1 and C >= 1
    dev = points.device
    N, M = int(point_off[-1] - point_off[0]), int(node_off[-1] - node_off[0])
    po = np.ascontiguousarray(point_off, dtype=np.int64)
    mo = np.ascontiguousarray(node_off, dtype=np.int64)
    nbytes = ctypes.c_size_t(0)
    _lib.check(_L().lcr_point_to_node_ws_bytes(N, M, ctypes.byref(nbytes)), "lcr_point_to_node_ws_bytes")
    ws = _lib.workspace(nbytes.value, dev)
    p2n = torch.empty((N,), dtype=torch.int32, device=dev)
    knn = torch.empty((M, point_limit), dtype=torch.int64, device=dev)
    km = torch.empty((M, point_limit), dtype=torch.uint8, device=dev)
    nm = torch.empty((M,), dtype=torch.uint8, device=dev)
    status = torch.zeros(1, dtype=torch.int32, device=dev)
    _lib.check(_L().lcr_point_to_node_partition_stack(_lib.ptr(points.contiguous()), po.ctypes.data, _lib.ptr(nodes.contiguous()), mo.ctypes.data, C,
                                                      int(point_limit), _lib.ptr(p2n), _lib.ptr(knn), _lib.ptr(km), _lib.ptr(nm), _lib.ptr(status),
                                                      _lib.ptr(ws), ws.numel(), _sp(points)), "lcr_point_to_node_partition_stack")
    return p2n, nm.bool(), knn, km.bool()


class _PendingStatus(threading.local):
    def __init__(self):
        self.items = []


_pending_ot_status = _PendingStatus()
_PENDING_OT_MAX = 32


def check_transport_status():
    items, _pending_ot_status.items = _pending_ot_status.items, []
    if items and any(int(t.reshape(()).item()) != 0 for t in items):
        raise RuntimeError("lcr_log_sinkhorn: a workgroup hand-off of the persistent form timed out (set LCR_SINKHORN_COOP=0)")


def log_optimal_transport(raw_scores, row_masks, col_masks, alpha, scale=1.0, iters=100, inf=1e12):
    B, M, N = raw_scores.shape
    dev = raw_scores.device
    rm, cm = row_masks.to(torch.uint8).contiguous(), col_masks.to(torch.uint8).contiguous()
    S = torch.empty((B, M + 1, N + 1), dtype=torch.float32, device=dev)
    _lib.check(_L().lcr_build_padded_scores(_lib.ptr(raw_scores.contiguous()), _lib.ptr(rm), _lib.ptr(cm), B, M, N, float(scale),
                                            _lib.ptr(alpha.reshape(1).float()), float(inf), _lib.ptr(S), _sp(S)), "lcr_build_padded_scores")
    return _transport_padded(S, rm, cm, iters, inf)


PATCH_SCORES_FUSED = [os.environ.get("LCR_PATCH_SCORES_FUSED", "1") != "0"]


def patch_log_optimal_transport(feats_a, idx_a, feats_b, idx_b, mask_a, mask_b, alpha, scale=1.0, iters=100, inf=1e12):
    P, K = idx_a.shape
    if not PATCH_SCORES_FUSED[0] or K != 128 or feats_a.shape[1] % 32 != 0 or P == 0:
        fa, fb = gather_rows(feats_a, idx_a.contiguous()), gather_rows(feats_b, idx_b.contiguous())
        return log_optimal_transport(bmm_nt(fa, fb), mask_a, mask_b, alpha, scale=scale, iters=iters, inf=inf)
    dev = feats_a.device
    fa, fb = feats_a.contiguous(), feats_b.contiguous()
# ... 607 lines not shown
```

### lcr-net_amd/modules/kpconv/modules.py

```python
import os

import torch
import torch.nn as nn

from ... import functional as F
from .kpconv import KPConv


class StageContext:

    def __init__(self, seg_len=None, order=None, min_rows=None):
        self.seg_len = seg_len
        self.order = order
        self.min_rows = min_rows

    def norm_on_load(self, K, N, M):
        if _NO_NORM_ON_LOAD or not F.gemm_anorm_ok(K, N):
            return False
        rows = M if self.seg_len is None else self.min_rows
        return rows is not None and rows >= F.ANORM_MIN_SEG_ROWS


_NO_NORM_ON_LOAD = bool(os.environ.get("LCR_NO_NORM_ON_LOAD"))
_WHOLE = StageContext(None)


class GroupNorm(nn.Module):
    def __init__(self, num_groups, num_channels):
        super().__init__()
        self.num_groups, self.num_channels = num_groups, num_channels
        self.norm = nn.GroupNorm(num_groups, num_channels)

    def forward(self, x, ctx=_WHOLE, act=False, slope=0.1):
        stats = F.groupnorm_stats(x.contiguous(), self.num_groups, ctx.seg_len)
        return F.groupnorm_apply(x.contiguous(), stats, self.norm.weight, self.norm.bias, self.num_groups, ctx.seg_len, act=act, slope=slope)


class UnaryBlock(nn.Module):
    def __init__(self, in_channels, out_channels, group_norm, has_relu=True, bias=True, layer_norm=False):
        super().__init__()
        assert not layer_norm, "layer_norm=True is not used by the reference configs"
        self.in_channels, self.out_channels, self.group_norm = in_channels, out_channels, group_norm
        self.mlp = nn.Linear(in_channels, out_channels, bias=bias)
        self.norm = GroupNorm(group_norm, out_channels)
        self.leaky_relu = nn.LeakyReLU(0.1) if has_relu else None

    def weight_split(self):
        w = self.mlp.weight
        c = getattr(self, "_ws_cache", None)
        if c is None or not c[0].same(w):
            with F.derived_lock:
                c = getattr(self, "_ws_cache", None)
                if c is None or not c[0].same(w):
                    c = self._ws_cache = (F.WeightStamp(w), F.publish_derived(F.split_bf16x3(w)))
        return c[1]

    def _apply(self, fn, *args, **kwargs):
        F.drop_derived(self, "_ws_cache")
        return super()._apply(fn, *args, **kwargs)

    def raw(self, x, ctx):
        if F.gemm_split_enabled() and F.gemm_split_ok(self.out_channels, self.in_channels):
            return F.gemm_bsplit(x.contiguous(), self.weight_split(), bias=self.mlp.bias, seg_len=ctx.seg_len, groups=self.group_norm)
        return F.gemm(x.contiguous(), self.mlp.weight, trans_b=True, bias=self.mlp.bias, seg_len=ctx.seg_len, groups=self.group_norm)

    def forward(self, x, ctx=_WHOLE, want_pos=False):
        y, stats = self.raw(x, ctx)
        return F.groupnorm_apply(y, stats, self.norm.norm.weight, self.norm.norm.bias, self.group_norm, ctx.seg_len,
                                 act=self.leaky_relu is not None, want_pos=want_pos)


class LastUnaryBlock(nn.Module):
    def __init__(self, in_channels, out_channels, bias=True):
        super().__init__()
        self.mlp = nn.Linear(in_channels, out_channels, bias=bias)

    def forward(self, x):
        w = self.mlp.weight
        if F.gemm_split_enabled() and F.gemm_split_ok(w.shape[0], w.shape[1]):
            c = getattr(self, "_ws_cache", None)
            if c is None or not c[0].same(w):
                with F.derived_lock:
                    c = getattr(self, "_ws_cache", None)
                    if c is None or not c[0].same(w):
                        c = self._ws_cache = (F.WeightStamp(w), F.publish_derived(F.split_bf16x3(w)))
            return F.gemm_bsplit(x.contiguous(), c[1], bias=self.mlp.bias)[0]
        return F.gemm(x.contiguous(), w, trans_b=True, bias=self.mlp.bias)[0]

    def _apply(self, fn, *args, **kwargs):
        F.drop_derived(self, "_ws_cache")
        return super()._apply(fn, *args, **kwargs)


class ConvBlock(nn.Module):
    def __init__(self, in_channels, out_channels, kernel_size, radius, sigma, group_norm, negative_slope=0.1, bias=True, layer_norm=False):
        super().__init__()
        assert not layer_norm
        self.in_channels, self.out_channels, self.group_norm = in_channels, out_channels, group_norm
        self.KPConv = KPConv(in_channels, out_channels, kernel_size, radius, sigma, bias=bias)
        self.norm = GroupNorm(group_norm, out_channels)
        self.leaky_relu = nn.LeakyReLU(negative_slope=negative_slope)
        self.negative_slope = negative_slope

    def forward(self, s_feats, q_points, s_points, neighbor_indices, q_ctx=_WHOLE, s_ctx=_WHOLE):
        x, stats = self.KPConv.forward_raw(s_feats, q_points, s_points, neighbor_indices, seg_len=q_ctx.seg_len, groups=self.group_norm,
                                           order=q_ctx.order)
        return F.groupnorm_apply(x, stats, self.norm.norm.weight, self.norm.norm.bias, self.group_norm, q_ctx.seg_len,
                                 act=True, slope=self.negative_slope)


class ResidualBlock(nn.Module):
    def __init__(self, in_channels, out_channels, kernel_size, radius, sigma, group_norm, strided=False, bias=True, layer_norm=False):
        super().__init__()
        assert not layer_norm
        self.in_channels, self.out_channels, self.strided, self.group_norm = in_channels, out_channels, strided, group_norm
        mid = out_channels // 4
        self.unary1 = UnaryBlock(in_channels, mid, group_norm, bias=bias) if in_channels != mid else nn.Identity()
        self.KPConv = KPConv(mid, mid, kernel_size, radius, sigma, bias=bias)
        self.norm_conv = GroupNorm(group_norm, mid)
        self.unary2 = UnaryBlock(mid, out_channels, group_norm, has_relu=False, bias=bias)
        self.unary_shortcut = (UnaryBlock(in_channels, out_channels, group_norm, has_relu=False, bias=bias)
                               if in_channels != out_channels else nn.Identity())
        self.leaky_relu = nn.LeakyReLU(0.1)

    def forward(self, s_feats, q_points, s_points, neighbor_indices, q_ctx=_WHOLE, s_ctx=_WHOLE):
        g = self.group_norm
        s_feats = s_feats.contiguous()
        if isinstance(self.unary1, nn.Identity):
            x, pos = s_feats, None
        else:
            x, pos = self.unary1(s_feats, s_ctx, want_pos=True)
        x, stats = self.KPConv.forward_raw(x, q_points, s_points, neighbor_indices, s_pos=pos, seg_len=q_ctx.seg_len, groups=g,
                                           order=q_ctx.order)
        if q_ctx.norm_on_load(x.shape[1], self.out_channels, x.shape[0]):
            y, ystats = F.gemm_anorm(x, stats, self.norm_conv.norm.weight, self.norm_conv.norm.bias, g, self.unary2.mlp.weight,
                                     bias=self.unary2.mlp.bias, seg_len=q_ctx.seg_len, groups=g)
        else:
            x = F.groupnorm_apply(x, stats, self.norm_conv.norm.weight, self.norm_conv.norm.bias, g, q_ctx.seg_len, act=True)
            y, ystats = self.unary2.raw(x, q_ctx)
        shortcut = F.maxpool(s_feats, neighbor_indices, order=q_ctx.order) if self.strided else s_feats
        if isinstance(self.unary_shortcut, nn.Identity):
            res, res_norm = shortcut, None
        else:
            res, rstats = self.unary_shortcut.raw(shortcut, q_ctx)
            res_norm = (rstats, self.unary_shortcut.norm.norm.weight, self.unary_shortcut.norm.norm.bias)
        return F.groupnorm_apply(y, ystats, self.unary2.norm.norm.weight, self.unary2.norm.norm.bias, g, q_ctx.seg_len,
                                 res=res, res_norm=res_norm, act=True, slope=0.1)
```

Measured before the change: 2993 scans/s.

## Add bf16x3-split GEMM with normalise-on-load and lower split threshold to K>=256

Adds a normalise-on-load variant of the bf16x3 split GEMM. It applies the producer's GroupNorm affine and leaky ReLU to A while parking tiles, and uses it for the residual-block unary2 GEMM after KPConv. It also lowers the split eligibility threshold from K>=288 to K>=256 and centralises that check in a shared library function. The goal is to move more fp32 GEMM work onto bf16 matrix cores while keeping the fused normalisation. The trade-offs are extra per-element FMA work in the park stage, reused LDS scratch, and a precision path now applied to K=256 GEMMs.

```diff
diff --git a/include/lcr_hip.h b/include/lcr_hip.h
--- a/include/lcr_hip.h
+++ b/include/lcr_hip.h
@@ -107,6 +107,7 @@
 int lcr_split_bf16x3_tiles(const float* w, int N, int K, uint16_t* tiles, void* stream);
 int lcr_gemm_f32_bsplit(const float* A, const uint16_t* Bs_tiles, float* C, int64_t M, int N, int K, const float* bias, const float* rowdiv,
                         const int64_t* seg_len, int S, int groups, double* stats, void* stream);
+int lcr_gemm_split_ok(int N, int K);
 int lcr_gemm_f32_masked(const float* A, const float* B, float* C, int64_t M, int N, int K, const float* bias, const float* rowdiv,
                         const int64_t* seg_len, int S, int groups, double* stats, const uint16_t* row_mask, int block_k, void* stream);
 int lcr_gemm_f32_bsplit_masked(const float* A, const uint16_t* Bs_tiles, float* C, int64_t M, int N, int K, const float* bias,
@@ -116,6 +117,9 @@
 int lcr_gemm_f32_anorm(const float* A, const float* B, float* C, int64_t M, int N, int K, const float* bias,
                        const double* a_stats, const float* a_gamma, const float* a_beta, int a_groups, float a_eps,
                        float a_slope, const int64_t* seg_len, int S, int groups, double* stats, void* stream);
+int lcr_gemm_f32_bsplit_anorm(const float* A, const uint16_t* Bs_tiles, float* C, int64_t M, int N, int K, const float* bias,
+                              const double* a_stats, const float* a_gamma, const float* a_beta, int a_groups, float a_eps,
+                              float a_slope, const int64_t* seg_len, int S, int groups, double* stats, void* stream);
 int lcr_gemm_f32_batched_ta(const float* A, const float* B, float* C, int64_t M, int N, int count, const int* k_host,
                             const int64_t* a_off_host, const int64_t* b_off_host, const int64_t* c_off_host, void* stream);
 int lcr_kpconv_aggregate(const float* s_feats, const uint8_t* s_pos, const float* q_pts, const float* s_pts,
diff --git a/lcr-net_amd/_lib.py b/lcr-net_amd/_lib.py
--- a/lcr-net_amd/_lib.py
+++ b/lcr-net_amd/_lib.py
@@ -92,6 +92,9 @@
     "lcr_split_bf16x3": (c_int, [c_vp, c_i64, c_vp, c_vp]),
     "lcr_split_bf16x3_tiles": (c_int, [c_vp, c_int, c_int, c_vp, c_vp]),
     "lcr_gemm_f32_bsplit": (c_int, [c_vp, c_vp, c_vp, c_i64, c_int, c_int, c_vp, c_vp, c_vp, c_int, c_int, c_vp, c_vp]),
+    "lcr_gemm_split_ok": (c_int, [c_int, c_int]),
+    "lcr_gemm_f32_bsplit_anorm": (c_int, [c_vp, c_vp, c_vp, c_i64, c_int, c_int, c_vp, c_vp, c_vp, c_vp, c_int, c_float, c_float, c_vp, c_int,
+                                          c_int, c_vp, c_vp]),
     "lcr_gemm_f32_bsplit_masked": (c_int, [c_vp, c_vp, c_vp, c_i64, c_int, c_int, c_vp, c_vp, c_vp, c_int, c_int, c_vp, c_vp, c_int, c_vp]),
     "lcr_gemm_f32_masked": (c_int, [c_vp, c_vp, c_vp, c_i64, c_int, c_int, c_vp, c_vp, c_vp, c_int, c_int, c_vp, c_vp, c_int, c_vp]),
     "lcr_kpconv_mask_ok": (c_int, [c_i64, c_int, c_int, c_int]),
diff --git a/lcr-net_amd/csrc/encoder.hip b/lcr-net_amd/csrc/encoder.hip
--- a/lcr-net_amd/csrc/encoder.hip
+++ b/lcr-net_amd/csrc/encoder.hip
@@ -50,7 +50,7 @@
   float* y = ws.take<float>(static_cast<size_t>(n) * cout);
   double* stats = sp.take();
   if (!y || !stats) return LCR_ESPACE;
-  const bool split = u.w_split && cin >= 288 && cin % 32 == 0 && cout >= 64;
+  const bool split = u.w_split && lcr_gemm_split_ok(cout, cin);
   int rc = split ? TURN(lcr_gemm_f32_bsplit(x, u.w_split, y, n, cout, cin, u.b, nullptr, st.seg, sp.S, sp.groups, stats, s))
                  : TURN(lcr_gemm_f32(x, u.w, y, n, cout, cin, 0, 1, u.b, nullptr, st.seg, sp.S, sp.groups, stats, s));
   *y_out = y;
@@ -114,8 +114,11 @@
     y = ws.take<float>(static_cast<size_t>(M) * b.cout);
     sty = sp.take();
     if (!y || !sty) return LCR_ESPACE;
-    if ((rc = TURN(lcr_gemm_f32_anorm(kpo, b.unary2.w, y, M, b.cout, mid, b.unary2.b, stc, b.normconv_w, b.normconv_b, g, ENC_GN_EPS, ENC_SLOPE,
-                                      q.seg, sp.S, g, sty, s))))
+    const bool u2_split = b.unary2.w_split && lcr_gemm_split_ok(b.cout, mid);
+    if ((rc = TURN(u2_split ? lcr_gemm_f32_bsplit_anorm(kpo, b.unary2.w_split, y, M, b.cout, mid, b.unary2.b, stc, b.normconv_w, b.normconv_b, g,
+                                                        ENC_GN_EPS, ENC_SLOPE, q.seg, sp.S, g, sty, s)
+                            : lcr_gemm_f32_anorm(kpo, b.unary2.w, y, M, b.cout, mid, b.unary2.b, stc, b.normconv_w, b.normconv_b, g, ENC_GN_EPS,
+                                                 ENC_SLOPE, q.seg, sp.S, g, sty, s))))
       return rc;
   } else {
     float* x2 = ws.take<float>(static_cast<size_t>(M) * mid);
diff --git a/lcr-net_amd/csrc/gemm_f32.hip b/lcr-net_amd/csrc/gemm_f32.hip
--- a/lcr-net_amd/csrc/gemm_f32.hip
+++ b/lcr-net_amd/csrc/gemm_f32.hip
@@ -38,6 +38,50 @@
   float         eps, slope;
 };
 constexpr int AN_KMAX = 256;
+
+__device__ __forceinline__ void anorm_affine(const ANorm& an, int K, float (&g)[2], float (&b)[2]) {
+#pragma unroll
+  for (int u = 0; u < 2; ++u) {
+    g[u] = b[u] = 0.f;
+    const int e = threadIdx.x + u * GM_T;
+    if (e < 2 * K) {
+      const int k = e >= K ? e - K : e;
+      g[u] = an.gamma[k];
+      b[u] = an.beta[k];
+    }
+  }
+}
+__device__ __forceinline__ void anorm_finalise(const ANorm& an, const GemmEpilogue& ep, int K, int blk_first, const float (&an_g)[2],
+                                               const float (&an_b)[2], float2* s_mr, float* s_an) {
+  const int gs = K / an.groups;
+  for (int e = threadIdx.x; e < 2 * an.groups; e += GM_T) {
+    const int slot = e >= an.groups ? 1 : 0, g = e - slot * an.groups;
+    const int sg = min(blk_first + slot, ep.S - 1);
+    const double cnt = static_cast<double>(ep.seg_len[sg]) * gs;
+    double sx = 0.0, sxx = 0.0;
+    for (int rep = 0; rep < GN_REPLICAS; ++rep) {
+      const int64_t o = ((static_cast<int64_t>(rep) * ep.S + sg) * an.groups + g) * 2;
+      sx += an.stats[o];
+      sxx += an.stats[o + 1];
+    }
+    const double mean = sx / cnt;
+    const double var = fmax(sxx / cnt - mean * mean, 0.0);
+    s_mr[e] = make_float2(static_cast<float>(mean), static_cast<float>(1.0 / sqrt(var + static_cast<double>(an.eps))));
+  }
+  __syncthreads();
+#pragma unroll
+  for (int u = 0; u < 2; ++u) {
+    const int e = threadIdx.x + u * GM_T;
+    if (e < 2 * K) {
+      const int slot = e >= K ? 1 : 0, k = e - slot * K;
+      const float2 mr = s_mr[slot * an.groups + k / gs];
+      const float sc = mr.y * an_g[u];
+      s_an[slot * 2 * AN_KMAX + k] = sc;
+      s_an[slot * 2 * AN_KMAX + AN_KMAX + k] = fmaf(-mr.x, sc, an_b[u]);
+    }
+  }
+  __syncthreads();
+}
 
 __device__ __forceinline__ float4 ld4(const float* p) { return *reinterpret_cast<const float4*>(p); }
 
@@ -158,10 +202,10 @@
   return s;
 }
 
-template <int BM, int BN, int WM, int WN, int NT>
+template <int BM, int BN, int WM, int WN, int NT, bool EXT = false>
 __device__ __forceinline__ void gemm_epilogue(floatx16 (&acc)[NT], float* __restrict__ C, int64_t M, int N, int64_t m0, int n0, int64_t m_tile,
                                               const GemmEpilogue& ep, const float (&bias_v)[NT], int blk_first, int64_t blk_seg_start,
-                                              int64_t blk_seg_end, int wm, int wn, int lane) {
+                                              int64_t blk_seg_end, int wm, int wn, int lane, float* scratch = nullptr) {
   const bool want_stats = ep.stats != nullptr;
   const int gs = want_stats ? N / ep.groups : 1;
   const int64_t wrow0 = m0 + wm * 32;
@@ -213,7 +257,8 @@
   }
 
   if (want_stats) {
-    __shared__ float s_part[2][2 * WM][BN];
+    __shared__ float s_own[EXT ? 1 : 2 * 2 * WM * BN];
+    float (*s_part)[2 * WM][BN] = reinterpret_cast<float (*)[2 * WM][BN]>(EXT ? scratch : s_own);
     double* rep = ep.stats + static_cast<int64_t>(m_tile % GN_REPLICAS) * ep.S * ep.groups * 2;
     int64_t seg_start = blk_seg_start, seg_end = blk_seg_end;
     const int64_t blk_last_row = min(m0 + BM - 1, M - 1);
@@ -390,17 +435,7 @@
     bias_v[j] = (ep.bias && col < N) ? ep.bias[col] : 0.f;
   }
   float an_g[2] = {0.f, 0.f}, an_b[2] = {0.f, 0.f};
-  if constexpr (ANORM) {
-#pragma unroll
-    for (int u = 0; u < 2; ++u) {
-      const int e = threadIdx.x + u * GM_T;
-      if (e < 2 * K) {
-        const int k = e >= K ? e - K : e;
-        an_g[u] = an.gamma[k];
-        an_b[u] = an.beta[k];
-      }
-    }
-  }
+  if constexpr (ANORM) anorm_affine(an, K, an_g, an_b);
   int blk_first = 0;
   int64_t blk_seg_start = 0, blk_seg_end = 0;
   if (want_stats || ANORM) {
@@ -415,35 +450,8 @@
   int an_split = BM;
   if constexpr (ANORM) {
     an_split = static_cast<int>(min(static_cast<int64_t>(BM), blk_seg_end - m0));
-    const int gs = K / an.groups;
     __shared__ float2 s_mr[2 * 64];
-    for (int e = threadIdx.x; e < 2 * an.groups; e += GM_T) {
-      const int slot = e >= an.groups ? 1 : 0, g = e - slot * an.groups;
-      const int sg = min(blk_first + slot, ep.S - 1);
-      const double cnt = static_cast<double>(ep.seg_len[sg]) * gs;
-      double sx = 0.0, sxx = 0.0;
-      for (int rep = 0; rep < GN_REPLICAS; ++rep) {
-        const int64_t o = ((static_cast<int64_t>(rep) * ep.S + sg) * an.groups + g) * 2;
-        sx += an.stats[o];
-        sxx += an.stats[o + 1];
-      }
-      const double mean = sx / cnt;
-      const double var = fmax(sxx / cnt - mean * mean, 0.0);
-      s_mr[e] = make_float2(static_cast<float>(mean), static_cast<float>(1.0 / sqrt(var + static_cast<double>(an.eps))));
-    }
-    __syncthreads();
-#pragma unroll
-    for (int u = 0; u < 2; ++u) {
-      const int e = threadIdx.x + u * GM_T;
-      if (e < 2 * K) {
-        const int slot = e >= K ? 1 : 0, k = e - slot * K;
-        const float2 mr = s_mr[slot * an.groups + k / gs];
-        const float sc = mr.y * an_g[u];
-        s_an[slot * 2 * AN_KMAX + k] = sc;
-        s_an[slot * 2 * AN_KMAX + AN_KMAX + k] = fmaf(-mr.x, sc, an_b[u]);
-      }
-    }
-    __syncthreads();
+    anorm_finalise(an, ep, K, blk_first, an_g, an_b, s_mr, s_an);
   }
   auto sstore_a0 = [&]() {
     if constexpr (ANORM) la_t[0].store_norm(As[0], s_an, an_split, an.slope);
@@ -852,10 +860,11 @@
   *reinterpret_cast<u32x4_t*>(dst + 8192) = p3;
 }
 
-template <int ABL, int NWM, int D = 2, bool MASK = false>
-__global__ __launch_bounds__(128 * NWM, 2) void k_gemm_f32_bsplit_p(const float* __restrict__ A, const uint16_t* __restrict__ Bs, float* __restrict__ C,
+template <int ABL, int NWM, int D = 2, bool MASK = false, bool ANORM = false>
+__global__ __launch_bounds__(128 * NWM, ANORM ? 3 : 2) void k_gemm_f32_bsplit_p(const float* __restrict__ A, const uint16_t* __restrict__ Bs, float* __restrict__ C,
                                                              int64_t M, int N, int K, GemmEpilogue ep, const uint16_t* __restrict__ amask,
-                                                             int kshift) {
+                                                             int kshift, ANorm an) {
+  static_assert(!ANORM || (!MASK && 128 * NWM == GM_T), "normalise-on-load: 256 threads, unmasked A");
   constexpr int BM = 32 * NWM, BN = 64, RS = 64, T = 128 * NWM, PLA = BM * RS, STGA = 3 * PLA, PL = 64 * RS;
   constexpr int NPB = (768 + T - 1) / T;
   constexpr int STG = 3 * PL + (NPB * T - 768) * 16;
@@ -921,13 +930,25 @@
 #pragma unroll
     for (int j = 0; j < NPB; ++j) rb[st][j] = *reinterpret_cast<const u32x4_t*>(bp + static_cast<int64_t>(tt) * 12288 + bsrc[j]);
   };
-  auto park = [&](auto st_c, int lds_stage) {
+  __shared__ __attribute__((aligned(16))) float s_an[ANORM ? 4 * AN_KMAX : 4];
+  int an_off[2] = {0, 0};
+  auto park = [&](auto st_c, int lds_stage, int t) {
     constexpr int st = decltype(st_c)::value;
     char* da = sA + lds_stage * STGA;
     char* db = sB + lds_stage * STG;
+    const int tt = t < nk ? t : nk - 1;
 #pragma unroll
     for (int j = 0; j < 2; ++j) {
       uint32_t h1, h2, h3, g1, g2, g3;
+      if constexpr (ANORM) {
+        const float* tb = s_an + an_off[j] + tt * GM_BK;
+        const float4 sc = *reinterpret_cast<const float4*>(tb), sh = *reinterpret_cast<const float4*>(tb + AN_KMAX);
+        f32x4_t v = ra[st][j];
+        v.x = fmaf(v.x, sc.x, sh.x), v.y = fmaf(v.y, sc.y, sh.y), v.z = fmaf(v.z, sc.z, sh.z), v.w = fmaf(v.w, sc.w, sh.w);
+        v.x = v.x > 0.f ? v.x : v.x * an.slope, v.y = v.y > 0.f ? v.y : v.y * an.slope;
+        v.z = v.z > 0.f ? v.z : v.z * an.slope, v.w = v.w > 0.f ? v.w : v.w * an.slope;
+        ra[st][j] = v;
+      }
       if constexpr (ABL & 2) {
         h1 = __float_as_uint(ra[st][j].x), h2 = __float_as_uint(ra[st][j].y), h3 = h1, g1 = __float_as_uint(ra[st][j].z), g2 = __float_as_uint(ra[st][j].w), g3 = g1;
       } else {
@@ -962,9 +983,11 @@
     const int col = n0 + wn * 32 + (lane & 31);
     bias_v[0] = (ep.bias && col < N) ? ep.bias[col] : 0.f;
   }
+  float an_g[2] = {0.f, 0.f}, an_b[2] = {0.f, 0.f};
+  if constexpr (ANORM) anorm_affine(an, K, an_g, an_b);
   int blk_first = 0;
   int64_t blk_seg_start = 0, blk_seg_end = 0;
-  if (ep.stats != nullptr) {
+  if (ep.stats != nullptr || ANORM) {
     blk_seg_end = ep.seg_len[0];
     while (blk_first + 1 < ep.S && m0 >= blk_seg_end) {
       ++blk_first;
@@ -972,7 +995,13 @@
       blk_seg_end += ep.seg_len[blk_first];
     }
   }
-  park(I0{}, 0);
+  if constexpr (ANORM) {
+    anorm_finalise(an, ep, K, blk_first, an_g, an_b, reinterpret_cast<float2*>(sB), s_an);
+    const int an_split = static_cast<int>(min(static_cast<int64_t>(BM), blk_seg_end - m0));
+#pragma unroll
+    for (int j = 0; j < 2; ++j) an_off[j] = (srow + j * (T / 8) >= an_split ? 2 * AN_KMAX : 0) + spc * 4;
+  }
+  park(I0{}, 0, 0);
   fetch(I0{}, D);
   __syncthreads();
   auto step = [&](auto lds_c, auto reg_c, int t) {
@@ -1012,7 +1041,7 @@
     mm(a0[1], b0[0], acc2);
     mm(a0[0], b0[1], acc);
     mm(a0[0], b0[0], acc2);
-    park(NX{}, P ^ 1);
+    park(NX{}, P ^ 1, t + 1);
     mm(a1[2], b1[0], acc);
     mm(a1[0], b1[2], acc2);
     mm(a1[1], b1[1], acc);
@@ -1047,7 +1076,8 @@
 #pragma unroll
   for (int r = 0; r < 16; ++r) acc[r] += acc2[r];
   floatx16 accs[1] = {acc};
-  gemm_epilogue<BM, BN, NWM, 2, 1>(accs, C, M, N, m0, n0, m_tile, ep, bias_v, blk_first, blk_seg_start, blk_seg_end, wm, wn, lane);
+  gemm_epilogue<BM, BN, NWM, 2, 1, ANORM>(accs, C, M, N, m0, n0, m_tile, ep, bias_v, blk_first, blk_seg_start, blk_seg_end, wm, wn, lane,
+                                          reinterpret_cast<float*>(sA));
 }
 
 struct GemmStreamK {
@@ -1431,7 +1461,8 @@
 }
 
 static int bsplit_impl(const float* A, const uint16_t* Bs, float* C, int64_t M, int N, int K, const float* bias, const float* rowdiv,
-                       const int64_t* seg_len, int S, int groups, double* stats, const uint16_t* amask, int kshift, void* stream) {
+                       const int64_t* seg_len, int S, int groups, double* stats, const uint16_t* amask, int kshift, void* stream,
+                       const ANorm* an = nullptr) {
   if (!A || !Bs || !C || M < 0 || N <= 0 || K <= 0 || K % GM_BK != 0 || reinterpret_cast<uintptr_t>(A) % 16 != 0 || reinterpret_cast<uintptr_t>(Bs) % 16 != 0 ||
       K < GM_BK) {
     set_error("lcr_gemm_f32_bsplit: needs K %% 32 == 0 and 16-byte aligned operands");
@@ -1448,19 +1479,23 @@
   const int mt8 = (div_up(M, 64) + 7) / 8 * 8;
   static const int abl = getenv("LCR_SPLIT_ABL") ? atoi(getenv("LCR_SPLIT_ABL")) : 0;
   const dim3 grid(mt8 * div_up(N, 64)), block(256);
+  if (an) {
+    LCR_LAUNCH_TIMED((k_gemm_f32_bsplit_p<0, 2, 2, false, true>), grid, block, 0, st, A, Bs, C, M, N, K, ep, amask, kshift, *an);
+    return check_launch("lcr_gemm_f32_bsplit_anorm");
+  }
   if (amask) {
-    LCR_LAUNCH_TIMED((k_gemm_f32_bsplit_p<0, 2, 2, true>), grid, block, 0, st, A, Bs, C, M, N, K, ep, amask, kshift);
+    LCR_LAUNCH_TIMED((k_gemm_f32_bsplit_p<0, 2, 2, true>), grid, block, 0, st, A, Bs, C, M, N, K, ep, amask, kshift, ANorm{});
     return check_launch("lcr_gemm_f32_bsplit_masked");
   }
   switch (abl) {
-    case 1: LCR_LAUNCH_TIMED((k_gemm_f32_bsplit_p<1, 2>), grid, block, 0, st, A, Bs, C, M, N, K, ep, amask, kshift); break;
-    case 2: LCR_LAUNCH_TIMED((k_gemm_f32_bsplit_p<2, 2>), grid, block, 0, st, A, Bs, C, M, N, K, ep, amask, kshift); break;
-    case 4: LCR_LAUNCH_TIMED((k_gemm_f32_bsplit_p<4, 2>), grid, block, 0, st, A, Bs, C, M, N, K, ep, amask, kshift); break;
-    case 8: LCR_LAUNCH_TIMED((k_gemm_f32_bsplit_p<8, 2>), grid, block, 0, st, A, Bs, C, M, N, K, ep, amask, kshift); break;
-    case 16: LCR_LAUNCH_TIMED((k_gemm_f32_bsplit_p<16, 2>), grid, block, 0, st, A, Bs, C, M, N, K, ep, amask, kshift); break;
-    case 23: LCR_LAUNCH_TIMED((k_gemm_f32_bsplit_p<23, 2>), grid, block, 0, st, A, Bs, C, M, N, K, ep, amask, kshift); break;
-    case 30: LCR_LAUNCH_TIMED((k_gemm_f32_bsplit_p<30, 2>), grid, block, 0, st, A, Bs, C, M, N, K, ep, amask, kshift); break;
-    default: LCR_LAUNCH_TIMED((k_gemm_f32_bsplit_p<0, 2>), grid, block, 0, st, A, Bs, C, M, N, K, ep, amask, kshift); break;
+    case 1: LCR_LAUNCH_TIMED((k_gemm_f32_bsplit_p<1, 2>), grid, block, 0, st, A, Bs, C, M, N, K, ep, amask, kshift, ANorm{}); break;
+    case 2: LCR_LAUNCH_TIMED((k_gemm_f32_bsplit_p<2, 2>), grid, block, 0, st, A, Bs, C, M, N, K, ep, amask, kshift, ANorm{}); break;
+    case 4: LCR_LAUNCH_TIMED((k_gemm_f32_bsplit_p<4, 2>), grid, block, 0, st, A, Bs, C, M, N, K, ep, amask, kshift, ANorm{}); break;
+    case 8: LCR_LAUNCH_TIMED((k_gemm_f32_bsplit_p<8, 2>), grid, block, 0, st, A, Bs, C, M, N, K, ep, amask, kshift, ANorm{}); break;
+    case 16: LCR_LAUNCH_TIMED((k_gemm_f32_bsplit_p<16, 2>), grid, block, 0, st, A, Bs, C, M, N, K, ep, amask, kshift, ANorm{}); break;
+    case 23: LCR_LAUNCH_TIMED((k_gemm_f32_bsplit_p<23, 2>), grid, block, 0, st, A, Bs, C, M, N, K, ep, amask, kshift, ANorm{}); break;
+    case 30: LCR_LAUNCH_TIMED((k_gemm_f32_bsplit_p<30, 2>), grid, block, 0, st, A, Bs, C, M, N, K, ep, amask, kshift, ANorm{}); break;
+    default: LCR_LAUNCH_TIMED((k_gemm_f32_bsplit_p<0, 2>), grid, block, 0, st, A, Bs, C, M, N, K, ep, amask, kshift, ANorm{}); break;
   }
   return check_launch("lcr_gemm_f32_bsplit");
 }
@@ -1468,6 +1503,23 @@
 extern "C" int lcr_gemm_f32_bsplit(const float* A, const uint16_t* Bs, float* C, int64_t M, int N, int K, const float* bias, const float* rowdiv,
                                    const int64_t* seg_len, int S, int groups, double* stats, void* stream) {
   return bsplit_impl(A, Bs, C, M, N, K, bias, rowdiv, seg_len, S, groups, stats, nullptr, 0, stream);
+}
+
+extern "C" int lcr_gemm_split_ok(int N, int K) {
+  return N >= 64 && K >= 256 && K % GM_BK == 0;
+}
+
+extern "C" int lcr_gemm_f32_bsplit_anorm(const float* A, const uint16_t* Bs, float* C, int64_t M, int N, int K, const float* bias,
+                                         const double* a_stats, const float* a_gamma, const float* a_beta, int a_groups, float a_eps,
+                                         float a_slope, const int64_t* seg_len, int S, int groups, double* stats, void* stream) {
+  if (K <= 0 || K > AN_KMAX || !a_stats || !a_gamma || !a_beta || a_groups < 1 || K % a_groups != 0 || a_groups > 64 || !seg_len || S < 1 ||
+      (M > 0 && M < 64 * static_cast<int64_t>(S))) {
+    set_error("lcr_gemm_f32_bsplit_anorm: needs K <= 256, a_groups <= 64 dividing K, the producer's statistics and affine, and a segment table "
+              "whose segments all hold >= 64 rows");
+    return LCR_EARG;
+  }
+  const ANorm an{a_stats, a_gamma, a_beta, a_groups, a_eps, a_slope};
+  return bsplit_impl(A, Bs, C, M, N, K, bias, nullptr, seg_len, S, groups, stats, nullptr, 0, stream, &an);
 }
 
 static int mask_kshift(int K, int block_k) {
diff --git a/lcr-net_amd/functional.py b/lcr-net_amd/functional.py
--- a/lcr-net_amd/functional.py
+++ b/lcr-net_amd/functional.py
@@ -174,7 +174,7 @@
 
 
 def gemm_split_ok(N, K):
-    return K >= 288 and K % 32 == 0 and N >= 64
+    return bool(_lib.lib().lcr_gemm_split_ok(int(N), int(K)))
 
 
 derived_lock = threading.RLock()
@@ -277,6 +277,23 @@
         _lib.ptr(a), _lib.ptr(weight), _lib.ptr(c), M, N, K, _lib.ptr(bias), _lib.ptr(a_stats), _lib.ptr(a_gamma), _lib.ptr(a_beta),
         int(a_groups), GN_EPS, float(slope), _lib.ptr(seg_len), S, int(groups), _lib.ptr(stats), _lib.stream_ptr(a.device)),
         "lcr_gemm_f32_anorm"), meta=(M, N, K))
+    return c, stats
+
+
+def gemm_bsplit_anorm(a, a_stats, a_gamma, a_beta, a_groups, planes, bias=None, seg_len=None, groups=0, slope=0.1):
+    _lib.require_cuda(a, planes)
+    assert a.dtype == torch.float32 and a.is_contiguous() and planes.dtype == torch.int16 and planes.is_contiguous() and planes.dim() == 5
+    M, K = a.shape
+    N = planes.lcr_n
+    assert planes.shape[1] * 32 == K and planes.shape[0] == (N + 63) // 64, "inner dimensions differ"
+    c = torch.empty((M, N), dtype=torch.float32, device=a.device)
+    seg_len = _seg(seg_len, M, a.device)
+    S = seg_len.numel()
+    stats = _zero_stats(S, groups, a.device) if groups else None
+    _timed("gemm", lambda: _lib.check(_lib.lib().lcr_gemm_f32_bsplit_anorm(
+        _lib.ptr(a), _lib.ptr(planes), _lib.ptr(c), M, N, K, _lib.ptr(bias), _lib.ptr(a_stats), _lib.ptr(a_gamma), _lib.ptr(a_beta),
+        int(a_groups), GN_EPS, float(slope), _lib.ptr(seg_len), S, int(groups), _lib.ptr(stats), _lib.stream_ptr(a.device)),
+        "lcr_gemm_f32_bsplit_anorm"), meta=(M, N, K))
     return c, stats
 
 
diff --git a/lcr-net_amd/modules/kpconv/modules.py b/lcr-net_amd/modules/kpconv/modules.py
--- a/lcr-net_amd/modules/kpconv/modules.py
+++ b/lcr-net_amd/modules/kpconv/modules.py
@@ -133,8 +133,12 @@
         x, stats = self.KPConv.forward_raw(x, q_points, s_points, neighbor_indices, s_pos=pos, seg_len=q_ctx.seg_len, groups=g,
                                            order=q_ctx.order)
         if q_ctx.norm_on_load(x.shape[1], self.out_channels, x.shape[0]):
-            y, ystats = F.gemm_anorm(x, stats, self.norm_conv.norm.weight, self.norm_conv.norm.bias, g, self.unary2.mlp.weight,
-                                     bias=self.unary2.mlp.bias, seg_len=q_ctx.seg_len, groups=g)
+            if F.gemm_split_enabled() and F.gemm_split_ok(self.out_channels, x.shape[1]):
+                y, ystats = F.gemm_bsplit_anorm(x, stats, self.norm_conv.norm.weight, self.norm_conv.norm.bias, g, self.unary2.weight_split(),
+                                                bias=self.unary2.mlp.bias, seg_len=q_ctx.seg_len, groups=g)
+            else:
+                y, ystats = F.gemm_anorm(x, stats, self.norm_conv.norm.weight, self.norm_conv.norm.bias, g, self.unary2.mlp.weight,
+                                         bias=self.unary2.mlp.bias, seg_len=q_ctx.seg_len, groups=g)
         else:
             x = F.groupnorm_apply(x, stats, self.norm_conv.norm.weight, self.norm_conv.norm.bias, g, q_ctx.seg_len, act=True)
             y, ystats = self.unary2.raw(x, q_ctx)
```

New measurement: 3013 scans/s, median of 6. No clear change (+0.6%).
